# psaegert/bcnf

Hardware: AMD Instinct MI355X
Metric: NLL-training samples/sec + log_prob max-abs-err vs ref, trajectory_FC_small (higher is better)
Workload: dtype f32; 1 GPU; trajectory_FC_small NLL training step (configs[1]); batch_per_gpu=4096, global_batch=4096, parallelism=dp1, hip_graph=True, n_blocks=32, n_conditions=80

## Files before the change

bcnf_amd/_native.py:

```python
from __future__ import annotations

import ctypes
import os
import threading

import torch

_HERE = os.path.dirname(os.path.abspath(__file__))
LIB_PATH = os.environ.get("BCNF_AMD_LIB") or os.path.join(_HERE, "libbcnf_amd.so")

MAX_HIDDEN = 8

OK, ERR_ARG, ERR_UNSUPPORTED, ERR_HIP = 0, 1, 2, 3
ERR_HIP_BASE = 1000

EXPORTS = (
    "bcnf_stack_supported", "bcnf_param_count", "bcnf_packed_bytes", "bcnf_workspace_bytes",
    "bcnf_slab_bytes", "bcnf_pack_params", "bcnf_stack_forward", "bcnf_stack_backward",
    "bcnf_stack_inverse", "bcnf_grad_reduce", "bcnf_status_string",
    "bcnf_nll_forward", "bcnf_nll_backward", "bcnf_grad_partials", "bcnf_adam_step", "bcnf_adam_step_bookkeep",
    "bcnf_grad_sumsq",
    "bcnf_clip_grad_norm", "bcnf_linear_forward", "bcnf_linear_work_bytes", "bcnf_linear_backward",
    "bcnf_linear_gelu_forward", "bcnf_linear_gelu_backward",
    "bcnf_inverse_scratch_bytes", "bcnf_stack_dh", "bcnf_backward_tail", "bcnf_gather_rows2",
    "bcnf_gather_batch", "bcnf_advance_counters", "bcnf_fold_bytes", "bcnf_fold_slab_bytes",
    "bcnf_pack_params_fold", "bcnf_fold_nll_forward", "bcnf_fold_backward_tail",
    "bcnf_fold_raw_table_bytes", "bcnf_fold_raw_table", "bcnf_fold_train_forward", "bcnf_lds_fill",
    "bcnf_wide_supported", "bcnf_wide_param_count", "bcnf_wide_packed_bytes", "bcnf_wide_workspace_bytes", "bcnf_wide_inverse_scratch_bytes",
    "bcnf_wide_pack", "bcnf_wide_forward", "bcnf_wide_nll_finalize", "bcnf_wide_backward", "bcnf_wide_inverse",
    "bcnf_wide_fold_prepare", "bcnf_wide_fold_forward", "bcnf_wide_fold_backward", "bcnf_wide_proj_rows",
    "bcnf_wide_fold_backward_range", "bcnf_wide_fold_backward_phase", "bcnf_wide_block_offset",
    "bcnf_wide_gemm_test", "bcnf_wide_backward_plan", "bcnf_rank_count", "bcnf_resimulate",
    "bcnf_guard_check_global", "bcnf_abi_version",
    "bcnf_head_work_bytes", "bcnf_head_mse_forward", "bcnf_head_mse_backward", "bcnf_hybrid_finalize",
    "bcnf_stack_inverse_logdet", "bcnf_wide_inverse_logdet",
    "bcnf_attn_forward", "bcnf_attn_backward", "bcnf_add_layernorm_forward", "bcnf_add_layernorm_work_bytes",
    "bcnf_add_layernorm_backward",
)
ABI_VERSION = 2
MAX_TENSORS = 48


class BcnfStackDesc(ctypes.Structure):
    _fields_ = [
        ("size", ctypes.c_int32),
        ("n_conditions", ctypes.c_int32),
        ("n_hidden", ctypes.c_int32),
        ("hidden", ctypes.c_int32 * MAX_HIDDEN),
        ("n_blocks", ctypes.c_int32),
        ("act_norm", ctypes.c_int32),
        ("two_way", ctypes.c_int32),
        ("dropout", ctypes.c_float),
        ("gemm_tiling", ctypes.c_int32),
    ]


class BcnfFoldAdam(ctypes.Structure):
    _fields_ = [
        ("params", ctypes.c_void_p * 3),
        ("exp_avg", ctypes.c_void_p * 3),
        ("exp_avg_sq", ctypes.c_void_p * 3),
        ("step", ctypes.c_void_p),
        ("lr", ctypes.c_double),
        ("beta1", ctypes.c_double),
        ("beta2", ctypes.c_double),
        ("eps", ctypes.c_double),
        ("weight_decay", ctypes.c_double),
        ("advance_cursor", ctypes.c_void_p),
        ("cursor_modulo", ctypes.c_int64),
        ("log_values", ctypes.c_void_p),
        ("log_history", ctypes.c_void_p),
        ("done_counter", ctypes.c_void_p),
        ("guard", ctypes.c_void_p),
    ]


class BcnfGather2(ctypes.Structure):
    _fields_ = [
        ("idx", ctypes.c_void_p),
        ("cursor", ctypes.c_void_p),
        ("n", ctypes.c_int64),
        ("src0", ctypes.c_void_p),
        ("cols0", ctypes.c_int32),
        ("dst0", ctypes.c_void_p),
        ("src1", ctypes.c_void_p),
        ("cols1", ctypes.c_int32),
        ("dst1", ctypes.c_void_p),
    ]


def make_desc(size, nested_sizes, n_blocks, n_conditions, dropout=0.0, act_norm=False, two_way=False):
    d = BcnfStackDesc()
    d.size = int(size)
    d.n_conditions = int(n_conditions)
    d.n_hidden = len(nested_sizes)
    if len(nested_sizes) > MAX_HIDDEN:
        raise ValueError(f"bcnf_amd supports at most {MAX_HIDDEN} nested layers, got {len(nested_sizes)}")
    for i, hsz in enumerate(nested_sizes):
        d.hidden[i] = int(hsz)
    d.n_blocks = int(n_blocks)
    d.act_norm = 1 if act_norm else 0
    d.two_way = 1 if two_way else 0
    d.dropout = float(dropout)
    return d


_lib = None
_lock = threading.Lock()

_vp = ctypes.c_void_p
_i32 = ctypes.c_int32
_i64 = ctypes.c_int64
_pdesc = ctypes.POINTER(BcnfStackDesc)
_pi64 = ctypes.POINTER(ctypes.c_int64)


def _bind(lib):
    sig = {
        "bcnf_stack_supported": (_i32, [_pdesc]),
        "bcnf_param_count": (_i32, [_pdesc, _pi64, _pi64]),
        "bcnf_packed_bytes": (_i32, [_pdesc, _pi64]),
        "bcnf_workspace_bytes": (_i32, [_pdesc, _i64, _i32, _pi64]),
        "bcnf_slab_bytes": (_i32, [_pdesc, _i64, _pi64]),
        "bcnf_pack_params": (_i32, [_pdesc, _vp, _vp, _vp, _vp]),
        "bcnf_inverse_scratch_bytes": (_i32, [_pdesc, _i64, _pi64]),
        "bcnf_stack_dh": (_i32, [_pdesc, _vp, _vp, _i64, _i32, _vp, _vp]),
        "bcnf_backward_tail": (_i32, [_pdesc, _vp, _vp, _vp, _vp, _i64, _i32, _vp, _vp, _vp]),
        "bcnf_gather_rows2": (_i32, [_vp, _i64, _vp, _i32, _vp, _vp, _i32, _vp, _vp]),
        "bcnf_gather_batch": (_i32, [_vp, _vp, _i64, _vp, _i32, _vp, _vp, _i32, _vp, _vp]),
        "bcnf_advance_counters": (_i32, [_vp, _vp, _i64, _vp]),
        "bcnf_guard_check_global": (_i32, [_vp, _vp, _vp]),
        "bcnf_stack_forward": (_i32, [_pdesc, _vp, _vp, _vp, _i64, _vp, _vp, _vp, _i32, _vp, _vp, _i32, _vp]),
        "bcnf_stack_backward": (_i32, [_pdesc, _vp, _vp, _vp, _vp, _i64, _i32, _vp, _vp, _vp, _vp, _vp, _vp]),
        "bcnf_stack_inverse": (_i32, [_pdesc, _vp, _vp, _vp, _i64, _vp, _i64, _vp, _i32, _vp, _vp, _vp]),
        "bcnf_stack_inverse_logdet": (_i32, [_pdesc, _vp, _vp, _vp, _i64, _vp, _i64, _vp, _vp, _vp, _vp, _vp]),
        "bcnf_grad_reduce": (_i32, [_pdesc, _vp, _vp, _vp, _i64, _i32, _vp, _vp]),
        "bcnf_nll_forward": (_i32, [_pdesc, _vp, _vp, _vp, _i64, _vp, _vp, _i32, _vp, _vp, _i32, _vp, _vp, _vp]),
        "bcnf_nll_backward": (_i32, [_pdesc, _vp, _vp, _vp, _vp, _i64, _i32, _vp, _vp, _vp, _vp, _vp, _vp, _vp,
                                     _vp, _vp]),
        "bcnf_fold_bytes": (_i32, [_pdesc, _i32, _pi64]),
        "bcnf_fold_slab_bytes": (_i32, [_pdesc, _i32, _i64, _pi64]),
        "bcnf_pack_params_fold": (_i32, [_pdesc, _vp, _vp, _vp, _vp, _i32, _vp, _vp, _vp, _vp]),
        "bcnf_fold_nll_forward": (_i32, [_pdesc, _vp, _vp, _i32, _vp, _vp, _i32, _i64, _vp, _vp, _i32, _vp, _vp,
                                         _i32, _vp, _vp, _vp]),
        "bcnf_fold_raw_table_bytes": (_i32, [_pdesc, _i32, _pi64]),
        "bcnf_lds_fill": (_i32, [ctypes.c_float, _vp]),
        "bcnf_fold_raw_table": (_i32, [_pdesc, _i32, _vp]),
        "bcnf_fold_train_forward": (_i32, [_pdesc, _vp, _vp, _vp, _vp, _vp, _i32, _vp, _vp, _vp, _i32, _i64, _vp,
                                           _vp, _vp, _i32, _vp, _vp, _i32, _vp, _vp, _vp]),
        "bcnf_fold_backward_tail": (_i32, [_pdesc, _vp, _vp, _vp, _i32, _i32, _vp, _vp, _vp, _i64, _i32, _vp, _vp,
                                           _vp, _vp, _vp]),
        "bcnf_grad_partials": (_i64, [_i64]),
        "bcnf_adam_step": (_i32, [_i32, _vp, _vp, _vp, _vp, _vp, _vp, ctypes.c_double, ctypes.c_double,
                                  ctypes.c_double, ctypes.c_double, ctypes.c_double, _vp, _i32, _vp, _vp]),
        "bcnf_adam_step_bookkeep": (_i32, [_i32, _vp, _vp, _vp, _vp, _vp, _vp, ctypes.c_double, ctypes.c_double,
                                           ctypes.c_double, ctypes.c_double, ctypes.c_double, _vp, _i64, _vp, _vp,
                                           _vp, _vp, _vp]),
        "bcnf_grad_sumsq": (_i32, [_i32, _vp, _vp, _vp, _vp]),
        "bcnf_clip_grad_norm": (_i32, [_i32, _vp, _vp, _vp, ctypes.c_float, _vp, _vp, _vp, _i64, _vp, _vp, _vp,
                                       _vp]),
        "bcnf_linear_forward": (_i32, [_vp, _vp, _vp, _i64, _i32, _i32, _vp, _vp]),
        "bcnf_linear_work_bytes": (_i64, [_i64, _i32, _i32]),
        "bcnf_linear_backward": (_i32, [_vp, _vp, _vp, _i64, _i32, _i32, _vp, _vp, _vp, _vp, _vp]),
        "bcnf_linear_gelu_forward": (_i32, [_vp, _vp, _vp, _i64, _i32, _i32, ctypes.c_float, _vp, _i32, _vp, _vp,
                                            _vp]),
        "bcnf_linear_gelu_backward": (_i32, [_vp, _vp, _vp, _vp, _i64, _i32, _i32, _vp, _vp, _vp, _vp, _vp]),
        "bcnf_wide_supported": (_i32, [_pdesc]),
        "bcnf_wide_param_count": (_i32, [_pdesc, _pi64, _pi64]),
        "bcnf_wide_packed_bytes": (_i32, [_pdesc, _pi64]),
        "bcnf_wide_workspace_bytes": (_i32, [_pdesc, _i64, _i32, _pi64]),
        "bcnf_wide_inverse_scratch_bytes": (_i32, [_pdesc, _i64, _i64, _pi64]),
        "bcnf_wide_pack": (_i32, [_pdesc, _vp, _vp, _vp, _vp]),
        "bcnf_wide_forward": (_i32, [_pdesc, _vp, _vp, _vp, _vp, _i64, _vp, _vp, _vp, _i32, _vp, _vp, _i32, _vp]),
        "bcnf_wide_fold_prepare": (_i32, [_pdesc, _vp, _vp, _i32, _vp, _vp]),
        "bcnf_wide_fold_forward": (_i32, [_pdesc, _vp, _vp, _vp, _vp, _i32, _vp, _i64, _vp, _vp, _i32, _vp, _vp, _vp]),
        "bcnf_wide_fold_backward": (_i32, [_pdesc, _vp, _vp, _vp, _i32, _vp, _vp, _vp, _vp, _i64, _vp, _vp, _vp, _vp,
                                           _vp, _vp]),
        "bcnf_wide_fold_backward_range": (_i32, [_pdesc, _vp, _vp, _vp, _i32, _vp, _vp, _vp, _vp, _i64, _vp, _vp, _vp,
                                                 _vp, _vp, _i32, _i32, _vp]),
        "bcnf_wide_fold_backward_phase": (_i32, [_pdesc, _vp, _vp, _vp, _i32, _vp, _vp, _vp, _vp, _i64, _vp, _vp, _vp,
                                                 _vp, _vp, _i32, _vp]),
        "bcnf_wide_block_offset": (_i32, [_pdesc, _i32, _pi64]),
        "bcnf_wide_proj_rows": (_i32, [_pdesc, _pi64]),
        "bcnf_wide_nll_finalize": (_i32, [_pdesc, _vp, _i64, _i32, _vp, _vp, _vp, _vp]),
        "bcnf_wide_backward": (_i32, [_pdesc, _vp, _vp, _vp, _vp, _vp, _vp, _vp, _i32, _i64, _vp, _vp, _vp, _vp,
                                      _vp]),
        "bcnf_wide_inverse": (_i32, [_pdesc, _vp, _vp, _vp, _vp, _i64, _vp, _i64, _vp, _i32, _vp, _vp, _vp]),
        "bcnf_wide_inverse_logdet": (_i32, [_pdesc, _vp, _vp, _vp, _vp, _i64, _vp, _i64, _vp, _vp, _vp, _vp, _vp]),
        "bcnf_rank_count": (_i32, [_vp, _vp, _i64, _i64, _i32, _vp, _vp]),
        "bcnf_resimulate": (_i32, [_vp, _i32, _i64, _i64, _i32, _vp, _vp, _vp, _i32, ctypes.c_double, _i32,
                                   ctypes.c_double, ctypes.c_double, _i32, _vp, _vp, _vp, _vp]),
        "bcnf_wide_gemm_test": (_i32, [_i32, _i32, _i32, _i32, _vp, _i64, _vp, _i64, _vp, _i64, _vp]),
        "bcnf_wide_backward_plan": (_i32, [_pdesc, _i64, _i32, _i32, _i32, _i32, _i32, _pi64]),
        "bcnf_head_work_bytes": (_i32, [_i64, _i32, _i32, _pi64]),
        "bcnf_head_mse_forward": (_i32, [_vp, _i64, _i32, _vp, _vp, _vp, _i64, _i32, _vp, _vp]),
        "bcnf_head_mse_backward": (_i32, [_vp, _i64, _i32, _vp, _vp, _vp, ctypes.c_float, _i64, _i32, _vp, _vp, _vp,
                                          _i64, _i32, _vp]),
        "bcnf_hybrid_finalize": (_i32, [_vp, _vp, _i64, _i32, ctypes.c_float, _vp, _vp]),
        "bcnf_attn_forward": (_i32, [_vp, _vp, _vp, _i64, _i32, _i32, _i32, _i64, _vp, _vp, _vp]),
        "bcnf_attn_backward": (_i32, [_vp, _vp, _vp, _vp, _vp, _vp, _i64, _i32, _i32, _i32, _i64, _vp, _vp, _vp, _vp]),
        "bcnf_add_layernorm_forward": (_i32, [_vp, _vp, _vp, _vp, _i64, _i32, ctypes.c_float, _vp, _vp, _vp, _vp]),
        "bcnf_add_layernorm_work_bytes": (_i32, [_i64, _i32, _pi64]),
        "bcnf_add_layernorm_backward": (_i32, [_vp, _vp, _vp, _vp, _vp, _vp, _i64, _i32, _vp, _vp, _vp, _vp, _vp]),
        "bcnf_status_string": (ctypes.c_char_p, [_i32]),
        "bcnf_abi_version": (_i32, []),
    }
    override = "BCNF_AMD_LIB" in os.environ
    for name, (res, args) in sig.items():
        if override and not hasattr(lib, name):
            continue
        fn = getattr(lib, name)
        fn.restype = res
        fn.argtypes = args


def lib():
    global _lib
    if _lib is None:
        with _lock:
            if _lib is None:
                if not os.path.exists(LIB_PATH):
                    raise RuntimeError(
                        f"bcnf_amd: HIP library {LIB_PATH} is missing. Build it with "
                        "`python -c 'import __graft_entry__ as g; g.build()'` (hipcc --offload-arch=gfx950).")
                handle = ctypes.CDLL(LIB_PATH)
                _bind(handle)
                if (hasattr(handle, "bcnf_abi_version") or "BCNF_AMD_LIB" not in os.environ) and \
                        handle.bcnf_abi_version() != ABI_VERSION:
                    raise RuntimeError(f"bcnf_amd: {LIB_PATH} has ABI version {handle.bcnf_abi_version()}, the "
                                       f"bindings expect {ABI_VERSION}: rebuild the library")
                _lib = handle
    return _lib


# ... 54 lines not shown
```

bcnf_amd/csrc/bcnf_stack.hip:

```cpp
#include "bcnf_device.h"
#include "../../include/bcnf_amd.h"

#include <math.h>
#include <stdlib.h>
#include <string.h>

#include <algorithm>
#include <utility>
#include <vector>


#ifdef BCNF_PHASE_STAMPS
#define BCNF_STAMPS 1
#else
#define BCNF_STAMPS 0
#endif

namespace {

constexpr int NC16_MAX = 16;
constexpr int TILE = 256;
__host__ __device__ constexpr int tile_slot(int r, int q) { return 4 * r + ((q + (r >> 1)) & 3); }
__host__ __device__ constexpr int tile_ix(int s, int r) { return 4 * tile_slot(r, s & 3) + (s >> 2); }
__host__ __device__ constexpr int sample_of(int t8) { return (t8 >> 6) + 4 * ((t8 >> 4) & 3); }
// ... 233 lines not shown
    return rec_f(L, P, Q, k, feat(q, r), (half ? L.rf_s : L.rf_t) + 16, true);
  }
  e -= 32;
  const int q = e >> 4, r = (e >> 2) & 3, i = e & 3;
  return rec_f(L, P, Q, k, feat(q, r), i, true);
}

constexpr int RAW_NP = 10, RAW_NQ = 2, RAW_NZ = 6;
constexpr int RAW_NS = RAW_NP + RAW_NQ + RAW_NZ;
constexpr int RAW_NSP = (RAW_NS + 3) & ~3;
constexpr int RAW_DUMMY = RING - 1;
constexpr int RAW_SRC_MAX = 1 << 20;

__host__ __device__ constexpr uint32_t raw_entry(int dst, int src) { return (uint32_t)dst | ((uint32_t)src << 12); }

int q_quad_source(const BcnfLayout& L, int j, int c, bool inverse, int* off) {
  int qi, src;
  if (!q_entry(L, j, c, &qi, &src)) return 0;
  const int Da = L.Da, Db = L.Db, D = L.D;
  const int no = (qi < 2) ? Da : Db, ni = (qi & 1) ? Db : Da;
  if (j >= no || src >= ni) return 0;
  const int gi = (qi & 1) ? Da + src : src, go = (qi < 2) ? j : Da + j;
  *off = inverse ? go * D + gi : gi * D + go;
  return 2;
}

int rec_f_source(const BcnfLayout& L, int j, int e, int* off) {
  const int Da = L.Da, Db = L.Db, D = L.D, NH = L.NH, an = L.an_size;
  auto lin_w = [&](int l, int row, int col) { return an + L.lin_w[l] + row * L.lin_in[l] + col; };
  *off = 0;
  if (e < 4) {
    if (!L.act_norm) return ((e == 0 && j < Da) || (e == 2 && j < Db)) ? -1 : 0;
    switch (e) {
      case 0: return j < Da ? (*off = j, 1) : 0;
      case 1: return j < Da ? (*off = D + j, 1) : 0;
      case 2: return j < Db ? (*off = Da + j, 1) : 0;
      default: return j < Db ? (*off = D + Da + j, 1) : 0;
    }
  }
  if (e == L.rf_b1) return j < L.H[1] ? (*off = an + L.lin_b[1] + j, 1) : 0;
  if (e >= L.rf_w1 && e < L.rf_w1 + 16) {
    const int src = rec_src(L, j, e - L.rf_w1, QBC_W1);
    return (j < L.H[1] && src < Da) ? (*off = lin_w(1, j, src), 1) : 0;
  }
  if (e >= L.rf_hid && e < L.rf_t) {
    const int l = 2 + (e - L.rf_hid) / 17, r = (e - L.rf_hid) % 17;
    if (r == 16) return j < L.H[l] ? (*off = an + L.lin_b[l] + j, 1) : 0;
    const int src = (j - r) & 15;
    return (j < L.H[l] && src < L.H[l - 1]) ? (*off = lin_w(l, j, src), 1) : 0;
  }
  if (e >= L.rf_t && e < L.rf_t + 34) {
    const int half = (e - L.rf_t) / 17, r = (e - L.rf_t) % 17;
    if (r == 16) return j < Db ? (*off = an + L.lin_b[NH + 1] + half * Db + j, 1) : 0;
    const int src = (j - r) & 15;
    return (j < Db && src < L.H[NH]) ? (*off = lin_w(NH + 1, half * Db + j, src), 1) : 0;
  }
  if (e >= L.rf_q && e < L.rf_q + 64) return q_quad_source(L, j, e - L.rf_q, false, off);
  return 0;
}

int rec_b_source(const BcnfLayout& L, int j, int e, int* off) {
  const int NH = L.NH, Da = L.Da, Db = L.Db, D = L.D, an = L.an_size;
  auto lin_w = [&](int l, int row, int col) { return an + L.lin_w[l] + row * L.lin_in[l] + col; };
  *off = 0;
  if (e >= L.rb_w1t && e < L.rb_w1t + 16) {
    const int src = (j - (e - L.rb_w1t)) & 15;
    return (j < Da && src < L.H[1]) ? (*off = lin_w(1, src, j), 1) : 0;
  }
  if (e >= L.rb_hid && e < L.rb_w1t) {
    const int l = NH - (e - L.rb_hid) / 16, r = (e - L.rb_hid) % 16, src = (j - r) & 15;
    return (j < L.H[l - 1] && src < L.H[l]) ? (*off = lin_w(l, src, j), 1) : 0;
  }
  if (e >= L.rb_tt && e < L.rb_tt + 32) {
    const int half = (e - L.rb_tt) / 16, src = rec_src(L, j, (e - L.rb_tt) % 16, QBC_HEAD);
    return (j < L.H[NH] && src < Db) ? (*off = lin_w(NH + 1, half * Db + src, j), 1) : 0;
  }
  if (e >= L.rb_qt && e < L.rb_qt + 64) return q_quad_source(L, j, e - L.rb_qt, true, off);
  if (e >= L.rb_an && e < L.rb_an + 4) return rec_f_source(L, j, e - L.rb_an, off);
  return 0;
}

long long raw_table_words(const BcnfLayout& L) { return (long long)RAW_NSP * BCNF_WG + 16LL * L.RB; }

bool build_raw_table(const BcnfLayout& L, uint32_t* out) {
  if (L.nb < 2 || 16 * L.RF > RAW_DUMMY || L.blk_stride >= RAW_SRC_MAX) return false;
  std::vector<std::pair<int, int>> ent[3];
  for (int j = 0; j < 16; ++j)
    for (int e = 0; e < L.RF; ++e) {
      int off;
      const int kind = rec_f_source(L, j, e, &off);
      if (kind < 0) return false;
      ent[kind == 1 ? 0 : kind == 2 ? 1 : 2].emplace_back(off, j * L.RF + e);
    }
  const int cap[3] = {RAW_NP, RAW_NQ, RAW_NZ}, first[3] = {0, RAW_NP, RAW_NP + RAW_NQ};
  for (int i = 0; i < RAW_NSP * BCNF_WG; ++i) out[i] = raw_entry(RAW_DUMMY, 0);
  if (L.an_size > BCNF_WG) return false;
  for (int g = 0; g < 3; ++g) {
    if ((int)ent[g].size() > cap[g] * BCNF_WG) return false;
    std::sort(ent[g].begin(), ent[g].end());
    for (int n = 0; n < (int)ent[g].size(); ++n)
      out[(n % BCNF_WG) * RAW_NSP + first[g] + n / BCNF_WG] = raw_entry(ent[g][n].second, ent[g][n].first);
  }
  uint32_t* pb = out + (long long)RAW_NSP * BCNF_WG;
  for (int j = 0; j < 16; ++j)
    for (int e = 0; e < L.RB; ++e) {
      int off;
      const int kind = rec_b_source(L, j, e, &off);
      if (kind < 0 || off >= (1 << 29)) return false;
      pb[j * L.RB + e] = ((uint32_t)off << 2) | (uint32_t)(kind == 1 ? 0 : kind == 2 ? 1 : 2);
    }
  return true;
}

constexpr int PACK_WG_MAX = 4096;

__device__ __forceinline__ void pack_body(const BcnfLayout& L, const float* __restrict__ P,
                                          const float* __restrict__ Q, float* __restrict__ out, int bx, int npw,
                                          float* __restrict__ part, bool train_only = false) {
  if (bx == 0) {
    float acc = 0.f;
    if (L.act_norm) {
      const int n = (L.nb - 1) * L.D;
      for (int i = threadIdx.x; i < n; i += BCNF_WG) {
        const int k = i / L.D, d = i - k * L.D;
        acc += logf(fabsf(P[k * L.blk_stride + d]));
      }
    }
    part[threadIdx.x] = acc;
    __syncthreads();
    for (int s = BCNF_WG / 2; s > 0; s >>= 1) {
      if ((int)threadIdx.x < s) part[threadIdx.x] += part[threadIdx.x + s];
      __syncthreads();
    }
    if (threadIdx.x == 0) out[L.ldc_off] = part[0];
    return;
  }
  const int n_pf = L.nb * 16 * L.RF;
  const int n_pb = L.nb * 16 * L.RB;
  const int n_w = L.Cp * L.NKp;
  const int n_pm = L.nb * L.PMB;
  const int total = train_only ? n_pf + n_pb + n_w : 2 * n_pf + n_pb + 2 * n_w + L.NKp + n_pm;
  for (int ii0 = (bx - 1) * BCNF_WG + threadIdx.x; ii0 < total; ii0 += npw * BCNF_WG) {
    float v;
    long long o;
    const int i = (train_only && ii0 >= n_pf + n_pb) ? ii0 + n_pf + n_w : ii0;
    if (i < n_pf) {
      const int kj = i / L.RF, e = i - kj * L.RF;
      v = rec_f(L, P, Q, kj >> 4, kj & 15, e, false);
      o = L.pf_off + i;
    } else if (i < n_pf + n_pb) {
      const int ii = i - n_pf;
      const int kj = ii / L.RB, e = ii - kj * L.RB;
      v = rec_b(L, P, Q, kj >> 4, kj & 15, e);
      o = L.pb_off + ii;
    } else if (i < 2 * n_pf + n_pb) {
      const int ii = i - n_pf - n_pb;
      const int kj = ii / L.RF, e = ii - kj * L.RF;
      v = rec_f(L, P, Q, kj >> 4, kj & 15, e, true);
      o = L.pi_off + ii;
    } else if (i < 2 * n_pf + n_pb + n_w) {
      const int ii = i - 2 * n_pf - n_pb;
      const int c = ii / L.NKp, kj = ii - c * L.NKp, k = kj >> 4, j = kj & 15;
      v = (k < L.nb && j < L.H[1] && c < L.C) ? cW(L, P, k, 1, j, L.Da + c) : 0.f;
      o = L.w1c_off + ii;
    } else if (i < 2 * n_pf + n_pb + 2 * n_w) {
      const int ii = i - 2 * n_pf - n_pb - n_w;
      const int kj = ii / L.Cp, c = ii - kj * L.Cp, k = kj >> 4, j = kj & 15;
      v = (k < L.nb && j < L.H[1] && c < L.C) ? cW(L, P, k, 1, j, L.Da + c) : 0.f;
      o = L.w1r_off + ii;
    } else if (i < 2 * n_pf + n_pb + 2 * n_w + L.NKp) {
      const int kj = i - 2 * n_pf - n_pb - 2 * n_w, k = kj >> 4, j = kj & 15;
      v = (k < L.nb && j < L.H[1]) ? cB(L, P, k, 1, j) : 0.f;
      o = L.b1c_off + kj;
    } else {
      const int ii = i - 2 * n_pf - n_pb - 2 * n_w - L.NKp;
      const int k = ii / L.PMB, e = ii - k * L.PMB;
      v = rec_pm(L, P, Q, k, e);
      o = L.pm_off + ii;
    }
    out[o] = v;
  }
}

__global__ __launch_bounds__(BCNF_WG) void k_pack(BcnfLayout L, const float* __restrict__ P,
                                                  const float* __restrict__ Q, float* __restrict__ out, int npw) {
  __shared__ float part[BCNF_WG];
  pack_body(L, P, Q, out, blockIdx.x, npw, part);
}

int pack_wgs(const BcnfLayout& L, bool train_only = false) {
  const long long total = train_only ? (long long)L.nb * 16 * (L.RF + L.RB) + (long long)L.Cp * L.NKp
                                     : 2LL * L.nb * 16 * L.RF + (long long)L.nb * 16 * L.RB + 2LL * L.Cp * L.NKp +
                                           L.NKp + (long long)L.nb * L.PMB;
  const long long w = (total + BCNF_WG - 1) / BCNF_WG;
  return (int)(w < PACK_WG_MAX ? (w > 0 ? w : 1) : PACK_WG_MAX);
// ... 443 lines not shown
        const int i4 = tid + 256 * e, r = i4 >> 5, col = c0 + (i4 & 31) * 4;
        if (col < L.Cp) *reinterpret_cast<floatx4*>(Bs + r * hs + col) = rv[e];
      }
    }
    __syncthreads();
#pragma unroll
    for (int j = 0; j < NT; ++j) {
      const int n = n_lo + j;
      if (n >= n_hi) continue;
#pragma unroll
      for (int t0 = 0; t0 < KH / 4; t0 += 8) {
        float a[8], bv[8];
#pragma unroll
        for (int t = 0; t < 8; ++t) {
          a[t] = As[(16 * kw + lr) * KHP + 4 * (t0 + t) + lq];
          bv[t] = Bs[(4 * (t0 + t) + lq) * hs + 16 * n + lr];
        }
#pragma unroll
        for (int t = 0; t < 8; t += 2) {
          acc[j] = mfma4(a[t], bv[t], acc[j]);
          acc1[j] = mfma4(a[t + 1], bv[t + 1], acc1[j]);
        }
      }
    }
  }
  if (k >= L.nb) return;
  float* o = work + (((long long)s * L.nb + k) * 16) * L.Cp;
#pragma unroll
  for (int j = 0; j < NT; ++j) {
    const int n = n_lo + j;
    if (n >= n_hi) continue;
    const floatx4 r = acc[j] + acc1[j];
#pragma unroll
    for (int i = 0; i < 4; ++i) o[(long long)(4 * lq + i) * L.Cp + 16 * n + lr] = r[i];
  }
}
size_t dw1h_half_lds_bytes(const BcnfLayout& L) {
  return sizeof(float) * (size_t)(32 * KHP + KH * bstride16(L.Cp));
}

__global__ __launch_bounds__(BCNF_WG) void k_dw1h_reduce(BcnfLayout L, const float* __restrict__ work, int splits,
                                                         float* __restrict__ dparams) {
  const long long per = 16LL * L.Cp, total = (long long)L.nb * per;
  const long long i = (long long)blockIdx.x * BCNF_WG + threadIdx.x;
  if (i >= total) return;
  const int k = (int)(i / per);
  const int rem = (int)(i - (long long)k * per);
  const int j = rem / L.Cp, c = rem - j * L.Cp;
  if (j >= L.H[1] || c >= L.C) return;
  float acc = 0.f;
  int s = 0;
  for (; s + 8 <= splits; s += 8) {
    float v[8];
#pragma unroll
    for (int t = 0; t < 8; ++t) v[t] = work[(long long)(s + t) * total + i];
#pragma unroll
    for (int t = 0; t < 8; ++t) acc += v[t];
  }
  for (; s < splits; ++s) acc += work[(long long)s * total + i];
  dparams[coupling_base(L, k) + L.lin_w[1] + j * L.lin_in[1] + L.Da + c] = acc;
}

__device__ __forceinline__ void gx_reduce_body(long long total, const float* __restrict__ work, int splits,
                                               float* __restrict__ gx, long long i) {
  if (i >= total) return;
  float acc = 0.f;
  int s = 0;
  for (; s + 16 <= splits; s += 16) {
    float v[16];
#pragma unroll
    for (int t = 0; t < 16; ++t) v[t] = work[(long long)(s + t) * total + i];
#pragma unroll
    for (int t = 0; t < 16; ++t) acc += v[t];
  }
  for (; s < splits; ++s) acc += work[(long long)s * total + i];
  gx[i] = acc;
}

__global__ __launch_bounds__(BCNF_WG) void k_fold_gx(long long total, const float* __restrict__ work, int splits,
                                                     float* __restrict__ gx) {
  gx_reduce_body(total, work, splits, gx, (long long)blockIdx.x * BCNF_WG + threadIdx.x);
}

__device__ __forceinline__ int c0_of_finish(int bx, int nct) { return (bx % nct) * 16; }

constexpr int FIN_KC = 512;
constexpr int FIN_SMEM = 2 * FIN_KC * 16;

__device__ __forceinline__ void tile16_accum(const float* __restrict__ As, const float* __restrict__ Bs, int kn,
                                             floatx4 (&acc)[4]) {
  const int lane = threadIdx.x & 63, ks = lane & 15, rb = lane >> 4, cb = threadIdx.x >> 6;
#pragma unroll 4
  for (int k = ks; k < kn; k += 16) {
    const floatx4 a = *reinterpret_cast<const floatx4*>(As + k * 16 + 4 * rb);
    const floatx4 b = *reinterpret_cast<const floatx4*>(Bs + k * 16 + 4 * cb);
#pragma unroll
    for (int r = 0; r < 4; ++r)
#pragma unroll
      for (int c = 0; c < 4; ++c) acc[r][c] = fmaf(a[r], b[c], acc[r][c]);
  }
}

__device__ __forceinline__ float tile16_reduce(float* __restrict__ red, const floatx4 (&acc)[4]) {
  const int lane = threadIdx.x & 63, ks = lane & 15, rb = lane >> 4, cb = threadIdx.x >> 6;
  __syncthreads();
#pragma unroll
  for (int r = 0; r < 4; ++r)
#pragma unroll
    for (int c = 0; c < 4; ++c) red[ks * 256 + (4 * rb + r) * 16 + 4 * cb + c] = acc[r][c];
  __syncthreads();
  float v = 0.f;
#pragma unroll
  for (int q = 0; q < 16; ++q) v += red[q * 256 + threadIdx.x];
  return v;
}

__global__ __launch_bounds__(BCNF_WG) void k_fold_finish(BcnfLayout L, const float* __restrict__ pk,
                                                         const float* __restrict__ gx, const float* __restrict__ wf,
                                                         const float* __restrict__ bf, int X,
                                                         float* __restrict__ dparams, float* __restrict__ dwf,
                                                         float* __restrict__ dbf, FoldAdamArgs A) {
  extern __shared__ __attribute__((aligned(16))) float smem[];
  float* As = smem;
  float* Bs = smem + FIN_KC * 16;
  const int Xp = fold_xp(X), tid = threadIdx.x, nct = L.Cp >> 4;
  floatx4 acc[4];
#pragma unroll
  for (int q = 0; q < 4; ++q) acc[q] = floatx4{0.f, 0.f, 0.f, 0.f};
  const bool adam = A.on && !(A.guard && A.guard[BCNF_GUARD_HALTED]);
  AdamScalars as{};
  const bool keeper = adam && blockIdx.x == 0 && tid == 0;
  const bool logger = keeper && A.log_values && A.log_history;
  long long log_row = 0;
  float step0 = 0.f, log_v[3];
  if (adam) {
    as = adam_scalars_of(A, A.asc[0], A.asc[1]);
    if (keeper) {
      log_row = A.cursor ? A.cursor[0] : 0LL;
      step0 = A.step[0];
    }
    if (logger) {
#pragma unroll
      for (int i = 0; i < 3; ++i) log_v[i] = A.log_values[i];
    }
  }
  int slot = -1;
  long long idx = 0;
  float ap = 0.f, am = 0.f, av = 0.f;
  if ((int)blockIdx.x < L.nb * nct) {
    const int j = tid >> 4, c = c0_of_finish(blockIdx.x, nct) + (tid & 15), k = blockIdx.x / nct;
    if (j < L.H[1] && c < L.C) {
      slot = 0;
      idx = coupling_base(L, k) + L.lin_w[1] + j * L.lin_in[1] + L.Da + c;
    }
  } else {
    const int tile = blockIdx.x - L.nb * nct, c = (tile % nct) * 16 + (tid >> 4), x = (tile / nct) * 16 + (tid & 15);
    if (c < L.C) {
      if (x < X) {
        slot = 1;
        idx = (long long)c * X + x;
      } else if (x == X && dbf) {
        slot = 2;
        idx = c;
      }
    }
  }
// ... 174 lines not shown
  return l <= NH ? 24 + 17 * (l - 1) : (l == NH + 1 ? RecF<NH>::S + 17 : RecF<NH>::USED);
}
template <int NH>
__host__ __device__ constexpr int rf_stage_q(int l) {
  int q = 6;
  for (int i = 1; i <= l; ++i) {
    const int want = (rf_stage_end<NH>(i + FWD_AHEAD < NH + 2 ? i + FWD_AHEAD : NH + 2) + 3) / 4;
    q = i >= NH + 2 ? want : (want < q + 8 ? want : q + 8);
  }
  return q;
}
template <int NH>
__device__ __forceinline__ void rf_issue(float* __restrict__ rr, const float* __restrict__ R, int l) {
  const floatx4* R4 = reinterpret_cast<const floatx4*>(R);
#pragma unroll
  for (int q = rf_stage_q<NH>(l - 1); q < rf_stage_q<NH>(l); ++q) {
    const floatx4 v = R4[q];
    rr[4 * q] = v.x;
    rr[4 * q + 1] = v.y;
    rr[4 * q + 2] = v.z;
    rr[4 * q + 3] = v.w;
  }
  __builtin_amdgcn_sched_barrier(0);
}
template <int NH, bool KEEP, bool DROP, typename Emit>
__device__ __forceinline__ void mlp_forward_s(float* __restrict__ rr, const float* __restrict__ R, float x, float hp,
                                              const float* __restrict__ msk, float& T, float& Sp, float* ar,
                                              Emit&& emit, bool qbc) {
  static_assert(RecF<NH>::HID == 24, "stage 1 reads only the prefetched head (FWD_HEAD = 24)");
  using F = RecF<NH>;
  using AR = ActRec<NH>;
  float a = x;
#pragma unroll
  for (int l = 1; l <= NH; ++l) {
    rf_issue<NH>(rr, R, l);
    const float* w = (l == 1) ? rr + F::W1 : rr + F::HID + 17 * (l - 2);
    const float pre = (l == 1 && qbc) ? bc10(a, w, hp) : rot16(a, w, (l == 1) ? hp : w[16]);
    if (KEEP) {
      float g, dg;
      gelu_fg(pre, g, dg);
      a = DROP ? g * msk[l - 1] : g;
      ar[AR::act(l - 1)] = a;
      ar[AR::gd(l - 1)] = DROP ? dg * msk[l - 1] : dg;
#pragma unroll
      for (int q = 0; q < AR::AR4; ++q)
        if (AR::ready_layer(q) == l) emit(q);
    } else if (DROP) {
      float g, dg;
      gelu_fg(pre, g, dg);
      a = g * msk[l - 1];
    } else {
      a = gelu_f(pre);
    }
  }
  rf_issue<NH>(rr, R, NH + 1);
  T = rr[F::T + 16];
  Sp = rr[F::S + 16];
  rot16x2(a, rr + F::T, T, a, rr + F::S, Sp);
  rf_issue<NH>(rr, R, NH + 2);
}

__device__ __forceinline__ void mix(const float* __restrict__ rq, float a, float b, float& na, float& nbv) {
  na = 0.f;
  nbv = 0.f;
  rot16x2(a, rq, na, a, rq + 32, nbv);
  rot16x2(b, rq + 16, na, b, rq + 48, nbv);
}

#if BCNF_STAMPS
__device__ unsigned long long g_phase[32];
#endif

struct ProjArgs {
  const float* h;
  const float* w1c;
  const float* b1c;
  long long ldh;
  int C, Cp, NKp;
};
struct RawArgs {
  const float* P;
  const float* Q;
  const uint32_t* table;
  const float* wf;
  const float* bf;
  const float* ypool;
  float* ydst;
  const float* xpool;
  float* xdst;
  const int64_t* idx;
  const long long* cursor;
  float* pk;
  int X, ldx;
};
constexpr int RAW_WQ = 8;
constexpr int RAW_TPW = 2;
constexpr int RAW_SIDE_Q = 4;
__host__ __device__ constexpr int raw_hs_pitch(int C) { return 16 * ((C + 15) / 16) + 4; }
__device__ __forceinline__ long long raw_row(const RawArgs& R, long long B, long long b) {
  return R.idx ? (long long)R.idx[(R.cursor ? R.cursor[0] * B : 0) + b] : b;
}

constexpr int FWD_WG = 2 * BCNF_WG;
constexpr int HP_SMAX = 16;
constexpr int FWD_SLOTS = 3;
constexpr int FWD_HP = FWD_SLOTS * 4 * 256;
constexpr int FWD_HEAD = 24;

template <int NH, bool DROP, bool SAVE, bool RAW = false>
__global__ __launch_bounds__(2 * BCNF_WG) void k_forward(BcnfLayout L, const float* __restrict__ pk,
                                                    const float* __restrict__ y, ProjArgs P,
                                                    long long B, float* __restrict__ z, float* __restrict__ ldj_out,
                                                    float* __restrict__ logp, const uint64_t* rng,
                                                    float* __restrict__ arec, float* __restrict__ nll_part,
                                                    RawArgs R) {
  extern __shared__ __attribute__((aligned(16))) float smem[];
  const int RFL = 16 * L.RF;
  float* rec = smem;
  float* hpb = rec + FWD_SLOTS * RING;
  floatx4* mkb = reinterpret_cast<floatx4*>(hpb + FWD_HP);
  float* lps = hpb + FWD_HP + FWD_SLOTS * 8 * 256;
  float* hs = lps + 4;
  using AR = ActRec<NH>;
  static_assert(NH <= 8, "two float4 of dropout multipliers");
  const int nb = L.nb;
  const float* pf = pk + L.pf_off;
  const bool helper = threadIdx.x >= BCNF_WG;
  const int t8 = (int)threadIdx.x & (BCNF_WG - 1);
  const int j = t8 & 15, s = sample_of(t8);
  const long long b = (long long)blockIdx.x * 16 + s;
  const long long bc = b < B ? b : B - 1;
  uint64_t seed = 0, off = 0;
  if (DROP) { seed = rng[0]; off = rng[1]; }
  unsigned long long ph_t = BCNF_STAMPS ? __builtin_amdgcn_s_memtime() : 0ULL, ph_acc[3] = {0, 0, 0};
  const unsigned long long ph_t0 = ph_t;
  const unsigned long long ph_r0 = BCNF_STAMPS ? __builtin_amdgcn_s_memrealtime() : 0ULL;
  unsigned long long ph_b[2] = {0, 0};
#define PHB(i)                                                 \
  if (BCNF_STAMPS) ph_b[i] = __builtin_amdgcn_s_memtime() - ph_t0;
  unsigned long long ph_p[4] = {0, 0, 0, 0};
#define PHP(i)                                                                           \
  if (BCNF_STAMPS) {                                                                     \
    asm volatile("s_waitcnt vmcnt(0) lgkmcnt(0)" ::: "memory");                          \
    ph_p[i] = __builtin_amdgcn_s_memtime() - ph_t0;                                      \
  }
#define PHF(i)                                                                                   \
  if (BCNF_STAMPS) {                                                                             \
    const unsigned long long _t = __builtin_amdgcn_s_memtime();                                  \
    ph_acc[i] += _t - ph_t;                                                                      \
    ph_t = _t;                                                                                   \
  }

  if (helper) {
    const int hw = __builtin_amdgcn_readfirstlane(t8 >> 6);
    const int l64 = t8 & 63, lr = l64 & 15, lq = l64 >> 4;
    if constexpr (RAW) {
      const int Da = L.Da, C = L.C, X = R.X, H1 = L.H[1], D = L.D, an = L.an_size;
      const int nt = (C + 15) >> 4;
      const long long row = (long long)blockIdx.x * 16 + lr;
      const float* xrow = R.xpool + raw_row(R, B, row < B ? row : B - 1) * R.ldx;
      uint32_t tw[RAW_NSP];
#pragma unroll
      for (int i = 0; i < RAW_NSP / 4; ++i) {
        const uint4 v = reinterpret_cast<const uint4*>(R.table + t8 * RAW_NSP)[i];
        tw[4 * i] = v.x;
        tw[4 * i + 1] = v.y;
        tw[4 * i + 2] = v.z;
        tw[4 * i + 3] = v.w;
      }
      const int rb16 = 16 * L.RB, ch = (rb16 + BCNF_WG - 1) / BCNF_WG, n_units = nb * ch + L.NKp;
      const uint32_t* tpb = R.table + RAW_NSP * BCNF_WG;
      uint32_t pbe[RAW_SIDE_Q];
#pragma unroll
      for (int q = 0; q < RAW_SIDE_Q; ++q) {
        const int u = blockIdx.x + q * gridDim.x, n = (u % ch) * BCNF_WG + t8;
        pbe[q] = tpb[n < rb16 ? n : 0];
      }
      asm volatile("" ::: "memory");
      uint32_t srcb[RAW_NP + RAW_NQ], dstb[RAW_NP + RAW_NQ];
#pragma unroll
      for (int i = 0; i < RAW_NP + RAW_NQ; ++i) {
        srcb[i] = (tw[i] >> 12) * 4u;
        dstb[i] = (tw[i] & 4095u) * 4u;
      }
      uint32_t zw[RAW_NZ];
#pragma unroll
      for (int i = 0; i < RAW_NZ; ++i) zw[i] = tw[RAW_NP + RAW_NQ + i] & 4095u;
      PHP(0)
      int wo[RAW_TPW];
      uint32_t wok = 0;
#pragma unroll
      for (int i = 0; i < RAW_TPW; ++i) {
        const int c0 = 16 * (hw + 4 * i) + 4 * lq;
        wo[i] = (c0 < C && lr < H1) ? L.lin_w[1] + lr * L.lin_in[1] + Da + c0 : 0;
#pragma unroll
        for (int r = 0; r < 4; ++r) wok |= (c0 + r < C && lr < H1) ? 1u << (4 * i + r) : 0u;
      }
      const bool bias_lane = hw == 0 && lr < H1;
      struct Pre {
// ... 14 lines not shown
        const int cb = coupling_base(L, k);
        const int sp = (k < nb - 1 ? k * L.blk_stride : k * L.blk_stride - an) * 4, sq = k * D * D * 4;
#pragma unroll
        for (int i = 0; i < RAW_NP; ++i)
          g.v[i] = __uint_as_float(__builtin_amdgcn_raw_buffer_load_b32(rP, srcb[i], sp, 0));
#pragma unroll
        for (int i = RAW_NP; i < RAW_NP + RAW_NQ; ++i)
          g.v[i] = __uint_as_float(__builtin_amdgcn_raw_buffer_load_b32(rQ, srcb[i], sq, 0));
#pragma unroll
        for (int i = 0; i < RAW_TPW; ++i) {
          const auto w = __builtin_amdgcn_raw_buffer_load_b128(rP, wo[i] * 4, cb * 4, 0);
          g.w4[i] = floatx4{__uint_as_float(w[0]), __uint_as_float(w[1]), __uint_as_float(w[2]), __uint_as_float(w[3])};
        }
        g.bias = __uint_as_float(__builtin_amdgcn_raw_buffer_load_b32(rP, (L.lin_b[1] + lr) * 4, cb * 4, 0));
      };
      float xa[RAW_TPW][4];
      auto finish_rec = [&](int k, int sl, const Pre& g) {
        if (DROP) {
          const uint32_t bits = dropout_bits<NH>(L, seed, off, bc, k, j, 0u);
          float m[8];
#pragma unroll
          for (int i = 0; i < 8; ++i) m[i] = ((bits >> i) & 1u) ? L.keep_scale : 0.f;
          mkb[(2 * sl) * BCNF_WG + t8] = floatx4{m[0], m[1], m[2], m[3]};
          mkb[(2 * sl + 1) * BCNF_WG + t8] = floatx4{m[4], m[5], m[6], m[7]};
        }
        char* slot = reinterpret_cast<char*>(rec + sl * RING);
        float v0 = g.v[0], vq[RAW_NQ];
#pragma unroll
        for (int i = 0; i < RAW_NQ; ++i) vq[i] = g.v[RAW_NP + i];
        if (k == nb - 1) {
          v0 = an_word ? an_val : v0;
#pragma unroll
          for (int i = 0; i < RAW_NQ; ++i) vq[i] = q_diag[i] ? 1.f : vq[i];
        }
        *reinterpret_cast<float*>(slot + dstb[0]) = v0;
#pragma unroll
        for (int i = 1; i < RAW_NP; ++i) *reinterpret_cast<float*>(slot + dstb[i]) = g.v[i];
#pragma unroll
        for (int i = 0; i < RAW_NQ; ++i) *reinterpret_cast<float*>(slot + dstb[RAW_NP + i]) = vq[i];
      };
      auto finish_proj = [&](int sl, const Pre& g) {
        const float bias = bias_lane ? g.bias : 0.f;
        floatx4 acc = {bias, bias, bias, bias};
#pragma unroll
        for (int i = 0; i < RAW_TPW; ++i)
          if (hw + 4 * i < nt)
#pragma unroll
            for (int r = 0; r < 4; ++r)
              acc = mfma4(xa[i][r], ((wok >> (4 * i + r)) & 1u) ? g.w4[i][r] : 0.f, acc);
        float* hd = hpb + sl * 1024 + hw * 256 + 64 * lq + lr;
#pragma unroll
        for (int r = 0; r < 4; ++r) hd[16 * r] = acc[r];
      };
      auto finish = [&](int k, int sl, const Pre& g) {
        finish_rec(k, sl, g);
        finish_proj(sl, g);
      };
      Pre gb[FWD_SLOTS];
      load(0, gb[0]);
      load(1, gb[1]);
      load(nb > 2 ? 2 : 1, gb[2]);
      asm volatile("" ::: "memory");
      PHP(1)
#pragma unroll
      for (int i = 0; i < RAW_NZ; ++i)
#pragma unroll
        for (int sl = 0; sl < FWD_SLOTS; ++sl) rec[sl * RING + zw[i]] = 0.f;
      finish_rec(0, 0, gb[0]);
      finish_rec(1, 1, gb[1]);
      PHP(2)
      __syncthreads();
      PHB(0)
      __syncthreads();
#pragma unroll
      for (int i = 0; i < RAW_TPW; ++i) {
        const floatx4 v = *reinterpret_cast<const floatx4*>(hs + lr * raw_hs_pitch(C) + 16 * (hw + 4 * i) + 4 * lq);
#pragma unroll
        for (int r = 0; r < 4; ++r) xa[i][r] = v[r];
      }
      finish_proj(0, gb[0]);
      finish_proj(1, gb[1]);
      auto side_unit = [&](int u, uint32_t e) {
        if (u < nb * ch) {
          const int k = u / ch, n = (u - k * ch) * BCNF_WG + t8;
          if (n >= rb16) return;
          const uint32_t kind = e & 3u, src = e >> 2;
          float v = 0.f;
          if (k < nb - 1) {
            if (kind == 0) v = R.P[(long long)k * L.blk_stride + src];
            else if (kind == 1) v = R.Q[(long long)k * D * D + src];
          } else if (kind == 0) {
            v = (int)src < an ? ((int)src < D ? 1.f : 0.f) : R.P[(long long)k * L.blk_stride - an + src];
          } else if (kind == 1) {
            v = (src % (uint32_t)(D + 1)) == 0 ? 1.f : 0.f;
          }
          R.pk[L.pb_off + (long long)k * rb16 + n] = v;
        } else if (u < n_units) {
          const int kj = u - nb * ch, k = kj >> 4, jj = kj & 15;
          const bool live = k < nb && jj < H1;
          const float* w = live ? R.P + coupling_base(L, k) + L.lin_w[1] + jj * L.lin_in[1] + Da : R.P;
          for (int c = t8; c < L.Cp; c += BCNF_WG) R.pk[L.w1r_off + (long long)kj * L.Cp + c] = (live && c < C) ? w[c] : 0.f;
        }
      };
      PHB(1)
      auto interval = [&](int k, int sl) {
        load(k + 3 < nb ? k + 3 : nb - 1, gb[sl == FWD_SLOTS - 1 ? 0 : sl + 1]);
        asm volatile("" ::: "memory");
        finish(k + 2, sl, gb[sl]);
        PHF(1)
        asm volatile("s_waitcnt lgkmcnt(0)\n\ts_barrier" ::: "memory");
        PHF(2)
      };
      __syncthreads();
      PHF(0)
      for (int k = 0; k < nb - 2; k += FWD_SLOTS) {
        interval(k, 2);
        if (k + 1 < nb - 2) interval(k + 1, 0);
        if (k + 2 < nb - 2) interval(k + 2, 1);
      }
#pragma unroll
      for (int q = 0; q < RAW_SIDE_Q; ++q) side_unit(blockIdx.x + q * gridDim.x, pbe[q]);
      {
        constexpr int LU = 4;
        float acc = 0.f;
        const int n = (nb - 1) * D;
        for (int i0 = t8; i0 < n; i0 += LU * BCNF_WG) {
          float v[LU];
#pragma unroll
          for (int u = 0; u < LU; ++u) {
            const int i = i0 + u * BCNF_WG, ii = i < n ? i : 0, kb = ii / D;
            v[u] = R.P[(long long)kb * L.blk_stride + (ii - kb * D)];
          }
#pragma unroll
          for (int u = 0; u < LU; ++u)
            if (i0 + u * BCNF_WG < n) acc += logf(fabsf(v[u]));
        }
#pragma unroll
        for (int m = 32; m > 0; m >>= 1) acc += __shfl_xor(acc, m);
        if (l64 == 0) lps[hw] = acc;
      }
      __syncthreads();
      __syncthreads();
      for (int u = blockIdx.x + RAW_SIDE_Q * gridDim.x; u < n_units; u += gridDim.x)
        side_unit(u, u < nb * ch ? tpb[(u % ch) * BCNF_WG + t8 < rb16 ? (u % ch) * BCNF_WG + t8 : 0] : 0u);
    } else {
    const int S = P.Cp >> 4;
    const long long row = (long long)blockIdx.x * 16 + lr;
    const float* hrow = P.h + (row < B ? row : B - 1) * P.ldh;
    float xa[HP_SMAX];
#pragma unroll
    for (int t = 0; t < HP_SMAX; ++t) {
      const int kk = 4 * (hw * S + t) + lq;
      xa[t] = (t < S && kk < P.C) ? hrow[kk < P.C ? kk : 0] : 0.f;
    }
    const float* wcol = P.w1c + (long long)(4 * hw * S + lq) * P.NKp + lr;
    auto prepare = [&](int k, int sl) {
      Stage<STAGE_REC> sr;
      sr.load_t(pf + (long long)k * RFL, RFL, t8);
      float wb[HP_SMAX];
#pragma unroll
      for (int t = 0; t < HP_SMAX; ++t) wb[t] = (t < S) ? wcol[(long long)4 * t * P.NKp + 16 * k] : 0.f;
      if (DROP) {
        const uint32_t bits = dropout_bits<NH>(L, seed, off, bc, k, j, 0u);
        float m[8];
#pragma unroll
        for (int i = 0; i < 8; ++i) m[i] = ((bits >> i) & 1u) ? L.keep_scale : 0.f;
// ... 142 lines not shown
        if (16 * ct < C) {
          floatx4 o;
#pragma unroll
          for (int r = 0; r < 4; ++r) {
            const int cc = 16 * ct + 4 * lq + r;
            o[r] = cc < C ? (acc[i][0][r] + acc[i][1][r]) + (R.bf ? hb[i][r] : 0.f) : 0.f;
          }
          *reinterpret_cast<floatx4*>(hs + lr * raw_hs_pitch(C) + 16 * ct + 4 * lq) = o;
        }
      }
      PHB(0)
      __syncthreads();
      PHB(1)
      if (R.ydst && b < B) {
        if (j < Da) R.ydst[b * D + j] = ya;
        if (j < Db) R.ydst[b * D + Da + j] = yb;
      }
    } else {
      ya = (j < Da) ? y[bc * D + j] : 0.f;
      yb = (j < Db) ? y[bc * D + Da + j] : 0.f;
      ldc = pk[L.ldc_off];
    }
    __syncthreads();
    float hd[FWD_HEAD], hq4[4];
    floatx4 mk0 = {1.f, 1.f, 1.f, 1.f}, mk1 = {1.f, 1.f, 1.f, 1.f};
    auto fetch_head = [&](int sl) {
      ld_rec<0, FWD_HEAD>(hd, rec + sl * RING + j * L.RF);
      const float* hq = hpb + sl * 1024 + 16 * s + j;
#pragma unroll
      for (int i = 0; i < 4; ++i) hq4[i] = hq[256 * i];
      if (DROP) {
        mk0 = mkb[(2 * sl) * BCNF_WG + tid];
        mk1 = mkb[(2 * sl + 1) * BCNF_WG + tid];
      }
    };
    fetch_head(0);
    float ldj = 0.f;
    int cur = 0;
    int gdim = gridDim.x;
    asm volatile("" : "+s"(gdim));
    floatx4* d4 = reinterpret_cast<floatx4*>(arec) + (long long)blockIdx.x * AR::AR4 * BCNF_WG + tid;
    float* d1p = arec + ar1_off(nb, gdim, AR::AR4) + (long long)blockIdx.x * AR::AR1 * BCNF_WG + tid;
    const long long d4s = (long long)gdim * AR::AR4 * BCNF_WG, d1s = (long long)gdim * AR::AR1 * BCNF_WG;
    for (int k = 0; k < nb; ++k) {
      const int nxt = cur == FWD_SLOTS - 1 ? 0 : cur + 1;
      float rr[RecF<NH>::USED];
#pragma unroll
      for (int i = 0; i < FWD_HEAD; ++i) rr[i] = hd[i];
      const float hpk = ((hq4[0] + hq4[1]) + hq4[2]) + hq4[3];
      const float msk[8] = {mk0[0], mk0[1], mk0[2], mk0[3], mk1[0], mk1[1], mk1[2], mk1[3]};
      const float xa = fmaf(rr[0], ya, rr[1]);
      const float xb = fmaf(rr[2], yb, rr[3]);
      float T, Sp;
      float ar[AR::AR];
      ar[AR::YA] = ya;
      ar[AR::YB] = yb;
      auto emit = [&](int q) {
        if (SAVE) st4_wt(d4 + q * BCNF_WG, floatx4{ar[4 * q], ar[4 * q + 1], ar[4 * q + 2], ar[4 * q + 3]});
      };
      mlp_forward_s<NH, SAVE, DROP>(rr, rec + cur * RING + j * L.RF, xa, hpk, msk, T, Sp, ar, emit, QBC_DEV(L, QBC_W1));
      const float Sv = tanh_bf(Sp);
      const float zb = fmaf(exp_fast(Sv), xb, T);
      ldj += Sv;
      if (SAVE) {
        ar[AR::S] = Sv;
#pragma unroll
        for (int q = 0; q < AR::AR4; ++q)
          if (AR::ready_layer(q) == NH + 1) emit(q);
#pragma unroll
        for (int i = 0; i < AR::AR1; ++i) st1_wt(d1p + i * BCNF_WG, ar[4 * AR::AR4 + i]);
        d4 += d4s;
        d1p += d1s;
      }
      fetch_head(nxt);
      if (QBC_DEV(L, QBC_MIX)) mix_bc(rr + RecF<NH>::Q, xa, zb, ya, yb);
      else mix(rr + RecF<NH>::Q, xa, zb, ya, yb);
      cur = nxt;
      PHF(1)
      asm volatile("s_barrier" ::: "memory");
      PHF(2)
    }
    if constexpr (RAW) ldc = ((lps[0] + lps[1]) + lps[2]) + lps[3];
    const float ltot = row_sum16(ldj) + ldc;
    const float q2 = row_sum16(ya * ya + yb * yb);
    if (j < Da) z[bc * D + j] = ya;
    if (j < Db) z[bc * D + Da + j] = yb;
    if (j == 0 && ldj_out) ldj_out[bc] = ltot;
    if (logp && j == 0) logp[bc] = -(0.5f * q2 - ltot) - 0.5f * (float)D * 1.8378770664093454836f;
    if (nll_part && j == 0) rec[s] = (b < B) ? 0.5f * q2 - ltot : 0.f;
  }
#if BCNF_STAMPS
  if (SAVE && blockIdx.x == 0 && (threadIdx.x == 0 || threadIdx.x == BCNF_WG))
  {
    for (int i = 0; i < 3; ++i) g_phase[8 + (helper ? 4 : 0) + i] = ph_acc[i];
    g_phase[helper ? 15 : 11] = (ph_b[1] << 32) | (ph_b[0] & 0xffffffffULL);
    for (int i = 0; i < 4; ++i) g_phase[16 + (helper ? 4 : 0) + i] = ph_p[i];
    g_phase[24 + (helper ? 2 : 0)] = __builtin_amdgcn_s_memtime() - ph_t0;
    g_phase[25 + (helper ? 2 : 0)] = __builtin_amdgcn_s_memrealtime() - ph_r0;
  }
#endif
#undef PHF
#undef PHB
#undef PHP
  if (nll_part) {
    __syncthreads();
    if (threadIdx.x == 0) {
      float acc = 0.f;
      for (int i = 0; i < 16; ++i) acc += rec[i];
      nll_part[blockIdx.x] = acc;
    }
  }
}

template <int NTH = BCNF_WG>
__device__ void nll_finalize(const float* __restrict__ part, int nparts, long long B, float* __restrict__ loss_out,
                             uint64_t* rng_w, int32_t* guard, float* __restrict__ red) {
  float acc = 0.f;
  for (int i = threadIdx.x; i < nparts; i += NTH) acc += part[i];
  red[threadIdx.x] = acc;
  __syncthreads();
  for (int w = NTH / 2; w > 0; w >>= 1) {
    if ((int)threadIdx.x < w) red[threadIdx.x] += red[threadIdx.x + w];
    __syncthreads();
  }
  if (threadIdx.x == 0) {
    const float nll = red[0] / (float)B;
    loss_out[0] = nll;
    loss_out[1] = nll;
    loss_out[2] = 0.f;
    bool halt = false;
    if (guard) {
      if (guard[BCNF_GUARD_DIVERGED]) {
        guard[BCNF_GUARD_HALTED] = 1;
        halt = true;
      } else if (guard[BCNF_GUARD_CHECK] && (nll > 1e5f || isnan(nll))) {
        guard[BCNF_GUARD_DIVERGED] = 1;
      }
    }
    if (rng_w && !halt) rng_w[1] += 1;
  }
}

__global__ __launch_bounds__(BCNF_WG) void k_nll_finalize(const float* __restrict__ part, int nparts, long long B,
                                                          float* __restrict__ loss_out, uint64_t* rng_w,
                                                          int32_t* guard) {
  __shared__ float red[BCNF_WG];
  nll_finalize(part, nparts, B, loss_out, rng_w, guard, red);
}

template <int NH, bool DROP>
__global__ __launch_bounds__(BCNF_WG) void k_inverse(BcnfLayout L, const float* __restrict__ pk,
                                                     const float* __restrict__ zin, const float* __restrict__ hp,
                                                     long long R, const int64_t* __restrict__ cond_index, long long N,
                                                     float* __restrict__ yout, const uint64_t* __restrict__ rng) {
  extern __shared__ __attribute__((aligned(16))) float smem[];
  const int RFL = 16 * L.RF;
  float* rec = smem;
  const int tid = threadIdx.x, j = tid & 15, s = tid >> 4;
  const long long b = (long long)blockIdx.x * 16 + s;
  const long long bc = b < N ? b : N - 1;
  const int D = L.D, Da = L.Da, Db = L.Db, nb = L.nb;
  const float* pi = pk + L.pi_off;
  const long long hr = cond_index ? (long long)cond_index[bc] : bc;
  const float* hpl = hp + hr * 16 + j;
  const long long hps = R * 16;

  float ya = (j < Da) ? zin[bc * D + j] : 0.f;
  float yb = (j < Db) ? zin[bc * D + Da + j] : 0.f;
  uint64_t seed = 0, off = 0;
  if (DROP) { seed = rng[0]; off = rng[1]; }
  const int kl = nb - 1;
  float hp_n = hpl[kl * hps];
  {
    Stage<STAGE_REC> sr;
    sr.load(pi + (long long)kl * RFL, RFL);
    sr.store(rec + (kl & 1) * RING);
  }
  __syncthreads();

  for (int k = kl; k >= 0; --k) {
    const int cur = k & 1;
    const int k1 = k >= 1 ? k - 1 : 0;
    Stage<STAGE_REC> sr;
    sr.load(pi + (long long)k1 * RFL, RFL);
    const float hpk = hp_n;
    hp_n = hpl[k1 * hps];
    __builtin_amdgcn_sched_barrier(0);
    float rr[RecF<NH>::USED];
    ld_rec<0, RecF<NH>::USED>(rr, rec + cur * RING + j * L.RF);
    float za, zb;
    if (QBC_DEV(L, QBC_MIX)) mix_bc(rr + RecF<NH>::Q, ya, yb, za, zb);
    else mix(rr + RecF<NH>::Q, ya, yb, za, zb);
    uint32_t bits = 0xffu;
    if (DROP) bits = dropout_bits<NH>(L, seed, off, bc, k, j, 0x40000000u);
    float T, Sp;
    mlp_forward<NH, false>(L, rr, za, hpk, bits, DROP, T, Sp, nullptr, nullptr);
    const float S = tanh_bf(Sp);
    const float ybn = (zb - T) * exp_fast(-S);
    ya = (j < Da) ? (za - rr[1]) * rr[0] : 0.f;
    yb = (j < Db) ? (ybn - rr[3]) * rr[2] : 0.f;
    sr.store(rec + (cur ^ 1) * RING);
// ... 203 lines not shown
    }
    asm volatile("s_waitcnt vmcnt(0)" ::: "memory");
    __syncthreads();
  }
#pragma unroll
  for (int g = 0; g < G; ++g) {
    if (b[g] < N) {
#pragma unroll
      for (int r = 0; r < 4; ++r) {
        const int f = feat(r);
        if (f < Da) yout[b[g] * D + f] = ya[g][r];
        if (f < Db) yout[b[g] * D + Da + f] = yb[g][r];
      }
    }
  }
  if (LDJ) {
    const float ldc = pk[L.ldc_off];
#pragma unroll
    for (int g = 0; g < G; ++g) {
      const float ltot = sum_rows4(ls[g]) + ldc;
      if (q == 0 && b[g] < N) {
        ldj_out[b[g]] = ltot;
        if (logp_out) logp_out[b[g]] += ltot;
      }
    }
  }
}

template <int NH>
struct BwdJobs {
  static constexpr int ND = NH + 6, NA = NH + 1;
  static constexpr int NW = NH + 2, NS = NH + 6;
  static constexpr int SUM_OFF = NW * 256;
  static constexpr int BLK = NW * 256 + NS * 16;
  __device__ static constexpr int wb(int c) { return c < NH ? c : NH; }
};

__device__ __forceinline__ float sum_rows4(float v) {
  const auto p = __builtin_amdgcn_permlane32_swap(__float_as_uint(v), __float_as_uint(v), false, false);
  v = __uint_as_float(p[0]) + __uint_as_float(p[1]);
  const auto p2 = __builtin_amdgcn_permlane16_swap(__float_as_uint(v), __float_as_uint(v), false, false);
  return __uint_as_float(p2[0]) + __uint_as_float(p2[1]);
}

template <int NH>
__device__ __forceinline__ void bwd_grad_jobs(const float* __restrict__ Td, const float* __restrict__ Ta,
                                              float* __restrict__ out, int hw) {
  using J = BwdJobs<NH>;
  const int l64 = threadIdx.x & 63, q = l64 >> 4, r = l64 & 15;
  constexpr int UW = (J::NW + 3) / 4, US = (J::NS + 3) / 4;
  floatx4 a[UW], bv[UW], v[US];
  const int o = 4 * tile_slot(r, q);
#pragma unroll
  for (int u = 0; u < UW; ++u) {
    const int c = hw + 4 * u < J::NW ? hw + 4 * u : J::NW - 1;
    a[u] = *reinterpret_cast<const floatx4*>(Td + c * TILE + o);
    bv[u] = *reinterpret_cast<const floatx4*>(Ta + J::wb(c) * TILE + o);
  }
#pragma unroll
  for (int u = 0; u < US; ++u) {
    const int c = hw + 4 * u < J::NS ? hw + 4 * u : J::NS - 1;
    v[u] = *reinterpret_cast<const floatx4*>(Td + c * TILE + o);
  }
  floatx4 acc[UW];
#pragma unroll
  for (int u = 0; u < UW; ++u) acc[u] = floatx4{0.f, 0.f, 0.f, 0.f};
#pragma unroll
  for (int t = 0; t < 4; ++t)
#pragma unroll
    for (int u = 0; u < UW; ++u) acc[u] = mfma4(a[u][t], bv[u][t], acc[u]);
#pragma unroll
  for (int u = 0; u < US; ++u) {
    const float tot = sum_rows4((v[u][0] + v[u][1]) + (v[u][2] + v[u][3]));
    if (hw + 4 * u < J::NS && q == 0) out[J::SUM_OFF + 16 * (hw + 4 * u) + r] = tot;
  }
#pragma unroll
  for (int u = 0; u < UW; ++u)
    if (hw + 4 * u < J::NW) st4_wt_mfma(reinterpret_cast<floatx4*>(out + 256 * (hw + 4 * u)) + l64, acc[u]);
}

constexpr int BWD_WG = 2 * BCNF_WG;
constexpr int BWD_G4 = 3;

template <int NH>
__global__ __launch_bounds__(BWD_WG) void k_backward(BcnfLayout L, const float* __restrict__ pk,
                                                     const float* __restrict__ dz, const float* __restrict__ dldj,
                                                     const float* __restrict__ dloss, int nll, long long B,
                                                     const float* __restrict__ arec,
                                                     float* __restrict__ dy, float* __restrict__ d1,
                                                     float* __restrict__ slab_all, long long slab_stride,
                                                     const float* __restrict__ nll_part, float* __restrict__ loss_out,
                                                     uint64_t* rng_w, int32_t* guard) {
  static_assert(NH + 3 <= 4 * BWD_G4, "derivative slot");
  extern __shared__ __attribute__((aligned(16))) float smem[];
  using AR = ActRec<NH>;
  using RBk = RecB<NH>;
  using J = BwdJobs<NH>;
  const int RBL = 16 * L.RB;
  float* recB = smem;
  float* dT = recB + 2 * RING;
  float* aT = dT + 2 * J::ND * TILE;
  floatx4* gsl = reinterpret_cast<floatx4*>(aT + 3 * J::NA * TILE);
  const int nb = L.nb;
  const float* pbk = pk + L.pb_off;
  const bool helper = threadIdx.x >= BCNF_WG;
  const int t8 = (int)threadIdx.x & (BCNF_WG - 1);
  const int j = t8 & 15, s = sample_of(t8);
  const int tix = tile_ix(s, j);
  unsigned long long ph_t = BCNF_STAMPS ? __builtin_amdgcn_s_memtime() : 0ULL, ph_acc[4] = {0, 0, 0, 0};
#define PHS(i)                                                                                   \
  if (BCNF_STAMPS) {                                                                             \
    const unsigned long long _t = __builtin_amdgcn_s_memtime();                                  \
    ph_acc[i] += _t - ph_t;                                                                      \
    ph_t = _t;                                                                                   \
  }

  if (helper) {
    const int hw = __builtin_amdgcn_readfirstlane(t8 >> 6);
    float* slab = slab_all + (long long)blockIdx.x * slab_stride;
    const floatx4* arl = reinterpret_cast<const floatx4*>(arec) + (long long)blockIdx.x * AR::AR4 * BCNF_WG + t8;
    const long long ars = (long long)gridDim.x * AR::AR4 * BCNF_WG;
    struct Prep {
      Stage<STAGE_REC> sr;
      floatx4 rec[AR::AR4];
      float rec1[AR::AR1 > 0 ? AR::AR1 : 1];
      float sa, ba;
    };
    const float* ar1l = arec + ar1_off(nb, gridDim.x, AR::AR4) + (long long)blockIdx.x * AR::AR1 * BCNF_WG + t8;
    const long long ar1s = (long long)gridDim.x * AR::AR1 * BCNF_WG;
    auto prep_load = [&](Prep& P, int k) {
      P.sr.load_t(pbk + (long long)k * RBL, RBL, t8);
#pragma unroll
      for (int i = 0; i < AR::AR4; ++i) P.rec[i] = arl[(long long)k * ars + i * BCNF_WG];
#pragma unroll
      for (int i = 0; i < AR::AR1; ++i) P.rec1[i] = ar1l[(long long)k * ar1s + i * BCNF_WG];
      const float* an = pbk + (long long)k * RBL + j * L.RB + RBk::AN;
      P.sa = an[0];
      P.ba = an[1];
    };
    auto prep_store = [&](Prep& P, int k) {
#pragma unroll
      for (int i = 0; i < AR::AR4; ++i) asm volatile("" : "+v"(P.rec[i]));
#pragma unroll
      for (int i = 0; i < AR::AR1; ++i) asm volatile("" : "+v"(P.rec1[i]));
      asm volatile("" : "+v"(P.sa), "+v"(P.ba));
      float ar[4 * AR::AR4 + AR::AR1];
#pragma unroll
      for (int i = 0; i < AR::AR4; ++i) {
        ar[4 * i] = P.rec[i][0];
        ar[4 * i + 1] = P.rec[i][1];
        ar[4 * i + 2] = P.rec[i][2];
        ar[4 * i + 3] = P.rec[i][3];
      }
#pragma unroll
      for (int i = 0; i < AR::AR1; ++i) ar[4 * AR::AR4 + i] = P.rec1[i];
      float* ta = aT + (k % 3) * J::NA * TILE + tix;
#pragma unroll
      for (int l = 1; l <= NH; ++l) ta[l * TILE] = ar[AR::act(l - 1)];
      ta[0] = fmaf(P.sa, ar[AR::YA], P.ba);
      float gs[4 * BWD_G4];
#pragma unroll
      for (int l = 0; l < NH; ++l) gs[l] = ar[AR::gd(l)];
      gs[NH] = ar[AR::S];
      gs[NH + 1] = ar[AR::YA];
      gs[NH + 2] = ar[AR::YB];
#pragma unroll
      for (int i = NH + 3; i < 4 * BWD_G4; ++i) gs[i] = 0.f;
      floatx4* gd = gsl + (k & 1) * BWD_G4 * BCNF_WG + t8;
#pragma unroll
      for (int i = 0; i < BWD_G4; ++i) gd[i * BCNF_WG] = floatx4{gs[4 * i], gs[4 * i + 1], gs[4 * i + 2], gs[4 * i + 3]};
      P.sr.store_t(recB + (k & 1) * RING, t8);
    };
    Prep Pa, Pb;
    prep_load(Pa, nb - 1);
    prep_load(Pb, nb >= 2 ? nb - 2 : 0);
    prep_store(Pa, nb - 1);
    __syncthreads();
    auto step = [&](int k, Prep& Pc, Prep& Pnext) {
      PHS(0)
      prep_load(Pnext, k >= 2 ? k - 2 : 0);
      PHS(1)
      if (k + 1 < nb)
        bwd_grad_jobs<NH>(dT + ((k + 1) & 1) * J::ND * TILE, aT + ((k + 1) % 3) * J::NA * TILE,
                          slab + (long long)(k + 1) * J::BLK, hw);
      PHS(2)
      if (k >= 1) prep_store(Pc, k - 1);
      PHS(3)
      __syncthreads();
    };
    for (int k = nb - 1; k >= 0; k -= 2) {
      step(k, Pb, Pa);
      if (k == 0) break;
      step(k - 1, Pa, Pb);
    }
    bwd_grad_jobs<NH>(dT, aT, slab, hw);
  } else {
    const int tid = t8;
    const long long b = (long long)blockIdx.x * 16 + s;
    const bool valid = b < B;
    const long long bc = valid ? b : B - 1;
    const int D = L.D, Da = L.Da, Db = L.Db;
    float* d1l = d1 + bc * 16 + j;
    float* d1_dummy = d1 + (long long)nb * B * 16 + j;
    const long long hps = B * 16;

    float gya = 0.f, gyb = 0.f, dl = 0.f;
    if (valid) {
      if (nll) {
        const float sc = (dloss ? dloss[0] + dloss[1] : 1.f) / (float)B;
        gya = (j < Da) ? dz[b * D + j] * sc : 0.f;
        gyb = (j < Db) ? dz[b * D + Da + j] * sc : 0.f;
        dl = -sc;
      } else {
        if (dz) {
          gya = (j < Da) ? dz[b * D + j] : 0.f;
          gyb = (j < Db) ? dz[b * D + Da + j] : 0.f;
        }
        if (dldj) dl = dldj[b];
      }
    }
    __syncthreads();
    PHS(0)
    for (int k = nb - 1; k >= 0; --k) {
      const int cur = k & 1;
      float gs[4 * BWD_G4];
      {
        const floatx4* gd4 = gsl + cur * BWD_G4 * BCNF_WG + tid;
#pragma unroll
        for (int i = 0; i < BWD_G4; ++i) {
          const floatx4 v = gd4[i * BCNF_WG];
          gs[4 * i] = v[0];
          gs[4 * i + 1] = v[1];
          gs[4 * i + 2] = v[2];
          gs[4 * i + 3] = v[3];
        }
      }
      float* Tt = dT + cur * J::ND * TILE + tix;
      const float* R = recB + cur * RING + j * L.RB;
      float rb[RBk::USED];
      ld_rec<0, RBk::HID>(rb, R);
      __builtin_amdgcn_sched_barrier(0);
      const float* gd = gs;
      const float S = gs[NH], ya = gs[NH + 1], yb = gs[NH + 2];
      const float an_sa = rb[RBk::AN], an_sb = rb[RBk::AN + 2], an_bb = rb[RBk::AN + 3];
      const float xb = fmaf(an_sb, yb, an_bb);
      const float e = exp_fast(S);
      float gza, gzb;
      if (QBC_DEV(L, QBC_MIX)) mix_bc(rb + RBk::QT, gya, gyb, gza, gzb);
      else mix(rb + RBk::QT, gya, gyb, gza, gzb);
      ld16(rb + RBk::HID, R + RBk::HID);
      __builtin_amdgcn_sched_barrier(0);
      const float dT_ = gzb;
      const float dS = (j < Db) ? fmaf(gzb * e, xb, dl) : 0.f;
      const float dSp = dS * (1.f - S * S);
      const float dxb = gzb * e;
      Tt[NH * TILE] = dT_;
      Tt[(NH + 1) * TILE] = dSp;
      float da = 0.f, da2 = 0.f;
      if (QBC_DEV(L, QBC_HEAD)) bc9x2(dT_, rb + RBk::TT, da, dSp, rb + RBk::ST, da2);
      else rot16x2(dT_, rb + RBk::TT, da, dSp, rb + RBk::ST, da2);
      da += da2;
#pragma unroll
      for (int l = NH; l >= 2; --l) {
        ld16(rb + RBk::HID + 16 * (NH - l + 1), R + RBk::HID + 16 * (NH - l + 1));
        __builtin_amdgcn_sched_barrier(0);
        const float dpre = da * gd[l - 1];
        Tt[(l - 1) * TILE] = dpre;
        da = rot16(dpre, rb + RBk::HID + 16 * (NH - l), 0.f);
      }
      const float dpre1 = da * gd[0];
      Tt[0] = dpre1;
      *(valid ? d1l + k * hps : d1_dummy) = dpre1;
      const float dxa = rot16(dpre1, rb + RBk::W1T, gza);
      {
        const float inv_a = (j < Da) ? __builtin_amdgcn_rcpf(an_sa) : 0.f;
        const float inv_b = (j < Db) ? __builtin_amdgcn_rcpf(an_sb) : 0.f;
        Tt[(NH + 2) * TILE] = fmaf(dxa, ya, dl * inv_a);
        Tt[(NH + 3) * TILE] = dxa;
        Tt[(NH + 4) * TILE] = fmaf(dxb, yb, dl * inv_b);
        Tt[(NH + 5) * TILE] = dxb;
      }
      gya = an_sa * dxa;
      gyb = an_sb * dxb;
      PHS(1)
      __syncthreads();
      PHS(2)
    }
    if (dy && valid) {
      if (j < Da) dy[b * D + j] = gya;
      if (j < Db) dy[b * D + Da + j] = gyb;
    }
  }
#if BCNF_STAMPS
  if (blockIdx.x == 0 && (threadIdx.x == 0 || threadIdx.x == BCNF_WG))
    for (int i = 0; i < 4; ++i) g_phase[(helper ? 4 : 0) + i] = ph_acc[i];
#endif
#undef PHS
  if (loss_out && blockIdx.x == 0) {
    __syncthreads();
    nll_finalize<BWD_WG>(nll_part, (int)gridDim.x, B, loss_out, rng_w, guard, dT);
  }
}

template <int N>
__device__ __forceinline__ int lpick(const int (&a)[N], int i) {
  int r = a[0];
#pragma unroll
  for (int t = 1; t < N; ++t) r = (i == t) ? a[t] : r;
  return r;
}

__device__ __forceinline__ long long slab_to_canonical(const BcnfLayout& L, int m, int o) {
  const int NH = L.NH, NW = NH + 2;
  const int cb = m * L.blk_stride + ((m < L.nb - 1) ? L.an_size : 0);
  if (o < NW * 256) {
    const int c = o >> 8, e = o & 255, lane = e >> 2;
    const int row = 4 * (lane >> 4) + (e & 3), col = lane & 15;
    const int l = c < NH ? c + 1 : NH + 1;
    const int nrows = c < NH ? lpick(L.H, l) : L.Db, ncols = (l == 1) ? L.Da : lpick(L.H, l - 1);
    if (row >= nrows || col >= ncols) return -1;
    const int row0 = (c == NH + 1) ? L.Db : 0;
    return (long long)cb + lpick(L.lin_w, l) + (row0 + row) * lpick(L.lin_in, l) + col;
  }
  const int o2 = o - NW * 256, c = o2 >> 4, r = o2 & 15;
  if (c < NH) return r < lpick(L.H, c + 1) ? (long long)cb + lpick(L.lin_b, c + 1) + r : -1;
  if (c < NH + 2) return r < L.Db ? (long long)cb + lpick(L.lin_b, NH + 1) + ((c == NH + 1) ? L.Db : 0) + r : -1;
  const int a = c - NH - 2;
  if (a >= 4 || !L.act_norm || m >= L.nb - 1 || r >= ((a < 2) ? L.Da : L.Db)) return -1;
  return (long long)m * L.blk_stride + ((a & 1) ? L.D : 0) + ((a < 2) ? 0 : L.Da) + r;
}

constexpr int RED_G = 8, RED_O4 = 32, RED_T = 16;

constexpr int RED_SMEM = RED_G * RED_O4 * 4 + 4;

__device__ __forceinline__ void reduce_body(const BcnfLayout& L, const float* __restrict__ slab, long long stride,
                                            int nwg, float* __restrict__ out, int bx, float* __restrict__ smem,
                                            const FoldAdamArgs* A = nullptr) {
  floatx4 (*part)[RED_O4] = reinterpret_cast<floatx4 (*)[RED_O4]>(smem);
  float* sc = smem + RED_G * RED_O4 * 4;
  const int g = threadIdx.x / RED_O4, o4 = threadIdx.x % RED_O4;
  const long long i = ((long long)bx * RED_O4 + o4) * 4;
  const bool live = i < stride;
  const long long ic = live ? i : 0;
  const int m = (int)(ic / L.sblk), o = (int)(ic - (long long)m * L.sblk);
  long long ci[4];
  float ap[4], am[4], av[4];
  const float step0 = A ? A->step[0] : 0.f;
#pragma unroll
  for (int e = 0; e < 4; ++e) {
    ci[e] = slab_to_canonical(L, m, o + e);
    if (A && g == 0) {
      const long long c = ci[e] >= 0 ? ci[e] : 0;
      ap[e] = A->p[0][c];
      am[e] = A->m[0][c];
      av[e] = A->v[0][c];
    }
  }
  bool scalars_due = A != nullptr;
  auto scalars = [&]() {
    const double t = (double)(step0 + 1.0f);
    if (threadIdx.x == 0) sc[0] = (float)(A->lr / (1.0 - pow(A->b1, t)));
    if (threadIdx.x == 64) sc[1] = (float)sqrt(1.0 - pow(A->b2, t));
    scalars_due = false;
  };
  floatx4 acc = {0.f, 0.f, 0.f, 0.f};
  int w = g;
  for (; w + RED_G * (RED_T - 1) < nwg; w += RED_G * RED_T) {
    floatx4 v[RED_T];
#pragma unroll
    for (int t = 0; t < RED_T; ++t)
      v[t] = *reinterpret_cast<const floatx4*>(slab + (long long)(w + RED_G * t) * stride + ic);
    if (scalars_due) scalars();
#pragma unroll
    for (int t = 0; t < RED_T; ++t) acc += v[t];
  }
  for (; w < nwg; w += RED_G) acc += *reinterpret_cast<const floatx4*>(slab + (long long)w * stride + ic);
  if (scalars_due) scalars();
  part[g][o4] = acc;
  __syncthreads();
  if (g != 0 || !live) return;
  floatx4 tot = part[0][o4];
#pragma unroll
  for (int q = 1; q < RED_G; ++q) tot += part[q][o4];
  AdamScalars as{};
  if (A) as = adam_scalars_of(*A, sc[0], sc[1]);
#pragma unroll
  for (int e = 0; e < 4; ++e) {
    if (ci[e] < 0) continue;
    out[ci[e]] = tot[e];
    if (A) {
      adam_elem(ap[e], tot[e], am[e], av[e], as);
      A->p[0][ci[e]] = ap[e];
      A->m[0][ci[e]] = am[e];
      A->v[0][ci[e]] = av[e];
    }
  }
}

struct TailGrid {
  int n_dh, gx_dh;
  int n_red;
  int gx_dw;
};

template <bool VEC>
__global__ __launch_bounds__(BCNF_WG) void k_bwd_tail(BcnfLayout L, TailGrid G, const float* __restrict__ pk,
                                                      const float* __restrict__ d1, const float* __restrict__ h,
                                                      long long B, float* __restrict__ dh,
                                                      const float* __restrict__ slab, long long stride, int nwg,
                                                      float* __restrict__ dparams, int rows_per_split,
                                                      float* __restrict__ work) {
  extern __shared__ __attribute__((aligned(16))) float smem[];
  int i = blockIdx.x;
  if (i < G.n_dh) {
    dh_body(L, pk, d1, B, dh, i % G.gx_dh, i / G.gx_dh, smem);
    return;
  }
  i -= G.n_dh;
  if (i < G.n_red) {
    reduce_body(L, slab, stride, nwg, dparams, i, smem);
    return;
  }
  i -= G.n_red;
  dw1h_body<VEC>(L, d1, h, B, rows_per_split, work, i % G.gx_dw, i / G.gx_dw, smem);
}

template <bool VEC, int NT>
__global__ __launch_bounds__(BCNF_WG, VEC && NT <= 3 ? 4 : 2) void k_fold_tail(BcnfLayout L, BcnfLayout F, const float* __restrict__ d1,
                                                       const float* __restrict__ x, long long B, int rows_per_split,
                                                       float* __restrict__ work, int gx_dw, int n_sk, int ones,
                                                       const float* __restrict__ slab, long long stride, int nwg,
                                                       float* __restrict__ dparams, const float* __restrict__ wf,
                                                       const float* __restrict__ bf, float* __restrict__ wf1,
                                                       FoldAdamArgs A) {
  extern __shared__ __attribute__((aligned(16))) float smem[];
  const int bx = blockIdx.x;
  if (bx < n_sk) {
    dw1h_half_body<VEC, NT>(F, d1, x, B, rows_per_split, work, bx % gx_dw, bx / gx_dw, smem, ones);
    return;
  }
  if (bx == n_sk) {
    const int nw = L.C * F.C, n1 = nw + (bf ? L.C : 0);
    for (int i0 = 0; i0 < n1; i0 += 16 * BCNF_WG) {
      float v[16];
#pragma unroll
      for (int e = 0; e < 16; ++e) {
        const int i = min(i0 + e * BCNF_WG + (int)threadIdx.x, n1 - 1);
        v[e] = i < nw ? wf[i] : bf[i - nw];
      }
#pragma unroll
      for (int e = 0; e < 16; ++e) {
        const int i = i0 + e * BCNF_WG + (int)threadIdx.x;
        if (i < n1) wf1[i] = v[e];
      }
    }
    if (A.on && threadIdx.x == 0) adam_scalars_publish(A);
    return;
  }
  if (A.on && !(A.guard && A.guard[BCNF_GUARD_HALTED])) {
    reduce_body(L, slab, stride, nwg, dparams, bx - n_sk - 1, smem, &A);
    return;
  }
  reduce_body(L, slab, stride, nwg, dparams, bx - n_sk - 1, smem);
}

__global__ __launch_bounds__(BCNF_WG) void k_fill_lds(float value) {
  extern __shared__ __attribute__((aligned(16))) float smem[];
  for (int i = threadIdx.x; i < (int)(LDS_MAX / 16); i += BCNF_WG)
    reinterpret_cast<floatx4*>(smem)[i] = floatx4{value, value, value, value};
  __syncthreads();
}

template <int NH>
bool layout_matches(const BcnfLayout& L) {
  return L.rf_b1 == RecF<NH>::B1 && L.rf_w1 == RecF<NH>::W1 && L.rf_hid == RecF<NH>::HID && L.rf_t == RecF<NH>::T &&
         L.rf_s == RecF<NH>::S && L.rf_q == RecF<NH>::Q && L.RF >= RecF<NH>::USED && L.rb_w1t == RecB<NH>::W1T &&
         L.rb_hid == RecB<NH>::HID && L.rb_tt == RecB<NH>::TT && L.rb_st == RecB<NH>::ST && L.rb_qt == RecB<NH>::QT &&
         L.rb_an == RecB<NH>::AN && L.RB >= RecB<NH>::USED;
}

bool vec_rows(const BcnfLayout& L, const float* h) { return L.ldh % 4 == 0 && ((uintptr_t)h & 15) == 0; }

int launch_hp(const BcnfLayout& L, const float* pk, const float* h, long long R, float* hp, hipStream_t st) {
  const size_t lds = hp_lds_bytes();
  const dim3 grid((unsigned)((R + 63) / 64), (unsigned)(L.NKp / 64));
  return vec_rows(L, h) ? launch<k_hp<true>>(grid, dim3(BCNF_WG), lds, st, L, pk, h, R, hp)
                        : launch<k_hp<false>>(grid, dim3(BCNF_WG), lds, st, L, pk, h, R, hp);
}

template <int NH>
int fwd_dispatch(const BcnfLayout& L, const float* pk, const float* y, const ProjArgs& P, long long B, float* z,
                 float* ldj, float* logp, bool drop, const uint64_t* rng, float* arec, float* part, hipStream_t st,
                 const RawArgs* raw = nullptr) {
  if (!layout_matches<NH>(L)) return BCNF_ERR_ARG;
  if (P.Cp % 16 != 0 || P.Cp / 16 > HP_SMAX || P.C > P.Cp) return BCNF_ERR_UNSUPPORTED;
  const dim3 grid((unsigned)((B + 15) / 16));
  const size_t lds = fwd2_lds_bytes(L, raw != nullptr);
  const bool save = arec != nullptr;
  const RawArgs R = raw ? *raw : RawArgs{};
#define FWD(DR, SV, RW) \
  launch<k_forward<NH, DR, SV, RW>>(grid, dim3(2 * BCNF_WG), lds, st, L, pk, y, P, B, z, ldj, logp, rng, arec, part, R)
  if (raw) return !save ? BCNF_ERR_ARG : drop ? FWD(true, true, true) : FWD(false, true, true);
  if (save) return drop ? FWD(true, true, false) : FWD(false, true, false);
  return drop ? FWD(true, false, false) : FWD(false, false, false);
#undef FWD
}

template <int NH>
int inv_dispatch(const BcnfLayout& L, const float* pk, const float* zin, const float* hp, long long R,
                 const int64_t* ci, long long N, float* y, bool drop, const uint64_t* rng, hipStream_t st) {
  if (!layout_matches<NH>(L)) return BCNF_ERR_ARG;
  if (!drop && L.RF == inv_m_rf<NH>() && L.PMB == (NH + 6) * 256 + (NH - 1) * 16 + 96) {
    const size_t lds_m = sizeof(float) * (size_t)(2 * RING);
    const dim3 grid_m((unsigned)((N + INV_M_SPB - 1) / INV_M_SPB));
    float* const none = nullptr;
    return L.Da <= 12 && L.Db <= 12
               ? launch<k_inverse_mfma<NH, true>>(grid_m, dim3(INV_M_WG), lds_m, st, L, pk, zin, hp, R, ci, N, y, none, none)
               : launch<k_inverse_mfma<NH, false>>(grid_m, dim3(INV_M_WG), lds_m, st, L, pk, zin, hp, R, ci, N, y, none, none);
  }
  const dim3 grid((unsigned)((N + 15) / 16));
  const size_t lds = fwd_lds_bytes(L);
  return drop ? launch<k_inverse<NH, true>>(grid, dim3(BCNF_WG), lds, st, L, pk, zin, hp, R, ci, N, y, rng)
              : launch<k_inverse<NH, false>>(grid, dim3(BCNF_WG), lds, st, L, pk, zin, hp, R, ci, N, y, rng);
}

template <int NH>
int inv_ldj_dispatch(const BcnfLayout& L, const float* pk, const float* zin, const float* hp, long long R,
                     const int64_t* ci, long long N, float* y, float* ldj, float* logp, hipStream_t st) {
  if (!layout_matches<NH>(L)) return BCNF_ERR_ARG;
  if (L.RF != inv_m_rf<NH>() || L.PMB != (NH + 6) * 256 + (NH - 1) * 16 + 96) return BCNF_ERR_UNSUPPORTED;
  const size_t lds_m = sizeof(float) * (size_t)(2 * RING);
  const dim3 grid_m((unsigned)((N + INV_M_SPB - 1) / INV_M_SPB));
  return L.Da <= 12 && L.Db <= 12
             ? launch<k_inverse_mfma<NH, true, true>>(grid_m, dim3(INV_M_WG), lds_m, st, L, pk, zin, hp, R, ci, N, y, ldj, logp)
             : launch<k_inverse_mfma<NH, false, true>>(grid_m, dim3(INV_M_WG), lds_m, st, L, pk, zin, hp, R, ci, N, y, ldj, logp);
}

long long slab_stride_of(const BcnfLayout& L) { return (long long)L.nb * L.sblk; }

template <int NH>
int bwd_dispatch(const BcnfLayout& L, const float* pk, const float* dz, const float* dldj, const float* dloss,
                 int nll, long long B, const float* arec, float* dy, float* d1, float* slab, long long stride,
                 const float* part, float* loss_out, uint64_t* rng_w, int32_t* guard, hipStream_t st) {
  if (!layout_matches<NH>(L)) return BCNF_ERR_ARG;
  const dim3 grid((unsigned)((B + 15) / 16));
  return launch<k_backward<NH>>(grid, dim3(BWD_WG), bwd_lds_bytes(L), st, L, pk, dz, dldj, dloss, nll, B, arec, dy, d1,
                                slab, stride, part, loss_out, rng_w, guard);
}

constexpr int W1H_ROWS_PER_SPLIT = KC;
long long w1h_splits(long long B) { return (B + W1H_ROWS_PER_SPLIT - 1) / W1H_ROWS_PER_SPLIT; }
long long w1h_work_floats(const BcnfLayout& L, long long B) { return w1h_splits(B) * L.nb * 16LL * L.Cp; }

long long ws_part_off(const BcnfLayout& L, long long B) {
  return (long long)L.nb * ((B + 15) / 16) * BCNF_WG * act_rec_floats(L.NH);
}
long long ws_hp_off(const BcnfLayout& L, long long B) { return ws_part_off(L, B) + (((B + 15) / 16 + 3) & ~3LL); }
long long ws_d1_off(const BcnfLayout& L, long long B) { return ws_hp_off(L, B) + (long long)L.nb * B * 16; }
long long ws_floats(const BcnfLayout& L, long long B) {
  return ws_d1_off(L, B) + (long long)L.nb * B * 16 + 16;
}

int stack_setup(const BcnfStackDesc* desc, BcnfLayout* L) {
  const int rc = make_layout(desc, L);
  if (rc) return rc;
  return layout_supported(*L, desc) ? BCNF_OK : BCNF_ERR_UNSUPPORTED;
}

int forward_impl(const BcnfStackDesc* desc, const void* packed, const float* y, const float* h, int64_t batch,
                 float* z, float* ldj, float* log_prob, int32_t training, const uint64_t* rng_state, void* workspace,
                 bool save, bool nll, bool finalize, float* loss_out, int32_t* guard, void* stream,
                 const float* fold = nullptr, int X = 0, int ldx = 0, const RawArgs* raw = nullptr) {
  BcnfLayout L;
  int rc = stack_setup(desc, &L);
  if (rc) return rc;
  if (batch < 0) return BCNF_ERR_ARG;
  if (batch == 0) return nll ? BCNF_ERR_ARG : BCNF_OK;
  if (!packed || !y || !h || !z || !workspace) return BCNF_ERR_ARG;
  if (nll && finalize && !loss_out) return BCNF_ERR_ARG;
  const bool drop = training && L.p > 0.f;
  if (drop && !rng_state) return BCNF_ERR_ARG;
  float* ws = (float*)workspace;
  float* arec = (save || nll) ? ws : nullptr;
  float* part = nll ? ws + ws_part_off(L, batch) : nullptr;
  const float* pk = (const float*)packed;
  hipStream_t st = (hipStream_t)stream;
  const BcnfLayout Lp = fold ? fold_layout(L, X, ldx) : L;
  const float* pbase = fold ? fold : pk;
  const ProjArgs P{h, pbase + Lp.w1c_off, pbase + Lp.b1c_off, (long long)Lp.ldh, Lp.C, Lp.Cp, Lp.NKp};
  switch (L.NH) {
#define BCNF_CASE(N) case N: rc = fwd_dispatch<N>(L, pk, y, P, batch, z, ldj, log_prob, drop, rng_state, arec, part, st, raw); break;
    BCNF_CASE(1) BCNF_CASE(2) BCNF_CASE(3) BCNF_CASE(4) BCNF_CASE(5) BCNF_CASE(6) BCNF_CASE(7) BCNF_CASE(8)
#undef BCNF_CASE
    default: return BCNF_ERR_UNSUPPORTED;
  }
  if (rc || !nll || !finalize) return rc;
  return launch<k_nll_finalize>(dim3(1), dim3(BCNF_WG), 0, st, (const float*)part, (int)((batch + 15) / 16),
                                (long long)batch, loss_out, drop ? const_cast<uint64_t*>(rng_state) : nullptr, guard);
}

int backward_impl(const BcnfStackDesc* desc, const void* packed, const float* h, const float* dz, const float* dldj,
                  const float* dloss, int nll, int64_t batch, int32_t training, void* workspace, float* dy,
                  float* dh, float* dparams, void* slab, float* loss_out, uint64_t* rng_state, int32_t* guard,
                  void* stream);

}

extern "C" {

int bcnf_stack_supported(const BcnfStackDesc* desc) {
  BcnfLayout L;
  return stack_setup(desc, &L) == BCNF_OK ? 1 : 0;
}

int bcnf_param_count(const BcnfStackDesc* desc, int64_t* n_trainable, int64_t* n_frozen) {
  BcnfLayout L;
  const int rc = make_layout(desc, &L);
  if (rc) return rc;
  if (n_trainable) *n_trainable = L.n_trainable;
  if (n_frozen) *n_frozen = (int64_t)(L.nb - 1) * L.D * L.D;
  return BCNF_OK;
}

int bcnf_packed_bytes(const BcnfStackDesc* desc, int64_t* bytes) {
  BcnfLayout L;
  const int rc = make_layout(desc, &L);
  if (rc) return rc;
  if (!bytes) return BCNF_ERR_ARG;
  *bytes = (int64_t)L.total * (int64_t)sizeof(float);
  return BCNF_OK;
// ... 30 lines not shown
  BcnfLayout L;
  const int rc = stack_setup(desc, &L);
  if (rc) return rc;
  if (!params || !packed || (L.nb > 1 && !qmats)) return BCNF_ERR_ARG;
  const int npw = pack_wgs(L);
  return launch<k_pack>(dim3(npw + 1), dim3(BCNF_WG), 0, (hipStream_t)stream, L, params, qmats, (float*)packed, npw);
}

int bcnf_stack_forward(const BcnfStackDesc* desc, const void* packed, const float* y, const float* h, int64_t batch,
                       float* z, float* ldj, float* log_prob, int32_t training, const uint64_t* rng_state,
                       void* workspace, int32_t save, void* stream) {
  return forward_impl(desc, packed, y, h, batch, z, ldj, log_prob, training, rng_state, workspace, save != 0, false,
                      false, nullptr, nullptr, stream);
}

int bcnf_nll_forward(const BcnfStackDesc* desc, const void* packed, const float* y, const float* h, int64_t batch,
                     float* z, float* ldj, int32_t training, uint64_t* rng_state, void* workspace, int32_t finalize,
                     float* loss_out, int32_t* guard, void* stream) {
  return forward_impl(desc, packed, y, h, batch, z, ldj, nullptr, training, rng_state, workspace, true, true,
                      finalize != 0, loss_out, guard, stream);
}

int bcnf_stack_backward(const BcnfStackDesc* desc, const void* packed, const float* h, const float* dz,
                        const float* dldj, int64_t batch, int32_t training, void* workspace, float* dy,
                        float* dh, float* dparams, void* slab, void* stream) {
  return backward_impl(desc, packed, h, dz, dldj, nullptr, 0, batch, training, workspace, dy, dh, dparams, slab,
                       nullptr, nullptr, nullptr, stream);
}

int bcnf_nll_backward(const BcnfStackDesc* desc, const void* packed, const float* h, const float* z,
                      const float* dloss, int64_t batch, int32_t training, void* workspace, float* dy,
                      float* dh, float* dparams, void* slab, float* loss_out, uint64_t* rng_state, int32_t* guard,
                      void* stream) {
  if (!z && batch > 0) return BCNF_ERR_ARG;
  return backward_impl(desc, packed, h, z, nullptr, dloss, 1, batch, training, workspace, dy, dh, dparams, slab,
                       loss_out, rng_state, guard, stream);
}

int bcnf_backward_tail(const BcnfStackDesc* desc, const void* packed, const void* slab, const float* h,
                       const void* workspace, int64_t batch, int32_t training, float* dh, float* dparams,
                       void* stream) {
  BcnfLayout L;
  int rc = stack_setup(desc, &L);
  if (rc) return rc;
  if (!packed || !slab || !h || !workspace || !dparams || batch < 1) return BCNF_ERR_ARG;
  hipStream_t st = (hipStream_t)stream;
  const long long S = slab_stride_of(L);
  const int nwg = (int)((batch + 15) / 16);
  const float* d1 = (const float*)workspace + ws_d1_off(L, batch);
  float* work = (float*)slab + (long long)nwg * S;
  const int rps = W1H_ROWS_PER_SPLIT;
  const long long splits = w1h_splits(batch);
  TailGrid G;
  G.gx_dh = (int)((batch + 63) / 64);
  G.n_dh = dh ? G.gx_dh * (L.Cp >> 4) : 0;
  G.n_red = (int)((S / 4 + RED_O4 - 1) / RED_O4);
  G.gx_dw = (L.nb + 3) / 4;
  const long long n_dw = (long long)G.gx_dw * splits;
  size_t lds = dw1h_lds_bytes(L);
  if (dh_lds_bytes() > lds) lds = dh_lds_bytes();
  const dim3 grid((unsigned)(G.n_dh + G.n_red + n_dw));
  rc = vec_rows(L, h) ? launch<k_bwd_tail<true>>(grid, dim3(BCNF_WG), lds, st, L, G, (const float*)packed, d1, h,
                                                 (long long)batch, dh, (const float*)slab, S, nwg, dparams, rps, work)
                      : launch<k_bwd_tail<false>>(grid, dim3(BCNF_WG), lds, st, L, G, (const float*)packed, d1, h,
                                                  (long long)batch, dh, (const float*)slab, S, nwg, dparams, rps, work);
  if (rc) return rc;
  const long long outs = (long long)L.nb * 16 * L.Cp;
  return launch<k_dw1h_reduce>(dim3((unsigned)((outs + BCNF_WG - 1) / BCNF_WG)), dim3(BCNF_WG), 0, st, L,
                               (const float*)work, (int)splits, dparams);
}

namespace {
int fold_setup(const BcnfStackDesc* desc, int32_t X, BcnfLayout* L) {
  const int rc = stack_setup(desc, L);
  if (rc) return rc;
  if (X < 1 || fold_xp(X) > 16 * NC16_MAX) return BCNF_ERR_UNSUPPORTED;
  if (dw1h_lds_bytes(fold_layout(*L, X, X)) > LDS_MAX) return BCNF_ERR_UNSUPPORTED;
  return BCNF_OK;
}
long long fold_floats(const BcnfLayout& L, int X) { return (long long)(fold_xp(X) + 1) * L.NKp; }
bool raw_applicable(const BcnfLayout& L, int X) {
  return X <= RAW_KP - 4 && L.C <= 64 * RAW_TPW && L.nb >= 2 && L.act_norm;
}
}

int bcnf_fold_bytes(const BcnfStackDesc* desc, int32_t in_features, int64_t* bytes) {
  BcnfLayout L;
  const int rc = fold_setup(desc, in_features, &L);
  if (rc) return rc;
  if (!bytes) return BCNF_ERR_ARG;
  *bytes = fold_floats(L, in_features) * 4;
  return BCNF_OK;
}

int bcnf_fold_slab_bytes(const BcnfStackDesc* desc, int32_t in_features, int64_t batch, int64_t* bytes) {
  BcnfLayout L;
  const int rc = fold_setup(desc, in_features, &L);
  if (rc) return rc;
  if (!bytes || batch < 0) return BCNF_ERR_ARG;
  const BcnfLayout F = fold_layout(L, in_features, in_features);
  *bytes = ((int64_t)((batch + 15) / 16) * slab_stride_of(L) + w1h_work_floats(F, batch) +
            (int64_t)L.nb * 16 * F.Cp + 4 +
            (int64_t)L.C * (in_features + 1)) * 4;
  return BCNF_OK;
}

int bcnf_pack_params_fold(const BcnfStackDesc* desc, const float* params, const float* qmats,
                          const float* feat_weight, const float* feat_bias, int32_t in_features, void* packed,
                          float* fold, const BcnfGather2* gather, void* stream) {
  BcnfLayout L;
  int rc = fold_setup(desc, in_features, &L);
  if (rc) return rc;
  if (!params || !packed || !fold || !feat_weight || (L.nb > 1 && !qmats)) return BCNF_ERR_ARG;
  BcnfGatherArgs ga = {};
  if (gather) {
    const BcnfGather2& g = *gather;
    if (g.n < 1 || g.cols0 < 1 || g.cols1 < 1 || !g.idx || !g.src0 || !g.dst0 || !g.src1 || !g.dst1)
      return BCNF_ERR_ARG;
    if (g.n * (int64_t)(g.cols0 + g.cols1) >= (1LL << 31)) return BCNF_ERR_UNSUPPORTED;
    ga = BcnfGatherArgs{g.idx, (const long long*)g.cursor, g.src0, g.dst0, g.src1, g.dst1, (int)g.n, 0, g.cols0,
                        g.cols1, 0};
    gather2_plan(g.n, &ga.rpw, &ga.nwg);
  }
  const int npw = pack_wgs(L, true);
  const unsigned grid = (unsigned)(L.NKp / 16 * FOLD_SPLIT + ga.nwg + npw + 1);
  return launch<k_pack_fold>(dim3(grid), dim3(BCNF_WG), 0, (hipStream_t)stream, L, params, qmats, (float*)packed,
                             feat_weight, feat_bias, (int)in_features, fold, ga, npw);
}

int bcnf_fold_nll_forward(const BcnfStackDesc* desc, const void* packed, const float* fold, int32_t in_features,
                          const float* y, const float* x, int32_t ldx, int64_t batch, float* z, float* ldj, int32_t training,
                          uint64_t* rng_state, void* workspace, int32_t finalize, float* loss_out, int32_t* guard,
                          void* stream) {
  BcnfLayout L;
  const int rc = fold_setup(desc, in_features, &L);
  if (rc) return rc;
  if (!fold || ldx < in_features) return BCNF_ERR_ARG;
  return forward_impl(desc, packed, y, x, batch, z, ldj, nullptr, training, rng_state, workspace, true, true,
                      finalize != 0, loss_out, guard, stream, fold, in_features, ldx);
}

int bcnf_lds_fill(float value, void* stream) {
  return launch<k_fill_lds>(dim3(4 * 256), dim3(BCNF_WG), LDS_MAX, (hipStream_t)stream, value);
}

int bcnf_fold_raw_table_bytes(const BcnfStackDesc* desc, int32_t in_features, int64_t* bytes) {
  BcnfLayout L;
  const int rc = fold_setup(desc, in_features, &L);
  if (rc) return rc;
  if (!bytes) return BCNF_ERR_ARG;
  if (!raw_applicable(L, in_features)) return BCNF_ERR_UNSUPPORTED;
  std::vector<uint32_t> t((size_t)raw_table_words(L));
  if (!build_raw_table(L, t.data())) return BCNF_ERR_UNSUPPORTED;
  *bytes = (int64_t)t.size() * (int64_t)sizeof(uint32_t);
  return BCNF_OK;
}

int bcnf_fold_raw_table(const BcnfStackDesc* desc, int32_t in_features, void* host_table) {
  BcnfLayout L;
  const int rc = fold_setup(desc, in_features, &L);
  if (rc) return rc;
  if (!host_table) return BCNF_ERR_ARG;
  if (!raw_applicable(L, in_features)) return BCNF_ERR_UNSUPPORTED;
  return build_raw_table(L, (uint32_t*)host_table) ? BCNF_OK : BCNF_ERR_UNSUPPORTED;
}

int bcnf_fold_train_forward(const BcnfStackDesc* desc, const float* params, const float* qmats, const void* table,
                            const float* feat_weight, const float* feat_bias, int32_t in_features,
                            const BcnfGather2* gather, const float* y, const float* x, int32_t ldx, int64_t batch,
                            void* packed, float* z, float* ldj, int32_t training, uint64_t* rng_state,
                            void* workspace, int32_t finalize, float* loss_out, int32_t* guard, void* stream) {
  BcnfLayout L;
  const int rc = fold_setup(desc, in_features, &L);
  if (rc) return rc;
  if (!raw_applicable(L, in_features)) return BCNF_ERR_UNSUPPORTED;
  if (!params || !qmats || !table || !feat_weight || !packed || batch < 1) return BCNF_ERR_ARG;
  RawArgs R = {};
  R.P = params;
  R.Q = qmats;
  R.table = (const uint32_t*)table;
  R.wf = feat_weight;
  R.bf = feat_bias;
  R.pk = (float*)packed;
  R.X = in_features;
  if (gather) {
    const BcnfGather2& g = *gather;
    if (g.n != batch || g.cols0 != L.D || g.cols1 < in_features || !g.idx || !g.src0 || !g.src1 || !g.dst0 ||
        !g.dst1)
      return BCNF_ERR_ARG;
    R.idx = g.idx;
    R.cursor = (const long long*)g.cursor;
    R.ypool = g.src0;
    R.ydst = g.dst0;
    R.xpool = g.src1;
    R.xdst = g.dst1;
    R.ldx = g.cols1;
  } else {
    if (!y || !x || ldx < in_features) return BCNF_ERR_ARG;
    R.ypool = y;
    R.xpool = x;
    R.ldx = ldx;
  }
  return forward_impl(desc, packed, R.ypool, R.xpool, batch, z, ldj, nullptr, training, rng_state, workspace, true,
                      true, finalize != 0, loss_out, guard, stream, nullptr, 0, 0, &R);
}

int bcnf_fold_backward_tail(const BcnfStackDesc* desc, const void* packed, const void* slab, const float* x,
                            int32_t ldx, int32_t in_features, const float* feat_weight, const float* feat_bias,
                            const void* workspace, int64_t batch, int32_t training, float* dparams,
                            float* dfeat_weight, float* dfeat_bias, const BcnfFoldAdam* adam, void* stream) {
  BcnfLayout L;
  int rc = fold_setup(desc, in_features, &L);
  if (rc) return rc;
  if (!packed || !slab || !x || !feat_weight || !workspace || !dparams || batch < 1 || ldx < in_features)
    return BCNF_ERR_ARG;
  FoldAdamArgs A = {};
  if (adam) {
    const BcnfFoldAdam& a = *adam;
    if (!a.params[0] || !a.exp_avg[0] || !a.exp_avg_sq[0] || !a.params[1] || !a.exp_avg[1] || !a.exp_avg_sq[1] ||
        !a.step || !a.done_counter || (feat_bias && (!a.params[2] || !a.exp_avg[2] || !a.exp_avg_sq[2])) ||
        (a.advance_cursor && a.cursor_modulo < 1))
      return BCNF_ERR_ARG;
    for (int t = 0; t < 3; ++t) {
      A.p[t] = a.params[t];
      A.m[t] = a.exp_avg[t];
      A.v[t] = a.exp_avg_sq[t];
    }
    if (!feat_bias) A.p[2] = A.m[2] = A.v[2] = nullptr;
    A.step = a.step;
    A.lr = a.lr;
    A.b1 = a.beta1;
    A.b2 = a.beta2;
    A.eps = a.eps;
    A.wd = a.weight_decay;
    A.cursor = (long long*)a.advance_cursor;
    A.n_batches = (long long)a.cursor_modulo;
    A.log_values = a.log_values;
    A.log_history = a.log_history;
    A.done = (int*)a.done_counter;
    A.guard = (const int*)a.guard;
    A.on = 1;
  }
  const BcnfLayout F = fold_layout(L, in_features, ldx);
  hipStream_t st = (hipStream_t)stream;
  const long long S = slab_stride_of(L);
  const int nwg = (int)((batch + 15) / 16);
  const float* d1 = (const float*)workspace + ws_d1_off(L, batch);
  float* work = (float*)slab + (long long)nwg * S;
  float* gx = work + w1h_work_floats(F, batch);
  A.asc = gx + (long long)L.nb * 16 * F.Cp;
  const int rps = W1H_ROWS_PER_SPLIT;
  const long long splits = w1h_splits(batch);
  float* wf1 = A.asc + 4;
  const float* bf1 = feat_bias ? wf1 + (long long)L.C * in_features : nullptr;
  const int n_red = (int)((S / 4 + RED_O4 - 1) / RED_O4);
  const int gx_dw = (L.nb + 1) / 2;
  const long long n_sk = (long long)gx_dw * splits;
  const dim3 grid((unsigned)(n_sk + 1 + n_red));
  size_t lds = dw1h_half_lds_bytes(F);
  if (lds < sizeof(float) * RED_SMEM) lds = sizeof(float) * RED_SMEM;
  const bool vec = vec_rows(F, x);
  const bool nt3 = (F.Cp >> 4) <= 6;
#define FOLD_TAIL(V, NT)                                                                                          \
  launch<k_fold_tail<V, NT>>(grid, dim3(BCNF_WG), lds, st, L, F, d1, x, (long long)batch, rps, work, gx_dw, (int)n_sk, \
                             (int)in_features, (const float*)slab, S, nwg, dparams, feat_weight, feat_bias, wf1, A)
  rc = vec ? (nt3 ? FOLD_TAIL(true, 3) : FOLD_TAIL(true, 8)) : (nt3 ? FOLD_TAIL(false, 3) : FOLD_TAIL(false, 8));
#undef FOLD_TAIL
  if (rc) return rc;
  const long long total = (long long)L.nb * 16 * F.Cp;
  rc = launch<k_fold_gx>(dim3((unsigned)((total + BCNF_WG - 1) / BCNF_WG)), dim3(BCNF_WG), 0, st, total,
                         (const float*)work, (int)splits, gx);
  if (rc) return rc;
  const int n_fin = (L.nb + (F.Cp >> 4)) * (L.Cp >> 4);
  return launch<k_fold_finish>(dim3((unsigned)n_fin), dim3(BCNF_WG), sizeof(float) * FIN_SMEM, st, L,
                               (const float*)packed, (const float*)gx, (const float*)wf1, bf1, (int)in_features,
                               dparams, dfeat_weight, dfeat_bias, A);
}

int bcnf_grad_reduce(const BcnfStackDesc* desc, const void* slab, const float* h, const void* workspace,
                     int64_t batch, int32_t training, float* dparams, void* stream) {
  return bcnf_backward_tail(desc, slab, slab, h, workspace, batch, training, nullptr, dparams, stream);
}

int bcnf_stack_dh(const BcnfStackDesc* desc, const void* packed, const void* workspace, int64_t batch, int32_t training,
                  float* dh, void* stream) {
  BcnfLayout L;
  const int rc = stack_setup(desc, &L);
  if (rc) return rc;
  if (batch < 0 || !packed || !workspace || !dh) return BCNF_ERR_ARG;
  if (batch == 0) return BCNF_OK;
  const float* d1 = (const float*)workspace + ws_d1_off(L, batch);
  return launch<k_dh>(dim3((unsigned)((batch + 63) / 64), (unsigned)(L.Cp >> 4)), dim3(BCNF_WG), dh_lds_bytes(),
                      (hipStream_t)stream, L, (const float*)packed, d1, (long long)batch, dh);
}

int bcnf_stack_inverse(const BcnfStackDesc* desc, const void* packed, const float* z, const float* h, int64_t h_rows,
                       const int64_t* cond_index, int64_t n_rows, float* y, int32_t training,
                       const uint64_t* rng_state, void* scratch, void* stream) {
  BcnfLayout L;
  int rc = stack_setup(desc, &L);
  if (rc) return rc;
  if (n_rows == 0) return BCNF_OK;
  if (n_rows < 0 || h_rows < 1 || !packed || !z || !h || !y || !scratch) return BCNF_ERR_ARG;
  if (!cond_index && h_rows != n_rows) return BCNF_ERR_ARG;
  const bool drop = training && L.p > 0.f;
  if (drop && !rng_state) return BCNF_ERR_ARG;
  const float* pk = (const float*)packed;
  hipStream_t st = (hipStream_t)stream;
  float* hp = (float*)scratch;
  if ((rc = launch_hp(L, pk, h, h_rows, hp, st))) return rc;
  switch (L.NH) {
#define BCNF_CASE(N) case N: return inv_dispatch<N>(L, pk, z, hp, h_rows, cond_index, n_rows, y, drop, rng_state, st);
    BCNF_CASE(1) BCNF_CASE(2) BCNF_CASE(3) BCNF_CASE(4) BCNF_CASE(5) BCNF_CASE(6) BCNF_CASE(7) BCNF_CASE(8)
#undef BCNF_CASE
    default: return BCNF_ERR_UNSUPPORTED;
  }
}

int bcnf_stack_inverse_logdet(const BcnfStackDesc* desc, const void* packed, const float* z, const float* h,
                              int64_t h_rows, const int64_t* cond_index, int64_t n_rows, float* y, float* ldj,
                              float* log_prob, void* scratch, void* stream) {
  if (!desc) return BCNF_ERR_ARG;
  if (desc->two_way) return BCNF_ERR_UNSUPPORTED;
  if (!y || !ldj) return BCNF_ERR_ARG;
  BcnfLayout L;
  int rc = stack_setup(desc, &L);
  if (rc) return rc;
  if (n_rows == 0) return BCNF_OK;
  if (n_rows < 0 || h_rows < 1 || !packed || !z || !h || !scratch) return BCNF_ERR_ARG;
  if (!cond_index && h_rows != n_rows) return BCNF_ERR_ARG;
  const float* pk = (const float*)packed;
  hipStream_t st = (hipStream_t)stream;
  float* hp = (float*)scratch;
  if ((rc = launch_hp(L, pk, h, h_rows, hp, st))) return rc;
  switch (L.NH) {
#define BCNF_CASE(N) case N: return inv_ldj_dispatch<N>(L, pk, z, hp, h_rows, cond_index, n_rows, y, ldj, log_prob, st);
    BCNF_CASE(1) BCNF_CASE(2) BCNF_CASE(3) BCNF_CASE(4) BCNF_CASE(5) BCNF_CASE(6) BCNF_CASE(7) BCNF_CASE(8)
#undef BCNF_CASE
    default: return BCNF_ERR_UNSUPPORTED;
  }
}

const char* bcnf_status_string(int status) {
  switch (status) {
    case BCNF_OK: return "ok";
    case BCNF_ERR_ARG: return "invalid argument";
    case BCNF_ERR_UNSUPPORTED: return "unsupported stack shape for the fused kernel family";
    default: return status >= BCNF_ERR_HIP_BASE ? hipGetErrorString((hipError_t)(status - BCNF_ERR_HIP_BASE))
                                                 : "unknown status";
  }
}

#if BCNF_STAMPS
int bcnf_debug_phases(unsigned long long* out) {
  return bcnf_rt::hip_status(hipMemcpyFromSymbol(out, HIP_SYMBOL(g_phase), sizeof(g_phase)));
}
#endif


// ... 39 lines not shown
```

bcnf_amd/fused.py:

```python
from __future__ import annotations

import ctypes
import math
import os
from dataclasses import dataclass

import torch

from bcnf_amd import _native as N


@dataclass
class StackConfig:
    size: int
    nested_sizes: tuple
    n_blocks: int
    n_conditions: int
    dropout: float
    act_norm: bool
    two_way: bool

    def desc(self):
        return N.make_desc(self.size, list(self.nested_sizes), self.n_blocks, self.n_conditions, self.dropout,
                           self.act_norm, self.two_way)
# ... 228 lines not shown
        z = torch.empty_like(y)
        ldj = torch.empty(B, dtype=torch.float32, device=y.device)
        rng = self.rng_state() if self._dropping(training) else None
        wb, _ = self.workspace_bytes(B, training)
        ws = torch.empty(max(wb // 4, 1), dtype=torch.float32, device=y.device)
        return z, ldj, rng, ws

    def _backward_buffers(self, h, slab_bytes, want_dy, want_dh):
        slab = torch.empty(max(slab_bytes // 4, 1), dtype=torch.float32, device=h.device)
        dparams = torch.empty_like(self.flat)
        dh = torch.empty_like(h) if want_dh else None
        dy = torch.empty((h.shape[0], self.cfg.size), dtype=torch.float32, device=h.device) if want_dy else None
        return slab, dparams, dh, dy

    def launch_forward(self, y, h, training: bool, save: bool, want_logp: bool = False):
        self._check_forward(y, h)
        B = y.shape[0]
        z, ldj, rng, ws = self._forward_buffers(y, training)
        logp = torch.empty(B, dtype=torch.float32, device=y.device) if want_logp else None
        pk = self.packed(fresh=save)
        N.call("bcnf_stack_forward", self._pdesc, pk, y, h, B, z, ldj, logp, training, rng, ws, save,
               N.stream_handle(y.device))
        self._advance_rng(rng)
        return z, ldj, logp, (ws, pk)

    def launch_backward(self, h, dz, dldj, training: bool, saved, want_dy: bool, want_dh: bool):
        ws, pk = saved
        B = h.shape[0]
        slab, dparams, dh, dy = self._backward_buffers(h, self.workspace_bytes(B, training)[1], want_dy, want_dh)
        N.call("bcnf_stack_backward", self._pdesc, pk, h, dz, dldj, B, training, ws, dy, None, None, slab,
               N.stream_handle(h.device))
        N.call(*self._tail_call(h, saved, slab, training, dh, dparams))
        return dy, dh, dparams

    def _tail_call(self, h, saved, slab, training, dh, dparams):
        ws, pk = saved
        return ("bcnf_backward_tail", self._pdesc, pk, slab, h, ws, h.shape[0], training, dh, dparams,
                N.stream_handle(h.device))

    def _nll_forward_call(self, y, h, training, finalize):
        self._check_forward(y, h)
        B = y.shape[0]
        if B == 0:
            raise ValueError("bcnf_amd: the NLL of an empty batch is undefined")
        z, ldj, rng, ws = self._forward_buffers(y, training)
        vals = torch.empty(3, dtype=torch.float32, device=y.device)
        pk = self.packed(fresh=True)
        launch = ("bcnf_nll_forward", self._pdesc, pk, y, h, B, z, ldj, training, rng, ws, finalize, vals,
                  self.guard if finalize else None, N.stream_handle(y.device))
        return launch, (z, ldj, vals, (ws, pk))

    def launch_nll_forward(self, y, h, training: bool, finalize: bool = True):
        launch, out = self._nll_forward_call(y, h, training, finalize)
        N.call(*launch)
        return out

    def _nll_backward_call(self, rows, z, dvals, training, saved, slab, dy, finalize_into):
        ws, pk = saved
        rng = self.rng_state() if (finalize_into is not None and self._dropping(training)) else None
        return ("bcnf_nll_backward", self._pdesc, pk, rows, z, dvals, rows.shape[0], training, ws, dy, None, None, slab,
                finalize_into, rng, self.guard if finalize_into is not None else None, N.stream_handle(rows.device))

    def _nll_backward_calls(self, h, z, dvals, training, saved, want_dy, want_dh, finalize_into=None):
        slab, dparams, dh, dy = self._backward_buffers(h, self.workspace_bytes(h.shape[0], training)[1], want_dy,
                                                       want_dh)
        return ((self._nll_backward_call(h, z, dvals, training, saved, slab, dy, finalize_into),
                 self._tail_call(h, saved, slab, training, dh, dparams)), (dy, dh, dparams))

    def launch_nll_backward(self, h, z, dvals, training: bool, saved, want_dy: bool, want_dh: bool,
                            finalize_into=None):
        launches, out = self._nll_backward_calls(h, z, dvals, training, saved, want_dy, want_dh, finalize_into)
        for launch in launches:
            N.call(*launch)
        return out

    def fold_supported(self, in_features: int) -> bool:
        return N.query_status("bcnf_fold_bytes", self._pdesc, int(in_features))[0] == N.OK

    use_raw_forward = os.environ.get("BCNF_FOLD_RAW", "1") != "0"

    def raw_table(self, X: int):
        if not self.use_raw_forward or not hasattr(N.lib(), "bcnf_fold_train_forward"):
            return None
        dev = self.flat.device
        key = (X, str(dev))
        if key not in self._raw_tables:
            if torch.cuda.is_current_stream_capturing():
                return None
            rc, (nb,) = N.query_status("bcnf_fold_raw_table_bytes", self._pdesc, X)
            if rc != N.OK:
                self._raw_tables[key] = None
            else:
                host = torch.empty(nb // 4, dtype=torch.int32)
                N.call("bcnf_fold_raw_table", self._pdesc, X, host)
                self._raw_tables[key] = host.to(dev)
        return self._raw_tables[key]

    def _fold_forward_calls(self, y, x, wf, bf, training, finalize, gather):
        self._check_device(y, x, wf, bf)
        B, X = x.shape
        if y.dim() != 2 or y.shape != (B, self.cfg.size):
            raise ValueError(f"bcnf_amd folded forward: y {tuple(y.shape)} vs x {tuple(x.shape)}")
        if B == 0:
            raise ValueError("bcnf_amd: the NLL of an empty batch is undefined")
        stream = N.stream_handle(y.device)
        pk = self._empty_pack()
        table = self.raw_table(X)
        z, ldj, rng, ws = self._forward_buffers(y, training)
        vals = torch.empty(3, dtype=torch.float32, device=y.device)
        guard = self.guard if finalize else None
        if table is not None:
            launches = (("bcnf_fold_train_forward", self._pdesc, self.flat, self.qflat, table, wf, bf, X, gather, y, x,
                         x.stride(0), B, pk, z, ldj, training, rng, ws, finalize, vals, guard, stream),)
        else:
            fold = torch.empty(N.query_i64("bcnf_fold_bytes", self._pdesc, X) // 4, dtype=torch.float32,
                               device=y.device)
            launches = (("bcnf_pack_params_fold", self._pdesc, self.flat, self.qflat, wf, bf, X, pk, fold, gather,
                         stream),
                        ("bcnf_fold_nll_forward", self._pdesc, pk, fold, X, y, x, x.stride(0), B, z, ldj, training,
                         rng, ws, finalize, vals, guard, stream))
        return launches, (z, ldj, vals, (ws, pk))

    def launch_fold_nll_forward(self, y, x, wf, bf, training: bool, finalize: bool = True, gather=None):
        launches, out = self._fold_forward_calls(y, x, wf, bf, training, finalize, gather)
        for launch in launches:
            N.call(*launch)
        return out

    pending_adam = None
    grad_bucket = None

    def _fold_backward_calls(self, x, z, dvals, wf, bf, training, saved, want_feat, finalize_into=None, adam=None):
        ws, pk = saved
        B, X = x.shape
        sb = N.query_i64("bcnf_fold_slab_bytes", self._pdesc, X, B)
        slab = torch.empty(max(sb // 4, 1), dtype=torch.float32, device=x.device)
        gb = self.grad_bucket
        if gb is not None and want_feat:
            bucket, offs = gb
            dparams = bucket.narrow(0, offs[0], self.flat.numel()).view_as(self.flat)
            dwf = bucket.narrow(0, offs[1], wf.numel()).view_as(wf)
            dbf = bucket.narrow(0, offs[2], bf.numel()).view_as(bf) if bf is not None else None
        else:
            dparams = torch.empty_like(self.flat)
            dwf = torch.empty_like(wf) if want_feat else None
            dbf = torch.empty_like(bf) if (want_feat and bf is not None) else None
        tail = ("bcnf_fold_backward_tail", self._pdesc, pk, slab, x, x.stride(0), X, wf, bf, ws, B, training, dparams,
                dwf, dbf, adam, N.stream_handle(x.device))
        return ((self._nll_backward_call(x, z, dvals, training, saved, slab, None, finalize_into), tail),
                (dparams, dwf, dbf))

    def launch_fold_nll_backward(self, x, z, dvals, wf, bf, training: bool, saved, want_feat: bool,
                                 finalize_into=None, adam=None):
        launches, out = self._fold_backward_calls(x, z, dvals, wf, bf, training, saved, want_feat, finalize_into, adam)
        for launch in launches:
            N.call(*launch)
        return out

    @torch.no_grad()
    def time_kernels(self, y, h, training: bool = True, iters: int = 20, fold=None):
        if fold is None:
            forward, (z, _, _, saved) = self._nll_forward_call(y, h, training, finalize=False)
            (backward, tail), _ = self._nll_backward_calls(h, z, None, training, saved, want_dy=False, want_dh=True)
            calls = {"k_forward": forward}
        else:
            x, wf, bf = fold
            forwards, (z, _, _, saved) = self._fold_forward_calls(y, x, wf, bf, training, finalize=False, gather=None)
            (backward, tail), _ = self._fold_backward_calls(x, z, None, wf, bf, training, saved, want_feat=True)
            calls = dict(zip(("k_pack_fold", "k_forward")[-len(forwards):], forwards))
        calls.update(k_backward=backward, tail=tail)
        return self._time_calls(calls, iters)

    def _inverse_scratch_bytes(self, feature_rows, n):
        return N.query_i64("bcnf_inverse_scratch_bytes", self._pdesc, feature_rows)

    def _native_inverse(self, z, h, cond_index, y, training, rng, scratch):
        N.call("bcnf_stack_inverse", self._pdesc, self.packed(), z, h, h.shape[0], cond_index, z.shape[0], y, training,
               rng, scratch, N.stream_handle(z.device))

    def _native_inverse_logdet(self, z, h, cond_index, y, training, ldj, logp, scratch):
        rc = N.call_raw("bcnf_stack_inverse_logdet", self._pdesc, self.packed(), z, h, h.shape[0], cond_index,
                           z.shape[0], y, ldj, logp, scratch, N.stream_handle(z.device))
        if rc == N.ERR_UNSUPPORTED:
            y = self.launch_inverse(z, h, cond_index, training)
            hh = h if cond_index is None else h.index_select(0, cond_index)
            _, ldj, _, _ = self.launch_forward(y, hh.contiguous(), False, save=False)
            return y, ldj, log_prob_of_latent(z, ldj)
        N.check(rc, "bcnf_stack_inverse_logdet")
        return y, ldj, logp


class _StackForward(torch.autograd.Function):

    @staticmethod
    def forward(ctx, y, h, flat_param, stack: StackBase, training: bool):
        needs = ctx.needs_input_grad
        save = any(needs[:3])
        z, ldj, _, saved = stack.launch_forward(y, h, training, save=save)
        ctx.stack = stack
        ctx.training = training
        ctx.saved = saved
        ctx.save_for_backward(h)
        return z, ldj

    @staticmethod
    def backward(ctx, dz, dldj):
        (h,) = ctx.saved_tensors
        stack = ctx.stack
        if dz is not None:
            dz = dz.contiguous()
        if dldj is not None:
            dldj = dldj.contiguous()
        need_y, need_h, need_p = ctx.needs_input_grad[0], ctx.needs_input_grad[1], ctx.needs_input_grad[2]
        dy, dh, dparams = stack.launch_backward(h, dz, dldj, ctx.training, ctx.saved, want_dy=need_y, want_dh=need_h)
        return dy, dh, (dparams if need_p else None), None, None


class _StackNLL(torch.autograd.Function):

    @staticmethod
    def forward(ctx, y, h, flat_param, stack: StackBase, training: bool, defer: bool):
        z, _, vals, saved = stack.launch_nll_forward(y, h, training, finalize=not defer)
        ctx.stack = stack
        ctx.training = training
        ctx.saved = saved
        ctx.defer = defer
        ctx.save_for_backward(h, z, vals)
        return vals

    @staticmethod
    def backward(ctx, dvals):
        h, z, vals = ctx.saved_tensors
        need_y, need_h, need_p = ctx.needs_input_grad[0], ctx.needs_input_grad[1], ctx.needs_input_grad[2]
        dy, dh, dparams = ctx.stack.launch_nll_backward(h, z, dvals.contiguous(), ctx.training, ctx.saved,
                                                        want_dy=need_y, want_dh=need_h,
                                                        finalize_into=vals if ctx.defer else None)
        return dy, dh, (dparams if need_p else None), None, None, None
# ... 18 lines not shown
    B, K = h.shape
    N.call("bcnf_head_mse_forward", h, h.stride(0), K, wp, bp, y, B, y.shape[1], work, N.stream_handle(h.device))


def launch_head_backward(h, wp, work, dvals, weight: float, D: int, dwp, dbp, dh, accumulate: bool):
    B, K = h.shape
    N.call("bcnf_head_mse_backward", h, h.stride(0), K, wp, work, dvals, weight, B, D, dwp, dbp, dh,
           dh.stride(0) if dh is not None else K, accumulate, N.stream_handle(h.device))


def launch_hybrid_finalize(vals, work, B: int, D: int, weight: float, guard):
    N.call("bcnf_hybrid_finalize", vals, work, B, D, weight, guard, N.stream_handle(vals.device))


class _HybridNLL(torch.autograd.Function):

    @staticmethod
    def forward(ctx, y, h, flat_param, wp, bp, stack: StackBase, training: bool, defer: bool, weight: float):
        z, _, vals, saved = stack.launch_nll_forward(y, h, training, finalize=not defer)
        B, D = y.shape
        work = head_workspace(B, h.shape[1], D, y.device)
        launch_head_forward(h, wp, bp, y, work)
        if not defer:
            launch_hybrid_finalize(vals, work, B, D, weight, stack.hybrid_guard())
        ctx.stack, ctx.training, ctx.saved, ctx.defer, ctx.weight, ctx.work = stack, training, saved, defer, weight, work
        ctx.has_bias = bp is not None
        ctx.save_for_backward(h, z, vals, wp)
        return vals

    @staticmethod
    def backward(ctx, dvals):
        h, z, vals, wp = ctx.saved_tensors
        stack, w, work = ctx.stack, ctx.weight, ctx.work
        need_y, need_h, need_p, need_w, need_b = ctx.needs_input_grad[:5]
        dvals = dvals.contiguous()
        B, D = z.shape
        hc = stack.hybrid_cot
        if hc is not None and hc[2] == w and dvals.data_ptr() == hc[0].data_ptr():
            cot = hc[1]
        else:
            cot = dvals * dvals.new_tensor([1.0 / (1.0 + w), 1.0, 0.0])
        dy, dh, dparams = stack.launch_nll_backward(h, z, cot, ctx.training, ctx.saved, want_dy=need_y,
                                                    want_dh=need_h, finalize_into=vals if ctx.defer else None)
        dwp = torch.empty_like(wp) if need_w else None
        dbp = torch.empty(D, dtype=torch.float32, device=wp.device) if (need_b and ctx.has_bias) else None
        if need_h or need_w or dbp is not None:
            launch_head_backward(h, wp, work, dvals, w, D, dwp, dbp, dh, accumulate=True)
        if need_y:
            g = dvals[0] * (w / (1.0 + w)) + dvals[2]
            dy = dy - (2.0 * g / (B * D)) * work[:B * D].view(B, D)
        if ctx.defer:
            launch_hybrid_finalize(vals, work, B, D, w, stack.hybrid_guard())
        return dy, dh, (dparams if need_p else None), dwp, dbp, None, None, None, None


def stack_hybrid(stack: StackBase, y, h, wp, bp, weight: float, training: bool, defer: bool = False):
    y = y.contiguous()
    h = h.contiguous()
    stack._check_device(y, h, wp, bp)
    if tuple(wp.shape) != (y.shape[1], h.shape[1]) or not wp.is_contiguous() or \
            (bp is not None and not bp.is_contiguous()):
        raise ValueError(f"bcnf_amd hybrid loss: prediction head {tuple(wp.shape)} does not map features "
                         f"{tuple(h.shape)} to {tuple(y.shape)}")
    stack.sync_grad_state()
    params_grad = stack.trainable[0].requires_grad
    fp = stack.flat_param
    any_grad = params_grad or y.requires_grad or h.requires_grad or wp.requires_grad or \
        (bp is not None and bp.requires_grad)
    if torch.is_grad_enabled() and any_grad:
        return _HybridNLL.apply(y, h, fp if params_grad else fp.detach(), wp, bp, stack, training, defer,
                                float(weight))
    z, _, vals, _ = stack.launch_nll_forward(y, h, training)
    B, D = y.shape
    work = head_workspace(B, h.shape[1], D, y.device)
    launch_head_forward(h, wp, bp, y, work)
    launch_hybrid_finalize(vals, work, B, D, float(weight), stack.hybrid_guard())
    return vals


class _FoldNLL(torch.autograd.Function):

    @staticmethod
    def forward(ctx, y, x, wf, bf, flat_param, stack: FusedStack, training: bool, defer: bool, gather):
        z, _, vals, saved = stack.launch_fold_nll_forward(y, x, wf, bf, training, finalize=not defer, gather=gather)
        ctx.stack = stack
        ctx.training = training
        ctx.saved = saved
        ctx.defer = defer
        ctx.save_for_backward(x, wf, bf, z, vals)
        return vals

    @staticmethod
    def backward(ctx, dvals):
        x, wf, bf, z, vals = ctx.saved_tensors
        need = ctx.needs_input_grad
        adam, ctx.stack.pending_adam = ctx.stack.pending_adam, None
        dparams, dwf, dbf = ctx.stack.launch_fold_nll_backward(x, z, dvals.contiguous(), wf, bf, ctx.training,
                                                               ctx.saved, want_feat=need[2] or need[3] or
                                                               adam is not None,
                                                               finalize_into=vals if ctx.defer else None, adam=adam)
        return (None, None, dwf if need[2] else None, dbf if need[3] else None, dparams if need[4] else None,
                None, None, None, None)


def stack_nll_fold(stack: FusedStack, y, x, wf, bf, training: bool, defer: bool = False, gather=None):
    if gather is not None and not (y.is_contiguous() and x.stride(1) == 1):
        raise ValueError("bcnf_amd: a deferred gather needs its own (contiguous) output buffers")
    y = y.contiguous()
    if x.stride(1) != 1 or x.stride(0) < x.shape[1]:
        x = x.contiguous()
    stack.sync_grad_state()
    params_grad = stack.trainable[0].requires_grad
    fp = stack.flat_param
    feat_grad = wf.requires_grad or (bf is not None and bf.requires_grad)
    if torch.is_grad_enabled() and (params_grad or feat_grad):
        return _FoldNLL.apply(y, x, wf, bf, fp if params_grad else fp.detach(), stack, training, defer, gather)
    return stack.launch_fold_nll_forward(y, x, wf, bf, training, gather=gather)[2]


def log_prob_of_latent(z, ldj):
    return -0.5 * z.pow(2).sum(dim=-1) + ldj - 0.5 * z.shape[-1] * math.log(2.0 * math.pi)


class _StackInverse(torch.autograd.Function):
    @staticmethod
    def forward(ctx, z, h, stack: StackBase, cond_index, training: bool, want_ldj: bool = False):
        out = stack.launch_inverse(z, h, cond_index, training, want_ldj)
        if want_ldj:
            ctx.mark_non_differentiable(*out[1:])
        return out

    @staticmethod
    def backward(ctx, dy, *unused):
        raise NotImplementedError("bcnf_amd: CondRealNVP_v2.inverse is not differentiable (sampling path); "
                                  "run it under torch.no_grad().")


def _set_standalone_params(stack: StackBase, flat, device):
    stack.flat = flat.detach().contiguous()
    if stack.qflat is None or stack.qflat.device != device:
        stack.qflat = torch.zeros(1, dtype=torch.float32, device=device)


def stack_forward(stack: StackBase, y, h, training: bool, flat=None):
    y = y.contiguous()
    h = h.contiguous()
    if flat is not None:
        _set_standalone_params(stack, flat, y.device)
        fp = flat
        params_grad = flat.requires_grad
    else:
        stack.sync_grad_state()
        params_grad = stack.trainable[0].requires_grad
        fp = stack.flat_param
    if torch.is_grad_enabled():
        if params_grad or y.requires_grad or h.requires_grad:
            return _StackForward.apply(y, h, fp if params_grad else fp.detach(), stack, training)
    z, ldj, _, _ = stack.launch_forward(y, h, training, save=False)
    return z, ldj


def stack_inverse(stack: StackBase, z, h, cond_index=None, training: bool = False, flat=None,
                  want_ldj: bool = False):
    z = z.contiguous()
    h = h.contiguous()
    if flat is not None:
        _set_standalone_params(stack, flat, z.device)
    if torch.is_grad_enabled() and (z.requires_grad or h.requires_grad):
        return _StackInverse.apply(z, h, stack, cond_index, training, want_ldj)
    return stack.launch_inverse(z, h, cond_index, training, want_ldj)
```

bcnf_amd/train.py:

```python
from __future__ import annotations

import contextlib
import math
import os

import torch
import torch.distributed as dist

from bcnf_amd.errors import TrainingDivergedError
from bcnf_amd.optim import FusedAdam, clip_grad_norm_
from bcnf_amd.utils import inn_nll_loss

GUARD_CHECK, GUARD_DIVERGED, GUARD_HALTED, GUARD_CHECK_GLOBAL, GUARD_WORDS = 0, 1, 2, 3, 4


class _PackedParameters:

    def __init__(self, members):
        self.members = list(members)
        dev = self.members[0].device
        flat = torch.empty(sum(p.numel() for p in self.members), dtype=torch.float32, device=dev)
        self.slices = []
        off = 0
        with torch.no_grad():
# ... 38 lines not shown
            feature = [p for p in self.params if id(p) in members]
            if feature and all(p.is_cuda and p.dtype == torch.float32 for p in feature):
                self._packed = _PackedParameters(feature)
                self.params = [p for p in self.params if id(p) not in members]
                self.params.insert(1, self._packed.param)
        self.hybrid_weight = float(hybrid_weight)
        self.max_norm = max_norm
        self.capture = capture and not self.layerwise
        self.pg = process_group
        self.world = dist.get_world_size(process_group) if (dist.is_available() and dist.is_initialized()) else 1
        self.opt = FusedAdam(self.params, lr=lr)
        self.mse = torch.nn.MSELoss()
        self.fused_loss = self.hybrid_weight == 0.0
        self._cot_stack = None
        self._cot = None
        self._graphs = None
        self._static = None
        self._pool = None
        self._multi = {}
        self._single_grads = None
        self._rebind = False
        self._book = None
        self._g2_hidden = None
        self._g21 = None
        self._cond_shape = None
        self._epoch = None
        self._bucket = None
        self._n_grad = 0
        self._gvals = None
        self._packed_inplace = False
        self._host_cursor = 0
        self.last_clip_norm = None
        self.overlap_ranges = 0
        self._works = []
        self._reduced = []
        self._hooks = None
        from bcnf_amd.wide import WideStack
        if self.world > 1 and overlap_ranges > 0 and isinstance(getattr(model, "fused", None), WideStack):
            self.overlap_ranges = min(int(overlap_ranges), model.fused.cfg.n_blocks)
            self.capture = False
        dev = self.params[0].device
        self._side = None
        if dev.type == "cuda" and self.overlap_ranges == 0 and isinstance(getattr(model, "fused", None), WideStack) \
                and os.environ.get("BCNF_WIDE_SIDE", "0") != "0":
            self._side = torch.cuda.Stream(device=dev)
        self._guard = None
        self._hist = None
        if dev.type == "cuda":
            self._guard = torch.zeros(GUARD_WORDS, dtype=torch.int32, device=dev)
            model.fused.guard = self._guard
            self._hist = torch.zeros((1, 3), dtype=torch.float32, pin_memory=True)

    def _forward_backward(self, y, traj, gather=None, adam=None):
        if self._packed is not None:
            if not self._packed.intact():
                raise RuntimeError("bcnf_amd TrainStep: the model's feature-network parameters were replaced (moved or "
                                   "cast) after this TrainStep packed them; build a new TrainStep")
            self._packed.clear()
        with self._stack_hooks(), self._side_overlap():
            vals = self._forward_backward_body(y, traj, gather, adam)
        if self._packed is not None:
            self._packed.gather()
        return vals

    @contextlib.contextmanager
    def _side_overlap(self):
        if self._side is None:
            yield
            return
        st = self.model.fused
        st.side_stream = self._side
        try:
            yield
        except BaseException:
            st.side_stream = None
            st.join_side(None)
            raise
        st.side_stream = None
        st.join_side(st.flat_param)

    def _forward_backward_body(self, y, traj, gather=None, adam=None):
        self.opt.zero_grad(set_to_none=True)
        if self.fused_loss:
            vals = self.model.nll_loss(y, traj, defer_reduction=True, gather=gather)
            if self._cot is None or self._cot.device != vals.device:
                self._cot = torch.tensor([1.0, 0.0, 0.0], device=vals.device)
            if adam is not None:
                self.model.fused.pending_adam = adam(vals)
            torch.autograd.backward(vals, self._cot)
            if adam is not None and self.model.fused.pending_adam is not None:
                self.model.fused.pending_adam = None
                raise RuntimeError("bcnf_amd TrainStep: the folded backward did not take the fused Adam update")
            return vals.detach()
        if self.hybrid:
            vals = self.model.hybrid_loss(y, traj, hybrid_weight=self.hybrid_weight, defer_reduction=True)
            if self._cot is None or self._cot.device != vals.device:
                self._cot = torch.tensor([1.0, 0.0, 0.0], device=vals.device)
                self._cot_stack = torch.tensor([1.0 / (1.0 + self.hybrid_weight), 0.0, 0.0], device=vals.device)
            st = self.model.fused
            st.hybrid_cot = (self._cot, self._cot_stack, self.hybrid_weight)
            st.hybrid_judge = self.world == 1
            try:
                torch.autograd.backward(vals, self._cot)
            finally:
                st.hybrid_cot = None
                st.hybrid_judge = True
            return vals.detach()
        z, h = self.model(y, traj, log_det_J=True, return_features=True)
        nll = inn_nll_loss(z, self.model.log_det_J)
        mse = self.mse(self.model.prediction_head(h), y)
        loss = (nll + mse * self.hybrid_weight) / (1 + self.hybrid_weight)
        loss.backward()
        return torch.stack([loss.detach(), nll.detach(), mse.detach()])

    def _pack_grads(self):
        grads = [p.grad for p in self.params]
        if any(g is None for g in grads):
            raise RuntimeError("bcnf_amd TrainStep: a parameter received no gradient")
        if self._bucket is None:
            self._alloc_bucket(grads[0].device)
        base, off, slots = self._bucket.data_ptr(), 0, []
        for g in grads:
            slots.append((g, off, g.is_contiguous() and g.data_ptr() == base + 4 * off))
            off += g.numel()
        self._packed_inplace = all(ok for _, _, ok in slots)
        if self._packed_inplace:
            return
        if not any(ok for _, _, ok in slots):
            torch.cat([g.reshape(-1) for g in grads], out=self._bucket[:self._n_grad])
            return
        for g, o, ok in slots:
            if ok:
                continue
            if any(lo < o + g.numel() and o < hi for lo, hi in self._reduced):
                raise RuntimeError("bcnf_amd TrainStep: a gradient of an already all-reduced bucket slice is not in "
                                   "its slot")
            self._bucket[o:o + g.numel()].copy_(g.reshape(-1))

    def _alloc_bucket(self, dev):
        self._n_grad = sum(p.numel() for p in self.params)
        self._bucket = torch.zeros(self._n_grad + 4, dtype=torch.float32, device=dev)
        self._gvals = self._bucket[self._n_grad:self._n_grad + 3]

    def _setup_bucket(self):
        if self.world == 1 or self._bucket is not None:
            return
        self._alloc_bucket(self.params[0].device)
        lin = self.model._fold_linear() if hasattr(self.model, "_fold_linear") else None
        if lin is None or not self.fused_loss or self.layerwise:
            return
        offs, off = {}, 0
        for p in self.params:
            offs[id(p)] = off
            off += p.numel()
        fp = self.model.fused.flat_param
        from bcnf_amd.wide import WideStack
        if isinstance(self.model.fused, WideStack):
            if id(fp) not in offs:
                return
            st = self.model.fused
            hooks = {"grad_bucket": (self._bucket, offs[id(fp)])}
            if self.overlap_ranges > 0:
                nb, r = st.cfg.n_blocks, self.overlap_ranges
                cuts = [round(nb * i / r) for i in range(r + 1)]
                hooks["range_blocks"] = [(cuts[i - 1], cuts[i]) for i in range(r, 0, -1) if cuts[i] > cuts[i - 1]]
                hooks["on_range"] = self._reduce_range
            self._hooks = hooks
            return
        if len(self.params) != (3 if lin.bias is not None else 2) or id(fp) not in offs or id(lin.weight) not in offs:
# ... 475 lines not shown
```

include/bcnf_amd.h:

```cpp
#ifndef BCNF_AMD_H
#define BCNF_AMD_H

#include <stdint.h>

#ifdef __cplusplus
extern "C" {
#endif

#define BCNF_MAX_HIDDEN 8
#define BCNF_MAX_TENSORS 48
#define BCNF_AMD_ABI_VERSION 2

int bcnf_abi_version(void);

enum {
  BCNF_OK = 0,
  BCNF_ERR_ARG = 1,
  BCNF_ERR_UNSUPPORTED = 2,
  BCNF_ERR_HIP = 3
};
#define BCNF_ERR_HIP_BASE 1000

typedef struct BcnfStackDesc {
  int32_t size;
// ... 4 lines not shown
  int32_t act_norm;
  int32_t two_way;
  float dropout;
  int32_t gemm_tiling;
} BcnfStackDesc;

int bcnf_stack_supported(const BcnfStackDesc* desc);

int bcnf_param_count(const BcnfStackDesc* desc, int64_t* n_trainable, int64_t* n_frozen);

int bcnf_packed_bytes(const BcnfStackDesc* desc, int64_t* bytes);

int bcnf_workspace_bytes(const BcnfStackDesc* desc, int64_t batch, int32_t training, int64_t* bytes);

int bcnf_slab_bytes(const BcnfStackDesc* desc, int64_t batch, int64_t* bytes);

int bcnf_inverse_scratch_bytes(const BcnfStackDesc* desc, int64_t h_rows, int64_t* bytes);

int bcnf_pack_params(const BcnfStackDesc* desc, const float* params, const float* qmats, void* packed,
                     void* stream);

int bcnf_stack_forward(const BcnfStackDesc* desc, const void* packed, const float* y, const float* h,
                       int64_t batch, float* z, float* ldj, float* log_prob, int32_t training,
                       const uint64_t* rng_state, void* workspace, int32_t save, void* stream);

int bcnf_stack_backward(const BcnfStackDesc* desc, const void* packed, const float* h, const float* dz,
                        const float* dldj, int64_t batch, int32_t training, void* workspace, float* dy,
                        float* dh, float* dparams, void* slab, void* stream);

int bcnf_stack_dh(const BcnfStackDesc* desc, const void* packed, const void* workspace, int64_t batch,
                  int32_t training, float* dh, void* stream);

int bcnf_backward_tail(const BcnfStackDesc* desc, const void* packed, const void* slab, const float* h,
                       const void* workspace, int64_t batch, int32_t training, float* dh, float* dparams,
                       void* stream);

int bcnf_fold_bytes(const BcnfStackDesc* desc, int32_t in_features, int64_t* bytes);
int bcnf_fold_slab_bytes(const BcnfStackDesc* desc, int32_t in_features, int64_t batch, int64_t* bytes);
typedef struct BcnfGather2 {
  const int64_t* idx;
  const int64_t* cursor;
  int64_t n;
  const float* src0;
  int32_t cols0;
  float* dst0;
  const float* src1;
  int32_t cols1;
  float* dst1;
} BcnfGather2;
int bcnf_pack_params_fold(const BcnfStackDesc* desc, const float* params, const float* qmats,
                          const float* feat_weight, const float* feat_bias, int32_t in_features, void* packed,
                          float* fold, const BcnfGather2* gather , void* stream);
int bcnf_fold_nll_forward(const BcnfStackDesc* desc, const void* packed, const float* fold, int32_t in_features,
                          const float* y, const float* x, int32_t ldx, int64_t batch, float* z, float* ldj,
                          int32_t training,
                          uint64_t* rng_state, void* workspace, int32_t finalize, float* loss_out, int32_t* guard,
                          void* stream);
int bcnf_fold_raw_table_bytes(const BcnfStackDesc* desc, int32_t in_features, int64_t* bytes);
int bcnf_fold_raw_table(const BcnfStackDesc* desc, int32_t in_features, void* host_table);
int bcnf_fold_train_forward(const BcnfStackDesc* desc, const float* params, const float* qmats, const void* table,
                            const float* feat_weight, const float* feat_bias, int32_t in_features,
                            const BcnfGather2* gather , const float* y, const float* x, int32_t ldx,
                            int64_t batch, void* packed, float* z, float* ldj, int32_t training,
                            uint64_t* rng_state, void* workspace, int32_t finalize, float* loss_out, int32_t* guard,
                            void* stream);
typedef struct BcnfFoldAdam {
  float* params[3];
  float* exp_avg[3];
  float* exp_avg_sq[3];
  float* step;
  double lr, beta1, beta2, eps, weight_decay;
  int64_t* advance_cursor;
  int64_t cursor_modulo;
  const float* log_values;
  float* log_history;
  int32_t* done_counter;
  const int32_t* guard;
} BcnfFoldAdam;
int bcnf_fold_backward_tail(const BcnfStackDesc* desc, const void* packed, const void* slab, const float* x,
                            int32_t ldx, int32_t in_features, const float* feat_weight, const float* feat_bias,
                            const void* workspace, int64_t batch, int32_t training, float* dparams,
                            float* dfeat_weight, float* dfeat_bias, const BcnfFoldAdam* adam ,
                            void* stream);

int bcnf_grad_reduce(const BcnfStackDesc* desc, const void* slab, const float* h, const void* workspace,
                     int64_t batch, int32_t training, float* dparams, void* stream);

int bcnf_stack_inverse(const BcnfStackDesc* desc, const void* packed, const float* z, const float* h,
                       int64_t h_rows, const int64_t* cond_index, int64_t n_rows, float* y, int32_t training,
                       const uint64_t* rng_state, void* scratch, void* stream);

int bcnf_stack_inverse_logdet(const BcnfStackDesc* desc, const void* packed, const float* z, const float* h,
                              int64_t h_rows, const int64_t* cond_index, int64_t n_rows, float* y, float* ldj,
                              float* log_prob , void* scratch, void* stream);

int bcnf_nll_forward(const BcnfStackDesc* desc, const void* packed, const float* y, const float* h, int64_t batch,
                     float* z, float* ldj, int32_t training, uint64_t* rng_state, void* workspace, int32_t finalize,
                     float* loss_out, int32_t* guard, void* stream);

int bcnf_nll_backward(const BcnfStackDesc* desc, const void* packed, const float* h, const float* z,
                      const float* dloss, int64_t batch, int32_t training, void* workspace, float* dy,
                      float* dh, float* dparams, void* slab, float* loss_out, uint64_t* rng_state, int32_t* guard,
                      void* stream);

int64_t bcnf_grad_partials(int64_t total_numel);

int bcnf_adam_step(int32_t n_tensors, float* const* params, float* const* grads, float* const* exp_avg,
                   float* const* exp_avg_sq, const int64_t* numel, float* step, double lr, double beta1,
                   double beta2, double eps, double weight_decay, float* grad_partials, int32_t advance_step,
                   const int32_t* guard, void* stream);

int bcnf_adam_step_bookkeep(int32_t n_tensors, float* const* params, float* const* grads, float* const* exp_avg,
                            float* const* exp_avg_sq, const int64_t* numel, float* step, double lr, double beta1,
                            double beta2, double eps, double weight_decay, int64_t* advance_cursor,
                            int64_t cursor_modulo, const float* log_values, float* log_history, int32_t* done_counter,
                            const int32_t* guard, void* stream);

int bcnf_grad_sumsq(int32_t n_tensors, float* const* grads, const int64_t* numel, float* grad_partials, void* stream);

int bcnf_clip_grad_norm(int32_t n_tensors, float* const* grads, const int64_t* numel, const float* grad_partials,
                        float max_norm, float* total_norm, float* advance_step, int64_t* advance_cursor,
                        int64_t cursor_modulo, const float* log_values, float* log_history, const int32_t* guard,
                        void* stream);

#define BCNF_GUARD_CHECK 0
#define BCNF_GUARD_DIVERGED 1
#define BCNF_GUARD_HALTED 2
#define BCNF_GUARD_CHECK_GLOBAL 3
#define BCNF_GUARD_WORDS 4

int bcnf_guard_check_global(const float* global_values, int32_t* guard, void* stream);

int bcnf_advance_counters(float* step, int64_t* cursor, int64_t n_batches, void* stream);

int bcnf_gather_rows2(const int64_t* idx, int64_t n, const float* src0, int32_t cols0, float* dst0,
                      const float* src1, int32_t cols1, float* dst1, void* stream);
int bcnf_gather_batch(const int64_t* order, const int64_t* cursor, int64_t batch, const float* src0, int32_t cols0,
                      float* dst0, const float* src1, int32_t cols1, float* dst1, void* stream);

int bcnf_linear_forward(const float* x, const float* weight, const float* bias, int64_t rows, int32_t in_features,
                        int32_t out_features, float* y, void* stream);
int64_t bcnf_linear_work_bytes(int64_t rows, int32_t in_features, int32_t out_features);
int bcnf_linear_backward(const float* x, const float* weight, const float* dy, int64_t rows, int32_t in_features,
                         int32_t out_features, float* dx, float* dweight, float* dbias, void* work, void* stream);
int bcnf_linear_gelu_forward(const float* x, const float* weight, const float* bias, int64_t rows, int32_t in_features,
                             int32_t out_features, float p, const uint64_t* rng, int32_t salt, float* a, float* g,
                             void* stream);
int bcnf_linear_gelu_backward(const float* x, const float* weight, const float* da, const float* g, int64_t rows,
                              int32_t in_features, int32_t out_features, float* dx, float* dweight, float* dbias,
                              void* work, void* stream);

int bcnf_wide_supported(const BcnfStackDesc* desc);
int bcnf_wide_param_count(const BcnfStackDesc* desc, int64_t* n_trainable, int64_t* n_frozen);
int bcnf_wide_packed_bytes(const BcnfStackDesc* desc, int64_t* bytes);
int bcnf_wide_workspace_bytes(const BcnfStackDesc* desc, int64_t batch, int32_t save, int64_t* bytes);
int bcnf_wide_inverse_scratch_bytes(const BcnfStackDesc* desc, int64_t h_rows, int64_t n_rows, int64_t* bytes);
int bcnf_wide_pack(const BcnfStackDesc* desc, const float* params, const float* qmats, void* packed, void* stream);
int bcnf_wide_forward(const BcnfStackDesc* desc, const float* params, const void* packed, const float* y,
                      const float* h, int64_t batch, float* z, float* ldj, float* nll_part, int32_t training,
                      const uint64_t* rng_state, void* workspace, int32_t save, void* stream);
int bcnf_wide_nll_finalize(const BcnfStackDesc* desc, const void* workspace, int64_t batch, int32_t save,
                           float* loss_out, uint64_t* rng_state, int32_t* guard, void* stream);
int bcnf_wide_backward(const BcnfStackDesc* desc, const float* params, const void* packed, const float* h,
                       const float* z, const float* dz, const float* dldj, const float* dloss, int32_t nll,
                       int64_t batch, void* workspace, float* dy, float* dh, float* dparams, void* stream);
int bcnf_wide_fold_prepare(const BcnfStackDesc* desc, const void* packed, const float* wfb, int32_t xp, float* wcb,
// ... 73 lines not shown
```

Baseline: 30.88 million samples/s.

## Fuse fold forward and backward into one kernel with raw backward weight table

Adds a fused forward+backward launch for the folded NLL training step. It is armed with the known cotangent, so the backward reads weights straight from the raw parameter and Q buffers through a new backward gather table rather than a packed copy. The NLL finalize reduction is folded into the last block of the gx-reduce kernel to save a launch. The aim is fewer kernel launches and less packed-weight traffic per step. The cost is more code paths, higher register and LDS pressure in the fused kernel, and fallbacks whenever the cotangent does not match.

```diff
diff --git a/bcnf_amd/_native.py b/bcnf_amd/_native.py
--- a/bcnf_amd/_native.py
+++ b/bcnf_amd/_native.py
@@ -26,6 +26,8 @@
     "bcnf_gather_batch", "bcnf_advance_counters", "bcnf_fold_bytes", "bcnf_fold_slab_bytes",
     "bcnf_pack_params_fold", "bcnf_fold_nll_forward", "bcnf_fold_backward_tail",
     "bcnf_fold_raw_table_bytes", "bcnf_fold_raw_table", "bcnf_fold_train_forward", "bcnf_lds_fill",
+    "bcnf_fold_train_fb", "bcnf_fold_backward_tail_fin", "bcnf_fold_nll_backward_raw",
+    "bcnf_fold_raw_btable_bytes", "bcnf_fold_raw_btable",
     "bcnf_wide_supported", "bcnf_wide_param_count", "bcnf_wide_packed_bytes", "bcnf_wide_workspace_bytes", "bcnf_wide_inverse_scratch_bytes",
     "bcnf_wide_pack", "bcnf_wide_forward", "bcnf_wide_nll_finalize", "bcnf_wide_backward", "bcnf_wide_inverse",
     "bcnf_wide_fold_prepare", "bcnf_wide_fold_forward", "bcnf_wide_fold_backward", "bcnf_wide_proj_rows",
@@ -150,6 +152,14 @@
                                            _vp, _vp, _i32, _vp, _vp, _i32, _vp, _vp, _vp]),
         "bcnf_fold_backward_tail": (_i32, [_pdesc, _vp, _vp, _vp, _i32, _i32, _vp, _vp, _vp, _i64, _i32, _vp, _vp,
                                            _vp, _vp, _vp]),
+        "bcnf_fold_raw_btable_bytes": (_i32, [_pdesc, _i32, _pi64]),
+        "bcnf_fold_raw_btable": (_i32, [_pdesc, _i32, _vp]),
+        "bcnf_fold_train_fb": (_i32, [_pdesc, _vp, _vp, _vp, _vp, _vp, _vp, _i32, _vp, _vp, _vp, _i32, _i64, _vp, _vp, _vp,
+                                      _i32, _vp, _vp, _vp, _vp, _vp]),
+        "bcnf_fold_backward_tail_fin": (_i32, [_pdesc, _vp, _vp, _vp, _i32, _i32, _vp, _vp, _vp, _i64, _i32, _vp,
+                                               _vp, _vp, _vp, _vp, _vp, _vp, _vp]),
+        "bcnf_fold_nll_backward_raw": (_i32, [_pdesc, _vp, _vp, _vp, _i32, _vp, _vp, _i64, _i32, _vp, _vp, _vp, _vp,
+                                              _vp, _vp]),
         "bcnf_grad_partials": (_i64, [_i64]),
         "bcnf_adam_step": (_i32, [_i32, _vp, _vp, _vp, _vp, _vp, _vp, ctypes.c_double, ctypes.c_double,
                                   ctypes.c_double, ctypes.c_double, ctypes.c_double, _vp, _i32, _vp, _vp]),
diff --git a/bcnf_amd/csrc/bcnf_stack.hip b/bcnf_amd/csrc/bcnf_stack.hip
--- a/bcnf_amd/csrc/bcnf_stack.hip
+++ b/bcnf_amd/csrc/bcnf_stack.hip
@@ -339,15 +339,15 @@
 
 long long raw_table_words(const BcnfLayout& L) { return (long long)RAW_NSP * BCNF_WG + 16LL * L.RB; }
 
-bool build_raw_table(const BcnfLayout& L, uint32_t* out) {
-  if (L.nb < 2 || 16 * L.RF > RAW_DUMMY || L.blk_stride >= RAW_SRC_MAX) return false;
+bool build_raw_slots(const BcnfLayout& L, int RW, int (*source)(const BcnfLayout&, int, int, int*), uint32_t* out) {
+  if (L.nb < 2 || 16 * RW > RAW_DUMMY || L.blk_stride >= RAW_SRC_MAX) return false;
   std::vector<std::pair<int, int>> ent[3];
   for (int j = 0; j < 16; ++j)
-    for (int e = 0; e < L.RF; ++e) {
+    for (int e = 0; e < RW; ++e) {
       int off;
-      const int kind = rec_f_source(L, j, e, &off);
+      const int kind = source(L, j, e, &off);
       if (kind < 0) return false;
-      ent[kind == 1 ? 0 : kind == 2 ? 1 : 2].emplace_back(off, j * L.RF + e);
+      ent[kind == 1 ? 0 : kind == 2 ? 1 : 2].emplace_back(off, j * RW + e);
     }
   const int cap[3] = {RAW_NP, RAW_NQ, RAW_NZ}, first[3] = {0, RAW_NP, RAW_NP + RAW_NQ};
   for (int i = 0; i < RAW_NSP * BCNF_WG; ++i) out[i] = raw_entry(RAW_DUMMY, 0);
@@ -358,6 +358,11 @@
     for (int n = 0; n < (int)ent[g].size(); ++n)
       out[(n % BCNF_WG) * RAW_NSP + first[g] + n / BCNF_WG] = raw_entry(ent[g][n].second, ent[g][n].first);
   }
+  return true;
+}
+
+bool build_raw_table(const BcnfLayout& L, uint32_t* out) {
+  if (!build_raw_slots(L, L.RF, rec_f_source, out)) return false;
   uint32_t* pb = out + (long long)RAW_NSP * BCNF_WG;
   for (int j = 0; j < 16; ++j)
     for (int e = 0; e < L.RB; ++e) {
@@ -368,6 +373,9 @@
     }
   return true;
 }
+
+long long raw_btable_words() { return (long long)RAW_NSP * BCNF_WG; }
+bool build_raw_btable(const BcnfLayout& L, uint32_t* out) { return build_raw_slots(L, L.RB, rec_b_source, out); }
 
 constexpr int PACK_WG_MAX = 4096;
 
@@ -977,6 +985,22 @@
   gx_reduce_body(total, work, splits, gx, (long long)blockIdx.x * BCNF_WG + threadIdx.x);
 }
 
+template <int NTH, int WIDE>
+__device__ void nll_finalize(const float* __restrict__ part, int nparts, long long B, float* __restrict__ loss_out,
+                             uint64_t* rng_w, int32_t* guard, float* __restrict__ red);
+
+__global__ __launch_bounds__(BCNF_WG) void k_fold_gx_fin(long long total, const float* __restrict__ work, int splits,
+                                                         float* __restrict__ gx, const float* __restrict__ part,
+                                                         int nparts, long long B, float* __restrict__ loss_out,
+                                                         uint64_t* rng_w, int32_t* guard) {
+  __shared__ float red[BCNF_WG];
+  if (blockIdx.x + 1 == gridDim.x) {
+    nll_finalize<BCNF_WG, 2>(part, nparts, B, loss_out, rng_w, guard, red);
+    return;
+  }
+  gx_reduce_body(total, work, splits, gx, (long long)blockIdx.x * BCNF_WG + threadIdx.x);
+}
+
 __device__ __forceinline__ int c0_of_finish(int bx, int nct) { return (bx % nct) * 16; }
 
 constexpr int FIN_KC = 512;
@@ -1317,6 +1341,7 @@
   const float* P;
   const float* Q;
   const uint32_t* table;
+  const uint32_t* btable;
   const float* wf;
   const float* bf;
   const float* ypool;
@@ -1342,14 +1367,14 @@
 constexpr int FWD_HP = FWD_SLOTS * 4 * 256;
 constexpr int FWD_HEAD = 24;
 
-template <int NH, bool DROP, bool SAVE, bool RAW = false>
-__global__ __launch_bounds__(2 * BCNF_WG) void k_forward(BcnfLayout L, const float* __restrict__ pk,
-                                                    const float* __restrict__ y, ProjArgs P,
-                                                    long long B, float* __restrict__ z, float* __restrict__ ldj_out,
-                                                    float* __restrict__ logp, const uint64_t* rng,
-                                                    float* __restrict__ arec, float* __restrict__ nll_part,
-                                                    RawArgs R) {
-  extern __shared__ __attribute__((aligned(16))) float smem[];
+template <int NH, bool DROP, bool SAVE, bool RAW, bool FUSED>
+__device__ __forceinline__ void fwd_body(float* __restrict__ smem, const BcnfLayout& L, const float* __restrict__ pk,
+                                         const float* __restrict__ y, const ProjArgs& P, long long B,
+                                         float* __restrict__ z, float* __restrict__ ldj_out,
+                                         float* __restrict__ logp, const uint64_t* rng, float* __restrict__ arec,
+                                         float* __restrict__ nll_part, const RawArgs& R, float& ya_out,
+                                         float& yb_out) {
+  static_assert(!FUSED || (RAW && SAVE), "the fused launch is the pack-free saving forward");
   const int RFL = 16 * L.RF;
   float* rec = smem;
   float* hpb = rec + FWD_SLOTS * RING;
@@ -1530,6 +1555,7 @@
       finish_proj(1, gb[1]);
       auto side_unit = [&](int u, uint32_t e) {
         if (u < nb * ch) {
+          if constexpr (FUSED) return;
           const int k = u / ch, n = (u - k * ch) * BCNF_WG + t8;
           if (n >= rb16) return;
           const uint32_t kind = e & 3u, src = e >> 2;
@@ -1838,12 +1864,14 @@
     }
     if constexpr (RAW) ldc = ((lps[0] + lps[1]) + lps[2]) + lps[3];
     const float ltot = row_sum16(ldj) + ldc;
-    const float q2 = row_sum16(ya * ya + yb * yb);
+    const float q2 = row_sum16(FUSED ? fmaf(yb, yb, ya * ya) : ya * ya + yb * yb);
     if (j < Da) z[bc * D + j] = ya;
     if (j < Db) z[bc * D + Da + j] = yb;
     if (j == 0 && ldj_out) ldj_out[bc] = ltot;
     if (logp && j == 0) logp[bc] = -(0.5f * q2 - ltot) - 0.5f * (float)D * 1.8378770664093454836f;
     if (nll_part && j == 0) rec[s] = (b < B) ? 0.5f * q2 - ltot : 0.f;
+    ya_out = ya;
+    yb_out = yb;
   }
 #if BCNF_STAMPS
   if (SAVE && blockIdx.x == 0 && (threadIdx.x == 0 || threadIdx.x == BCNF_WG))
@@ -1858,6 +1886,7 @@
 #undef PHF
 #undef PHB
 #undef PHP
+  if constexpr (FUSED) return;
   if (nll_part) {
     __syncthreads();
     if (threadIdx.x == 0) {
@@ -1868,11 +1897,28 @@
   }
 }
 
-template <int NTH = BCNF_WG>
+template <int NH, bool DROP, bool SAVE, bool RAW = false>
+__global__ __launch_bounds__(2 * BCNF_WG) void k_forward(BcnfLayout L, const float* __restrict__ pk,
+                                                    const float* __restrict__ y, ProjArgs P,
+                                                    long long B, float* __restrict__ z, float* __restrict__ ldj_out,
+                                                    float* __restrict__ logp, const uint64_t* rng,
+                                                    float* __restrict__ arec, float* __restrict__ nll_part,
+                                                    RawArgs R) {
+  extern __shared__ __attribute__((aligned(16))) float smem[];
+  float ya, yb;
+  fwd_body<NH, DROP, SAVE, RAW, false>(smem, L, pk, y, P, B, z, ldj_out, logp, rng, arec, nll_part, R, ya, yb);
+}
+
+template <int NTH = BCNF_WG, int WIDE = 1>
 __device__ void nll_finalize(const float* __restrict__ part, int nparts, long long B, float* __restrict__ loss_out,
                              uint64_t* rng_w, int32_t* guard, float* __restrict__ red) {
   float acc = 0.f;
-  for (int i = threadIdx.x; i < nparts; i += NTH) acc += part[i];
+  for (int i = threadIdx.x; i < nparts; i += NTH * WIDE) acc += part[i];
+  if (WIDE == 2) {
+    float hi = 0.f;
+    for (int i = threadIdx.x + NTH; i < nparts; i += NTH * WIDE) hi += part[i];
+    acc += hi;
+  }
   red[threadIdx.x] = acc;
   __syncthreads();
   for (int w = NTH / 2; w > 0; w >>= 1) {
@@ -2242,23 +2288,20 @@
 constexpr int BWD_WG = 2 * BCNF_WG;
 constexpr int BWD_G4 = 3;
 
-template <int NH>
-__global__ __launch_bounds__(BWD_WG) void k_backward(BcnfLayout L, const float* __restrict__ pk,
-                                                     const float* __restrict__ dz, const float* __restrict__ dldj,
-                                                     const float* __restrict__ dloss, int nll, long long B,
-                                                     const float* __restrict__ arec,
-                                                     float* __restrict__ dy, float* __restrict__ d1,
-                                                     float* __restrict__ slab_all, long long slab_stride,
-                                                     const float* __restrict__ nll_part, float* __restrict__ loss_out,
-                                                     uint64_t* rng_w, int32_t* guard) {
+template <int NH, bool RAWB, bool FUSED>
+__device__ __forceinline__ void bwd_body(float* __restrict__ recB, float* __restrict__ dT, const BcnfLayout& L,
+                                         const float* __restrict__ pk, const float* __restrict__ dz,
+                                         const float* __restrict__ dldj, const float* __restrict__ dloss, int nll,
+                                         long long B, const float* __restrict__ arec, float* __restrict__ dy,
+                                         float* __restrict__ d1, float* __restrict__ slab_all, long long slab_stride,
+                                         const float* __restrict__ nll_part, float* __restrict__ loss_out,
+                                         uint64_t* rng_w, int32_t* guard, const RawArgs& R, float ya_in,
+                                         float yb_in) {
   static_assert(NH + 3 <= 4 * BWD_G4, "derivative slot");
-  extern __shared__ __attribute__((aligned(16))) float smem[];
   using AR = ActRec<NH>;
   using RBk = RecB<NH>;
   using J = BwdJobs<NH>;
   const int RBL = 16 * L.RB;
-  float* recB = smem;
-  float* dT = recB + 2 * RING;
   float* aT = dT + 2 * J::ND * TILE;
   floatx4* gsl = reinterpret_cast<floatx4*>(aT + 3 * J::NA * TILE);
   const int nb = L.nb;
@@ -2280,8 +2323,45 @@
     float* slab = slab_all + (long long)blockIdx.x * slab_stride;
     const floatx4* arl = reinterpret_cast<const floatx4*>(arec) + (long long)blockIdx.x * AR::AR4 * BCNF_WG + t8;
     const long long ars = (long long)gridDim.x * AR::AR4 * BCNF_WG;
+    constexpr int NWD = RAWB ? RAW_NP + RAW_NQ : 1;
+    uint32_t srcb[NWD], dstb[NWD], sab[2] = {0, 0};
+    bool an_word = false, q_diag[RAW_NQ] = {};
+    float an_val = 0.f;
+    const __amdgpu_buffer_rsrc_t rP = __builtin_amdgcn_make_buffer_rsrc(const_cast<float*>(R.P), (short)0,
+                                                                       (int)(L.n_trainable * 4), 0x00020000);
+    const __amdgpu_buffer_rsrc_t rQ = __builtin_amdgcn_make_buffer_rsrc(const_cast<float*>(R.Q), (short)0,
+                                                                       (nb - 1) * L.D * L.D * 4, 0x00020000);
+    if constexpr (RAWB) {
+      uint32_t tw[RAW_NSP];
+#pragma unroll
+      for (int i = 0; i < RAW_NSP / 4; ++i) {
+        const uint4 v = reinterpret_cast<const uint4*>(R.btable + t8 * RAW_NSP)[i];
+        tw[4 * i] = v.x;
+        tw[4 * i + 1] = v.y;
+        tw[4 * i + 2] = v.z;
+        tw[4 * i + 3] = v.w;
+      }
+#pragma unroll
+      for (int i = 0; i < NWD; ++i) {
+        srcb[i] = (tw[i] >> 12) * 4u;
+        dstb[i] = (tw[i] & 4095u) * 4u;
+      }
+#pragma unroll
+      for (int i = 0; i < RAW_NZ; ++i) {
+        const uint32_t z = tw[RAW_NP + RAW_NQ + i] & 4095u;
+        recB[z] = 0.f;
+        recB[RING + z] = 0.f;
+      }
+      an_word = (int)(srcb[0] >> 2) < L.an_size;
+      an_val = (int)(srcb[0] >> 2) < L.D ? 1.f : 0.f;
+#pragma unroll
+      for (int i = 0; i < RAW_NQ; ++i) q_diag[i] = ((srcb[RAW_NP + i] >> 2) % (uint32_t)(L.D + 1)) == 0;
+      sab[0] = j < L.Da ? (uint32_t)j * 4u : 0x7fff0000u;
+      sab[1] = j < L.Da ? (uint32_t)(L.D + j) * 4u : 0x7fff0000u;
+    }
     struct Prep {
-      Stage<STAGE_REC> sr;
+      Stage<RAWB ? 1 : STAGE_REC> sr;
+      float w[NWD];
       floatx4 rec[AR::AR4];
       float rec1[AR::AR1 > 0 ? AR::AR1 : 1];
       float sa, ba;
@@ -2289,21 +2369,55 @@
     const float* ar1l = arec + ar1_off(nb, gridDim.x, AR::AR4) + (long long)blockIdx.x * AR::AR1 * BCNF_WG + t8;
     const long long ar1s = (long long)gridDim.x * AR::AR1 * BCNF_WG;
     auto prep_load = [&](Prep& P, int k) {
-      P.sr.load_t(pbk + (long long)k * RBL, RBL, t8);
+      if constexpr (RAWB) {
+        const bool last = k == nb - 1;
+        const int sp = (last ? k * L.blk_stride - L.an_size : k * L.blk_stride) * 4, sq = k * L.D * L.D * 4;
+#pragma unroll
+        for (int i = 0; i < RAW_NP; ++i)
+          P.w[i] = __uint_as_float(__builtin_amdgcn_raw_buffer_load_b32(rP, srcb[i], sp, 0));
+#pragma unroll
+        for (int i = RAW_NP; i < NWD; ++i)
+          P.w[i] = __uint_as_float(__builtin_amdgcn_raw_buffer_load_b32(rQ, srcb[i], sq, 0));
+        P.sa = __uint_as_float(__builtin_amdgcn_raw_buffer_load_b32(rP, sab[0], sp, 0));
+        P.ba = __uint_as_float(__builtin_amdgcn_raw_buffer_load_b32(rP, sab[1], sp, 0));
+      } else {
+        P.sr.load_t(pbk + (long long)k * RBL, RBL, t8);
+      }
 #pragma unroll
       for (int i = 0; i < AR::AR4; ++i) P.rec[i] = arl[(long long)k * ars + i * BCNF_WG];
 #pragma unroll
       for (int i = 0; i < AR::AR1; ++i) P.rec1[i] = ar1l[(long long)k * ar1s + i * BCNF_WG];
-      const float* an = pbk + (long long)k * RBL + j * L.RB + RBk::AN;
-      P.sa = an[0];
-      P.ba = an[1];
+      if constexpr (!RAWB) {
+        const float* an = pbk + (long long)k * RBL + j * L.RB + RBk::AN;
+        P.sa = an[0];
+        P.ba = an[1];
+      }
     };
     auto prep_store = [&](Prep& P, int k) {
 #pragma unroll
       for (int i = 0; i < AR::AR4; ++i) asm volatile("" : "+v"(P.rec[i]));
 #pragma unroll
       for (int i = 0; i < AR::AR1; ++i) asm volatile("" : "+v"(P.rec1[i]));
-      asm volatile("" : "+v"(P.sa), "+v"(P.ba));
+      if constexpr (RAWB) {
+#pragma unroll
+        for (int i = 0; i < NWD; ++i) asm volatile("" : "+v"(P.w[i]));
+        asm volatile("" : "+v"(P.sa), "+v"(P.ba));
+        float wv[NWD];
+#pragma unroll
+        for (int i = 0; i < NWD; ++i) wv[i] = P.w[i];
+        if (k == nb - 1) {
+          wv[0] = an_word ? an_val : wv[0];
+#pragma unroll
+          for (int i = 0; i < RAW_NQ; ++i) wv[RAW_NP + i] = q_diag[i] ? 1.f : wv[RAW_NP + i];
+          P.sa = j < L.Da ? 1.f : 0.f;
+          P.ba = 0.f;
+        }
+        char* slot = reinterpret_cast<char*>(recB + (k & 1) * RING);
+#pragma unroll
+        for (int i = 0; i < NWD; ++i) *reinterpret_cast<float*>(slot + dstb[i]) = wv[i];
+      } else {
+        asm volatile("" : "+v"(P.sa), "+v"(P.ba));
+      }
       float ar[4 * AR::AR4 + AR::AR1];
 #pragma unroll
       for (int i = 0; i < AR::AR4; ++i) {
@@ -2329,7 +2443,7 @@
       floatx4* gd = gsl + (k & 1) * BWD_G4 * BCNF_WG + t8;
 #pragma unroll
       for (int i = 0; i < BWD_G4; ++i) gd[i * BCNF_WG] = floatx4{gs[4 * i], gs[4 * i + 1], gs[4 * i + 2], gs[4 * i + 3]};
-      P.sr.store_t(recB + (k & 1) * RING, t8);
+      if constexpr (!RAWB) P.sr.store_t(recB + (k & 1) * RING, t8);
     };
     Prep Pa, Pb;
     prep_load(Pa, nb - 1);
@@ -2368,8 +2482,8 @@
     if (valid) {
       if (nll) {
         const float sc = (dloss ? dloss[0] + dloss[1] : 1.f) / (float)B;
-        gya = (j < Da) ? dz[b * D + j] * sc : 0.f;
-        gyb = (j < Db) ? dz[b * D + Da + j] * sc : 0.f;
+        gya = (j < Da) ? (FUSED ? ya_in : dz[b * D + j]) * sc : 0.f;
+        gyb = (j < Db) ? (FUSED ? yb_in : dz[b * D + Da + j]) * sc : 0.f;
         dl = -sc;
       } else {
         if (dz) {
@@ -2456,10 +2570,67 @@
     for (int i = 0; i < 4; ++i) g_phase[(helper ? 4 : 0) + i] = ph_acc[i];
 #endif
 #undef PHS
+  if constexpr (FUSED) return;
   if (loss_out && blockIdx.x == 0) {
     __syncthreads();
     nll_finalize<BWD_WG>(nll_part, (int)gridDim.x, B, loss_out, rng_w, guard, dT);
   }
+}
+
+template <int NH>
+__global__ __launch_bounds__(BWD_WG) void k_backward(BcnfLayout L, const float* __restrict__ pk,
+                                                     const float* __restrict__ dz, const float* __restrict__ dldj,
+                                                     const float* __restrict__ dloss, int nll, long long B,
+                                                     const float* __restrict__ arec,
+                                                     float* __restrict__ dy, float* __restrict__ d1,
+                                                     float* __restrict__ slab_all, long long slab_stride,
+                                                     const float* __restrict__ nll_part, float* __restrict__ loss_out,
+                                                     uint64_t* rng_w, int32_t* guard) {
+  extern __shared__ __attribute__((aligned(16))) float smem[];
+  bwd_body<NH, false, false>(smem, smem + 2 * RING, L, pk, dz, dldj, dloss, nll, B, arec, dy, d1, slab_all,
+                             slab_stride, nll_part, loss_out, rng_w, guard, RawArgs{}, 0.f, 0.f);
+}
+
+template <int NH>
+__global__ __launch_bounds__(BWD_WG) void k_backward_raw(BcnfLayout L, const float* __restrict__ dz,
+                                                         const float* __restrict__ dloss, long long B,
+                                                         const float* __restrict__ arec, float* __restrict__ d1,
+                                                         float* __restrict__ slab_all, long long slab_stride,
+                                                         const float* __restrict__ nll_part,
+                                                         float* __restrict__ loss_out, uint64_t* rng_w,
+                                                         int32_t* guard, RawArgs R) {
+  extern __shared__ __attribute__((aligned(16))) float smem[];
+  bwd_body<NH, true, false>(smem, smem + 2 * RING, L, nullptr, dz, nullptr, dloss, 1, B, arec, nullptr, d1, slab_all,
+                            slab_stride, nll_part, loss_out, rng_w, guard, R, 0.f, 0.f);
+}
+
+constexpr int FB_RECB_OFF = FWD_SLOTS * RING + FWD_HP + FWD_SLOTS * 8 * 256 + 4;
+template <int NH, bool DROP>
+__global__ __launch_bounds__(2 * BCNF_WG) void k_train_fb(BcnfLayout L, ProjArgs P, long long B,
+                                                          float* __restrict__ z, float* __restrict__ ldj_out,
+                                                          const uint64_t* rng, float* __restrict__ arec,
+                                                          float* __restrict__ nll_part, RawArgs R,
+                                                          const float* __restrict__ dloss, float* __restrict__ d1,
+                                                          float* __restrict__ slab_all, long long slab_stride) {
+  extern __shared__ __attribute__((aligned(16))) float smem[];
+  static_assert(FB_RECB_OFF % 4 == 0, "16-byte aligned record ring");
+  static_assert(2 * BwdJobs<NH>::ND * TILE + 3 * BwdJobs<NH>::NA * TILE + 2 * BWD_G4 * 4 * BCNF_WG <= FB_RECB_OFF,
+                "the backward's tiles fit under its record ring");
+  float ya = 0.f, yb = 0.f;
+  fwd_body<NH, DROP, true, true, true>(smem, L, R.pk, R.ypool, P, B, z, ldj_out, nullptr, rng, arec, nll_part, R, ya,
+                                       yb);
+  if (threadIdx.x < BCNF_WG) {
+    __builtin_amdgcn_s_setprio(0);
+    asm volatile("s_waitcnt vmcnt(0)" ::: "memory");
+  }
+  __syncthreads();
+  if (threadIdx.x == 0) {
+    float acc = 0.f;
+    for (int i = 0; i < 16; ++i) acc += smem[i];
+    nll_part[blockIdx.x] = acc;
+  }
+  bwd_body<NH, true, true>(smem + FB_RECB_OFF, smem, L, nullptr, nullptr, nullptr, dloss, 1, B, arec, nullptr, d1,
+                           slab_all, slab_stride, nullptr, nullptr, nullptr, nullptr, R, ya, yb);
 }
 
 template <int N>
@@ -2593,7 +2764,7 @@
                                                        const float* __restrict__ slab, long long stride, int nwg,
                                                        float* __restrict__ dparams, const float* __restrict__ wf,
                                                        const float* __restrict__ bf, float* __restrict__ wf1,
-                                                       FoldAdamArgs A) {
+                                                       FoldAdamArgs A, int fin_after) {
   extern __shared__ __attribute__((aligned(16))) float smem[];
   const int bx = blockIdx.x;
   if (bx < n_sk) {
@@ -2618,7 +2789,7 @@
     if (A.on && threadIdx.x == 0) adam_scalars_publish(A);
     return;
   }
-  if (A.on && !(A.guard && A.guard[BCNF_GUARD_HALTED])) {
+  if (A.on && !(A.guard && (A.guard[BCNF_GUARD_HALTED] || (fin_after && A.guard[BCNF_GUARD_DIVERGED])))) {
     reduce_body(L, slab, stride, nwg, dparams, bx - n_sk - 1, smem, &A);
     return;
   }
@@ -2707,6 +2878,34 @@
   const dim3 grid((unsigned)((B + 15) / 16));
   return launch<k_backward<NH>>(grid, dim3(BWD_WG), bwd_lds_bytes(L), st, L, pk, dz, dldj, dloss, nll, B, arec, dy, d1,
                                 slab, stride, part, loss_out, rng_w, guard);
+}
+
+template <int NH>
+int bwd_raw_dispatch(const BcnfLayout& L, const RawArgs& R, const float* z, const float* dloss, long long B,
+                     const float* arec, float* d1, float* slab, long long stride, const float* part, float* loss_out,
+                     uint64_t* rng_w, int32_t* guard, hipStream_t st) {
+  if (!layout_matches<NH>(L)) return BCNF_ERR_ARG;
+  const dim3 grid((unsigned)((B + 15) / 16));
+  return launch<k_backward_raw<NH>>(grid, dim3(BWD_WG), bwd_lds_bytes(L), st, L, z, dloss, B, arec, d1, slab, stride,
+                                    part, loss_out, rng_w, guard, R);
+}
+
+size_t fb_lds_bytes(const BcnfLayout& L) {
+  return std::max(fwd2_lds_bytes(L, true), sizeof(float) * (size_t)(FB_RECB_OFF + 2 * RING));
+}
+
+template <int NH>
+int fb_dispatch(const BcnfLayout& L, const RawArgs& R, const ProjArgs& P, long long B, float* z, float* ldj, bool drop,
+                const uint64_t* rng, float* arec, float* part, const float* dloss, float* d1, float* slab,
+                long long stride, hipStream_t st) {
+  if (!layout_matches<NH>(L)) return BCNF_ERR_ARG;
+  if (P.Cp % 16 != 0 || P.Cp / 16 > HP_SMAX || P.C > P.Cp) return BCNF_ERR_UNSUPPORTED;
+  const dim3 grid((unsigned)((B + 15) / 16));
+  const size_t lds = fb_lds_bytes(L);
+  return drop ? launch<k_train_fb<NH, true>>(grid, dim3(2 * BCNF_WG), lds, st, L, P, B, z, ldj, rng, arec, part, R,
+                                             dloss, d1, slab, stride)
+              : launch<k_train_fb<NH, false>>(grid, dim3(2 * BCNF_WG), lds, st, L, P, B, z, ldj, rng, arec, part, R,
+                                              dloss, d1, slab, stride);
 }
 
 constexpr int W1H_ROWS_PER_SPLIT = KC;
@@ -2903,98 +3102,9 @@
 bool raw_applicable(const BcnfLayout& L, int X) {
   return X <= RAW_KP - 4 && L.C <= 64 * RAW_TPW && L.nb >= 2 && L.act_norm;
 }
-}
-
-int bcnf_fold_bytes(const BcnfStackDesc* desc, int32_t in_features, int64_t* bytes) {
-  BcnfLayout L;
-  const int rc = fold_setup(desc, in_features, &L);
-  if (rc) return rc;
-  if (!bytes) return BCNF_ERR_ARG;
-  *bytes = fold_floats(L, in_features) * 4;
-  return BCNF_OK;
-}
-
-int bcnf_fold_slab_bytes(const BcnfStackDesc* desc, int32_t in_features, int64_t batch, int64_t* bytes) {
-  BcnfLayout L;
-  const int rc = fold_setup(desc, in_features, &L);
-  if (rc) return rc;
-  if (!bytes || batch < 0) return BCNF_ERR_ARG;
-  const BcnfLayout F = fold_layout(L, in_features, in_features);
-  *bytes = ((int64_t)((batch + 15) / 16) * slab_stride_of(L) + w1h_work_floats(F, batch) +
-            (int64_t)L.nb * 16 * F.Cp + 4 +
-            (int64_t)L.C * (in_features + 1)) * 4;
-  return BCNF_OK;
-}
-
-int bcnf_pack_params_fold(const BcnfStackDesc* desc, const float* params, const float* qmats,
-                          const float* feat_weight, const float* feat_bias, int32_t in_features, void* packed,
-                          float* fold, const BcnfGather2* gather, void* stream) {
-  BcnfLayout L;
-  int rc = fold_setup(desc, in_features, &L);
-  if (rc) return rc;
-  if (!params || !packed || !fold || !feat_weight || (L.nb > 1 && !qmats)) return BCNF_ERR_ARG;
-  BcnfGatherArgs ga = {};
-  if (gather) {
-    const BcnfGather2& g = *gather;
-    if (g.n < 1 || g.cols0 < 1 || g.cols1 < 1 || !g.idx || !g.src0 || !g.dst0 || !g.src1 || !g.dst1)
-      return BCNF_ERR_ARG;
-    if (g.n * (int64_t)(g.cols0 + g.cols1) >= (1LL << 31)) return BCNF_ERR_UNSUPPORTED;
-    ga = BcnfGatherArgs{g.idx, (const long long*)g.cursor, g.src0, g.dst0, g.src1, g.dst1, (int)g.n, 0, g.cols0,
-                        g.cols1, 0};
-    gather2_plan(g.n, &ga.rpw, &ga.nwg);
-  }
-  const int npw = pack_wgs(L, true);
-  const unsigned grid = (unsigned)(L.NKp / 16 * FOLD_SPLIT + ga.nwg + npw + 1);
-  return launch<k_pack_fold>(dim3(grid), dim3(BCNF_WG), 0, (hipStream_t)stream, L, params, qmats, (float*)packed,
-                             feat_weight, feat_bias, (int)in_features, fold, ga, npw);
-}
-
-int bcnf_fold_nll_forward(const BcnfStackDesc* desc, const void* packed, const float* fold, int32_t in_features,
-                          const float* y, const float* x, int32_t ldx, int64_t batch, float* z, float* ldj, int32_t training,
-                          uint64_t* rng_state, void* workspace, int32_t finalize, float* loss_out, int32_t* guard,
-                          void* stream) {
-  BcnfLayout L;
-  const int rc = fold_setup(desc, in_features, &L);
-  if (rc) return rc;
-  if (!fold || ldx < in_features) return BCNF_ERR_ARG;
-  return forward_impl(desc, packed, y, x, batch, z, ldj, nullptr, training, rng_state, workspace, true, true,
-                      finalize != 0, loss_out, guard, stream, fold, in_features, ldx);
-}
-
-int bcnf_lds_fill(float value, void* stream) {
-  return launch<k_fill_lds>(dim3(4 * 256), dim3(BCNF_WG), LDS_MAX, (hipStream_t)stream, value);
-}
-
-int bcnf_fold_raw_table_bytes(const BcnfStackDesc* desc, int32_t in_features, int64_t* bytes) {
-  BcnfLayout L;
-  const int rc = fold_setup(desc, in_features, &L);
-  if (rc) return rc;
-  if (!bytes) return BCNF_ERR_ARG;
-  if (!raw_applicable(L, in_features)) return BCNF_ERR_UNSUPPORTED;
-  std::vector<uint32_t> t((size_t)raw_table_words(L));
-  if (!build_raw_table(L, t.data())) return BCNF_ERR_UNSUPPORTED;
-  *bytes = (int64_t)t.size() * (int64_t)sizeof(uint32_t);
-  return BCNF_OK;
-}
-
-int bcnf_fold_raw_table(const BcnfStackDesc* desc, int32_t in_features, void* host_table) {
-  BcnfLayout L;
-  const int rc = fold_setup(desc, in_features, &L);
-  if (rc) return rc;
-  if (!host_table) return BCNF_ERR_ARG;
-  if (!raw_applicable(L, in_features)) return BCNF_ERR_UNSUPPORTED;
-  return build_raw_table(L, (uint32_t*)host_table) ? BCNF_OK : BCNF_ERR_UNSUPPORTED;
-}
-
-int bcnf_fold_train_forward(const BcnfStackDesc* desc, const float* params, const float* qmats, const void* table,
-                            const float* feat_weight, const float* feat_bias, int32_t in_features,
-                            const BcnfGather2* gather, const float* y, const float* x, int32_t ldx, int64_t batch,
-                            void* packed, float* z, float* ldj, int32_t training, uint64_t* rng_state,
-                            void* workspace, int32_t finalize, float* loss_out, int32_t* guard, void* stream) {
-  BcnfLayout L;
-  const int rc = fold_setup(desc, in_features, &L);
-  if (rc) return rc;
-  if (!raw_applicable(L, in_features)) return BCNF_ERR_UNSUPPORTED;
+int raw_args_setup(const BcnfLayout& L, const float* params, const float* qmats, const void* table,
+                   const float* feat_weight, const float* feat_bias, int32_t in_features, const BcnfGather2* gather,
+                   const float* y, const float* x, int32_t ldx, int64_t batch, void* packed, RawArgs* out) {
   if (!params || !qmats || !table || !feat_weight || !packed || batch < 1) return BCNF_ERR_ARG;
   RawArgs R = {};
   R.P = params;
@@ -3022,19 +3132,142 @@
     R.xpool = x;
     R.ldx = ldx;
   }
+  *out = R;
+  return BCNF_OK;
+}
+}
+
+int bcnf_fold_bytes(const BcnfStackDesc* desc, int32_t in_features, int64_t* bytes) {
+  BcnfLayout L;
+  const int rc = fold_setup(desc, in_features, &L);
+  if (rc) return rc;
+  if (!bytes) return BCNF_ERR_ARG;
+  *bytes = fold_floats(L, in_features) * 4;
+  return BCNF_OK;
+}
+
+int bcnf_fold_slab_bytes(const BcnfStackDesc* desc, int32_t in_features, int64_t batch, int64_t* bytes) {
+  BcnfLayout L;
+  const int rc = fold_setup(desc, in_features, &L);
+  if (rc) return rc;
+  if (!bytes || batch < 0) return BCNF_ERR_ARG;
+  const BcnfLayout F = fold_layout(L, in_features, in_features);
+  *bytes = ((int64_t)((batch + 15) / 16) * slab_stride_of(L) + w1h_work_floats(F, batch) +
+            (int64_t)L.nb * 16 * F.Cp + 4 +
+            (int64_t)L.C * (in_features + 1)) * 4;
+  return BCNF_OK;
+}
+
+int bcnf_pack_params_fold(const BcnfStackDesc* desc, const float* params, const float* qmats,
+                          const float* feat_weight, const float* feat_bias, int32_t in_features, void* packed,
+                          float* fold, const BcnfGather2* gather, void* stream) {
+  BcnfLayout L;
+  int rc = fold_setup(desc, in_features, &L);
+  if (rc) return rc;
+  if (!params || !packed || !fold || !feat_weight || (L.nb > 1 && !qmats)) return BCNF_ERR_ARG;
+  BcnfGatherArgs ga = {};
+  if (gather) {
+    const BcnfGather2& g = *gather;
+    if (g.n < 1 || g.cols0 < 1 || g.cols1 < 1 || !g.idx || !g.src0 || !g.dst0 || !g.src1 || !g.dst1)
+      return BCNF_ERR_ARG;
+    if (g.n * (int64_t)(g.cols0 + g.cols1) >= (1LL << 31)) return BCNF_ERR_UNSUPPORTED;
+    ga = BcnfGatherArgs{g.idx, (const long long*)g.cursor, g.src0, g.dst0, g.src1, g.dst1, (int)g.n, 0, g.cols0,
+                        g.cols1, 0};
+    gather2_plan(g.n, &ga.rpw, &ga.nwg);
+  }
+  const int npw = pack_wgs(L, true);
+  const unsigned grid = (unsigned)(L.NKp / 16 * FOLD_SPLIT + ga.nwg + npw + 1);
+  return launch<k_pack_fold>(dim3(grid), dim3(BCNF_WG), 0, (hipStream_t)stream, L, params, qmats, (float*)packed,
+                             feat_weight, feat_bias, (int)in_features, fold, ga, npw);
+}
+
+int bcnf_fold_nll_forward(const BcnfStackDesc* desc, const void* packed, const float* fold, int32_t in_features,
+                          const float* y, const float* x, int32_t ldx, int64_t batch, float* z, float* ldj, int32_t training,
+                          uint64_t* rng_state, void* workspace, int32_t finalize, float* loss_out, int32_t* guard,
+                          void* stream) {
+  BcnfLayout L;
+  const int rc = fold_setup(desc, in_features, &L);
+  if (rc) return rc;
+  if (!fold || ldx < in_features) return BCNF_ERR_ARG;
+  return forward_impl(desc, packed, y, x, batch, z, ldj, nullptr, training, rng_state, workspace, true, true,
+                      finalize != 0, loss_out, guard, stream, fold, in_features, ldx);
+}
+
+int bcnf_lds_fill(float value, void* stream) {
+  return launch<k_fill_lds>(dim3(4 * 256), dim3(BCNF_WG), LDS_MAX, (hipStream_t)stream, value);
+}
+
+int bcnf_fold_raw_table_bytes(const BcnfStackDesc* desc, int32_t in_features, int64_t* bytes) {
+  BcnfLayout L;
+  const int rc = fold_setup(desc, in_features, &L);
+  if (rc) return rc;
+  if (!bytes) return BCNF_ERR_ARG;
+  if (!raw_applicable(L, in_features)) return BCNF_ERR_UNSUPPORTED;
+  std::vector<uint32_t> t((size_t)raw_table_words(L));
+  if (!build_raw_table(L, t.data())) return BCNF_ERR_UNSUPPORTED;
+  *bytes = (int64_t)t.size() * (int64_t)sizeof(uint32_t);
+  return BCNF_OK;
+}
+
+int bcnf_fold_raw_table(const BcnfStackDesc* desc, int32_t in_features, void* host_table) {
+  BcnfLayout L;
+  const int rc = fold_setup(desc, in_features, &L);
+  if (rc) return rc;
+  if (!host_table) return BCNF_ERR_ARG;
+  if (!raw_applicable(L, in_features)) return BCNF_ERR_UNSUPPORTED;
+  return build_raw_table(L, (uint32_t*)host_table) ? BCNF_OK : BCNF_ERR_UNSUPPORTED;
+}
+
+int bcnf_fold_raw_btable_bytes(const BcnfStackDesc* desc, int32_t in_features, int64_t* bytes) {
+  BcnfLayout L;
+  const int rc = fold_setup(desc, in_features, &L);
+  if (rc) return rc;
+  if (!bytes) return BCNF_ERR_ARG;
+  if (!raw_applicable(L, in_features)) return BCNF_ERR_UNSUPPORTED;
+  std::vector<uint32_t> t((size_t)raw_btable_words());
+  if (!build_raw_btable(L, t.data())) return BCNF_ERR_UNSUPPORTED;
+  *bytes = (int64_t)t.size() * (int64_t)sizeof(uint32_t);
+  return BCNF_OK;
+}
+
+int bcnf_fold_raw_btable(const BcnfStackDesc* desc, int32_t in_features, void* host_table) {
+  BcnfLayout L;
+  const int rc = fold_setup(desc, in_features, &L);
+  if (rc) return rc;
+  if (!host_table) return BCNF_ERR_ARG;
+  if (!raw_applicable(L, in_features)) return BCNF_ERR_UNSUPPORTED;
+  return build_raw_btable(L, (uint32_t*)host_table) ? BCNF_OK : BCNF_ERR_UNSUPPORTED;
+}
+
+int bcnf_fold_train_forward(const BcnfStackDesc* desc, const float* params, const float* qmats, const void* table,
+                            const float* feat_weight, const float* feat_bias, int32_t in_features,
+                            const BcnfGather2* gather, const float* y, const float* x, int32_t ldx, int64_t batch,
+                            void* packed, float* z, float* ldj, int32_t training, uint64_t* rng_state,
+                            void* workspace, int32_t finalize, float* loss_out, int32_t* guard, void* stream) {
+  BcnfLayout L;
+  int rc = fold_setup(desc, in_features, &L);
+  if (rc) return rc;
+  if (!raw_applicable(L, in_features)) return BCNF_ERR_UNSUPPORTED;
+  RawArgs R;
+  if ((rc = raw_args_setup(L, params, qmats, table, feat_weight, feat_bias, in_features, gather, y, x, ldx, batch,
+                           packed, &R)))
+    return rc;
   return forward_impl(desc, packed, R.ypool, R.xpool, batch, z, ldj, nullptr, training, rng_state, workspace, true,
                       true, finalize != 0, loss_out, guard, stream, nullptr, 0, 0, &R);
 }
 
-int bcnf_fold_backward_tail(const BcnfStackDesc* desc, const void* packed, const void* slab, const float* x,
-                            int32_t ldx, int32_t in_features, const float* feat_weight, const float* feat_bias,
-                            const void* workspace, int64_t batch, int32_t training, float* dparams,
-                            float* dfeat_weight, float* dfeat_bias, const BcnfFoldAdam* adam, void* stream) {
+namespace {
+int fold_tail_impl(const BcnfStackDesc* desc, const void* packed, const void* slab, const float* x,
+                   int32_t ldx, int32_t in_features, const float* feat_weight, const float* feat_bias,
+                   const void* workspace, int64_t batch, int32_t training, float* dparams,
+                   float* dfeat_weight, float* dfeat_bias, const BcnfFoldAdam* adam, float* loss_out,
+                   uint64_t* rng_state, int32_t* guard, void* stream) {
   BcnfLayout L;
   int rc = fold_setup(desc, in_features, &L);
   if (rc) return rc;
   if (!packed || !slab || !x || !feat_weight || !workspace || !dparams || batch < 1 || ldx < in_features)
     return BCNF_ERR_ARG;
+  const int fin_after = loss_out != nullptr;
   FoldAdamArgs A = {};
   if (adam) {
     const BcnfFoldAdam& a = *adam;
@@ -3084,18 +3317,98 @@
   const bool nt3 = (F.Cp >> 4) <= 6;
 #define FOLD_TAIL(V, NT)                                                                                          \
   launch<k_fold_tail<V, NT>>(grid, dim3(BCNF_WG), lds, st, L, F, d1, x, (long long)batch, rps, work, gx_dw, (int)n_sk, \
-                             (int)in_features, (const float*)slab, S, nwg, dparams, feat_weight, feat_bias, wf1, A)
+                             (int)in_features, (const float*)slab, S, nwg, dparams, feat_weight, feat_bias, wf1, A, \
+                             fin_after)
   rc = vec ? (nt3 ? FOLD_TAIL(true, 3) : FOLD_TAIL(true, 8)) : (nt3 ? FOLD_TAIL(false, 3) : FOLD_TAIL(false, 8));
 #undef FOLD_TAIL
   if (rc) return rc;
   const long long total = (long long)L.nb * 16 * F.Cp;
-  rc = launch<k_fold_gx>(dim3((unsigned)((total + BCNF_WG - 1) / BCNF_WG)), dim3(BCNF_WG), 0, st, total,
-                         (const float*)work, (int)splits, gx);
+  const unsigned n_gx = (unsigned)((total + BCNF_WG - 1) / BCNF_WG);
+  if (fin_after) {
+    const bool drop = training && L.p > 0.f;
+    if (drop && !rng_state) return BCNF_ERR_ARG;
+    rc = launch<k_fold_gx_fin>(dim3(n_gx + 1), dim3(BCNF_WG), 0, st, total, (const float*)work, (int)splits, gx,
+                               (const float*)workspace + ws_part_off(L, batch), nwg, (long long)batch, loss_out,
+                               drop ? rng_state : nullptr, guard);
+  } else {
+    rc = launch<k_fold_gx>(dim3(n_gx), dim3(BCNF_WG), 0, st, total, (const float*)work, (int)splits, gx);
+  }
   if (rc) return rc;
   const int n_fin = (L.nb + (F.Cp >> 4)) * (L.Cp >> 4);
   return launch<k_fold_finish>(dim3((unsigned)n_fin), dim3(BCNF_WG), sizeof(float) * FIN_SMEM, st, L,
                                (const float*)packed, (const float*)gx, (const float*)wf1, bf1, (int)in_features,
                                dparams, dfeat_weight, dfeat_bias, A);
+}
+}
+
+int bcnf_fold_backward_tail(const BcnfStackDesc* desc, const void* packed, const void* slab, const float* x,
+                            int32_t ldx, int32_t in_features, const float* feat_weight, const float* feat_bias,
+                            const void* workspace, int64_t batch, int32_t training, float* dparams,
+                            float* dfeat_weight, float* dfeat_bias, const BcnfFoldAdam* adam, void* stream) {
+  return fold_tail_impl(desc, packed, slab, x, ldx, in_features, feat_weight, feat_bias, workspace, batch, training,
+                        dparams, dfeat_weight, dfeat_bias, adam, nullptr, nullptr, nullptr, stream);
+}
+
+int bcnf_fold_backward_tail_fin(const BcnfStackDesc* desc, const void* packed, const void* slab, const float* x,
+                                int32_t ldx, int32_t in_features, const float* feat_weight, const float* feat_bias,
+                                const void* workspace, int64_t batch, int32_t training, float* dparams,
+                                float* dfeat_weight, float* dfeat_bias, const BcnfFoldAdam* adam, float* loss_out,
+                                uint64_t* rng_state, int32_t* guard, void* stream) {
+  if (!loss_out) return BCNF_ERR_ARG;
+  return fold_tail_impl(desc, packed, slab, x, ldx, in_features, feat_weight, feat_bias, workspace, batch, training,
+                        dparams, dfeat_weight, dfeat_bias, adam, loss_out, rng_state, guard, stream);
+}
+
+int bcnf_fold_train_fb(const BcnfStackDesc* desc, const float* params, const float* qmats, const void* table,
+                       const void* btable, const float* feat_weight, const float* feat_bias, int32_t in_features,
+                       const BcnfGather2* gather, const float* y, const float* x, int32_t ldx, int64_t batch,
+                       void* packed, float* z, float* ldj, int32_t training, const uint64_t* rng_state,
+                       void* workspace, const float* dloss, void* slab, void* stream) {
+  BcnfLayout L;
+  int rc = fold_setup(desc, in_features, &L);
+  if (rc) return rc;
+  if (!raw_applicable(L, in_features)) return BCNF_ERR_UNSUPPORTED;
+  RawArgs R;
+  if ((rc = raw_args_setup(L, params, qmats, table, feat_weight, feat_bias, in_features, gather, y, x, ldx, batch,
+                           packed, &R)))
+    return rc;
+  if (!z || !workspace || !dloss || !slab || !btable) return BCNF_ERR_ARG;
+  R.btable = (const uint32_t*)btable;
+  const bool drop = training && L.p > 0.f;
+  if (drop && !rng_state) return BCNF_ERR_ARG;
+  float* ws = (float*)workspace;
+  const float* pk = (const float*)packed;
+  const ProjArgs P{R.xpool, pk + L.w1c_off, pk + L.b1c_off, (long long)L.ldh, L.C, L.Cp, L.NKp};
+  switch (L.NH) {
+#define BCNF_CASE(N) case N: return fb_dispatch<N>(L, R, P, batch, z, ldj, drop, rng_state, ws, ws + ws_part_off(L, batch), dloss, ws + ws_d1_off(L, batch), (float*)slab, slab_stride_of(L), (hipStream_t)stream);
+    BCNF_CASE(1) BCNF_CASE(2) BCNF_CASE(3) BCNF_CASE(4) BCNF_CASE(5) BCNF_CASE(6) BCNF_CASE(7) BCNF_CASE(8)
+#undef BCNF_CASE
+    default: return BCNF_ERR_UNSUPPORTED;
+  }
+}
+
+int bcnf_fold_nll_backward_raw(const BcnfStackDesc* desc, const float* params, const float* qmats, const void* btable,
+                               int32_t in_features, const float* z, const float* dloss, int64_t batch,
+                               int32_t training, void* workspace, void* slab, float* loss_out, uint64_t* rng_state,
+                               int32_t* guard, void* stream) {
+  BcnfLayout L;
+  const int rc = fold_setup(desc, in_features, &L);
+  if (rc) return rc;
+  if (!raw_applicable(L, in_features)) return BCNF_ERR_UNSUPPORTED;
+  if (!params || !qmats || !btable || !z || !workspace || !slab || batch < 1) return BCNF_ERR_ARG;
+  RawArgs R = {};
+  R.P = params;
+  R.Q = qmats;
+  R.btable = (const uint32_t*)btable;
+  const bool drop = training && L.p > 0.f;
+  float* ws = (float*)workspace;
+  uint64_t* rng_w = (loss_out && drop) ? rng_state : nullptr;
+  switch (L.NH) {
+#define BCNF_CASE(N) case N: return bwd_raw_dispatch<N>(L, R, z, dloss, batch, ws, ws + ws_d1_off(L, batch), (float*)slab, slab_stride_of(L), ws + ws_part_off(L, batch), loss_out, rng_w, guard, (hipStream_t)stream);
+    BCNF_CASE(1) BCNF_CASE(2) BCNF_CASE(3) BCNF_CASE(4) BCNF_CASE(5) BCNF_CASE(6) BCNF_CASE(7) BCNF_CASE(8)
+#undef BCNF_CASE
+    default: return BCNF_ERR_UNSUPPORTED;
+  }
 }
 
 int bcnf_grad_reduce(const BcnfStackDesc* desc, const void* slab, const float* h, const void* workspace,
diff --git a/bcnf_amd/fused.py b/bcnf_amd/fused.py
--- a/bcnf_amd/fused.py
+++ b/bcnf_amd/fused.py
@@ -334,17 +334,25 @@
     def raw_table(self, X: int):
         if not self.use_raw_forward or not hasattr(N.lib(), "bcnf_fold_train_forward"):
             return None
+        return self._device_table("bcnf_fold_raw_table", X)
+
+    def raw_btable(self, X: int):
+        if not hasattr(N.lib(), "bcnf_fold_raw_btable"):
+            return None
+        return self._device_table("bcnf_fold_raw_btable", X)
+
+    def _device_table(self, name, X):
         dev = self.flat.device
-        key = (X, str(dev))
+        key = (name, X, str(dev))
         if key not in self._raw_tables:
             if torch.cuda.is_current_stream_capturing():
                 return None
-            rc, (nb,) = N.query_status("bcnf_fold_raw_table_bytes", self._pdesc, X)
+            rc, (nb,) = N.query_status(name + "_bytes", self._pdesc, X)
             if rc != N.OK:
                 self._raw_tables[key] = None
             else:
                 host = torch.empty(nb // 4, dtype=torch.int32)
-                N.call("bcnf_fold_raw_table", self._pdesc, X, host)
+                N.call(name, self._pdesc, X, host)
                 self._raw_tables[key] = host.to(dev)
         return self._raw_tables[key]
 
@@ -382,11 +390,44 @@
     pending_adam = None
     grad_bucket = None
 
-    def _fold_backward_calls(self, x, z, dvals, wf, bf, training, saved, want_feat, finalize_into=None, adam=None):
+    use_fused_fb = os.environ.get("BCNF_FUSE_FB", "0") != "0"
+    armed_cot = None
+
+    def fused_fb_applies(self, B: int, X: int) -> bool:
+        if not self.use_fused_fb or not hasattr(N.lib(), "bcnf_fold_train_fb") or self.raw_table(X) is None or \
+                self.raw_btable(X) is None:
+            return False
+        dev = self.flat.device
+        return (B + 15) // 16 <= torch.cuda.get_device_properties(dev).multi_processor_count
+
+    def _fold_slab(self, x):
+        B, X = x.shape
+        sb = N.query_i64("bcnf_fold_slab_bytes", self._pdesc, X, B)
+        return torch.empty(max(sb // 4, 1), dtype=torch.float32, device=x.device)
+
+    def launch_fold_train_fb(self, y, x, wf, bf, training: bool, cot, gather=None):
+        self._check_device(y, x, wf, bf)
+        B, X = x.shape
+        if y.dim() != 2 or y.shape != (B, self.cfg.size):
+            raise ValueError(f"bcnf_amd folded forward: y {tuple(y.shape)} vs x {tuple(x.shape)}")
+        pk = self._empty_pack()
+        z, ldj, rng, ws = self._forward_buffers(y, training)
+        vals = torch.empty(3, dtype=torch.float32, device=y.device)
+        slab = self._fold_slab(x)
+        N.call("bcnf_fold_train_fb", self._pdesc, self.flat, self.qflat, self.raw_table(X), self.raw_btable(X), wf, bf, X,
+               gather, y, x, x.stride(0), B, pk, z, ldj, training, rng, ws, cot, slab, N.stream_handle(y.device))
+        return z, ldj, vals, (ws, pk), slab
+
+    def launch_fold_tail_fin(self, x, wf, bf, training: bool, saved, slab, want_feat: bool, vals, adam=None):
         ws, pk = saved
         B, X = x.shape
-        sb = N.query_i64("bcnf_fold_slab_bytes", self._pdesc, X, B)
-        slab = torch.empty(max(sb // 4, 1), dtype=torch.float32, device=x.device)
+        dparams, dwf, dbf = self._fold_grad_buffers(wf, bf, want_feat)
+        rng = self.rng_state() if self._dropping(training) else None
+        N.call("bcnf_fold_backward_tail_fin", self._pdesc, pk, slab, x, x.stride(0), X, wf, bf, ws, B, training,
+               dparams, dwf, dbf, adam, vals, rng, self.guard, N.stream_handle(x.device))
+        return dparams, dwf, dbf
+
+    def _fold_grad_buffers(self, wf, bf, want_feat):
         gb = self.grad_bucket
         if gb is not None and want_feat:
             bucket, offs = gb
@@ -397,14 +438,29 @@
             dparams = torch.empty_like(self.flat)
             dwf = torch.empty_like(wf) if want_feat else None
             dbf = torch.empty_like(bf) if (want_feat and bf is not None) else None
+        return dparams, dwf, dbf
+
+    def _fold_backward_calls(self, x, z, dvals, wf, bf, training, saved, want_feat, finalize_into=None, adam=None,
+                             raw_records=False):
+        ws, pk = saved
+        B, X = x.shape
+        slab = self._fold_slab(x)
+        dparams, dwf, dbf = self._fold_grad_buffers(wf, bf, want_feat)
         tail = ("bcnf_fold_backward_tail", self._pdesc, pk, slab, x, x.stride(0), X, wf, bf, ws, B, training, dparams,
                 dwf, dbf, adam, N.stream_handle(x.device))
-        return ((self._nll_backward_call(x, z, dvals, training, saved, slab, None, finalize_into), tail),
-                (dparams, dwf, dbf))
+        if raw_records:
+            rng = self.rng_state() if (finalize_into is not None and self._dropping(training)) else None
+            backward = ("bcnf_fold_nll_backward_raw", self._pdesc, self.flat, self.qflat, self.raw_btable(X), X, z, dvals,
+                        B, training, ws, slab, finalize_into, rng, self.guard if finalize_into is not None else None,
+                        N.stream_handle(x.device))
+        else:
+            backward = self._nll_backward_call(x, z, dvals, training, saved, slab, None, finalize_into)
+        return (backward, tail), (dparams, dwf, dbf)
 
     def launch_fold_nll_backward(self, x, z, dvals, wf, bf, training: bool, saved, want_feat: bool,
-                                 finalize_into=None, adam=None):
-        launches, out = self._fold_backward_calls(x, z, dvals, wf, bf, training, saved, want_feat, finalize_into, adam)
+                                 finalize_into=None, adam=None, raw_records=False):
+        launches, out = self._fold_backward_calls(x, z, dvals, wf, bf, training, saved, want_feat, finalize_into, adam,
+                                                  raw_records)
         for launch in launches:
             N.call(*launch)
         return out
@@ -589,7 +645,14 @@
 
     @staticmethod
     def forward(ctx, y, x, wf, bf, flat_param, stack: FusedStack, training: bool, defer: bool, gather):
-        z, _, vals, saved = stack.launch_fold_nll_forward(y, x, wf, bf, training, finalize=not defer, gather=gather)
+        cot, stack.armed_cot = stack.armed_cot, None
+        ctx.fb_cot = ctx.slab = None
+        if defer and cot is not None and x.shape[0] > 0 and stack.fused_fb_applies(x.shape[0], x.shape[1]):
+            z, _, vals, saved, ctx.slab = stack.launch_fold_train_fb(y, x, wf, bf, training, cot, gather=gather)
+            ctx.fb_cot = cot
+        else:
+            z, _, vals, saved = stack.launch_fold_nll_forward(y, x, wf, bf, training, finalize=not defer,
+                                                              gather=gather)
         ctx.stack = stack
         ctx.training = training
         ctx.saved = saved
@@ -602,10 +665,17 @@
         x, wf, bf, z, vals = ctx.saved_tensors
         need = ctx.needs_input_grad
         adam, ctx.stack.pending_adam = ctx.stack.pending_adam, None
-        dparams, dwf, dbf = ctx.stack.launch_fold_nll_backward(x, z, dvals.contiguous(), wf, bf, ctx.training,
-                                                               ctx.saved, want_feat=need[2] or need[3] or
-                                                               adam is not None,
-                                                               finalize_into=vals if ctx.defer else None, adam=adam)
+        want_feat = need[2] or need[3] or adam is not None
+        dvals = dvals.contiguous()
+        fb = ctx.fb_cot is not None
+        if fb and dvals.data_ptr() == ctx.fb_cot.data_ptr() and dvals.shape == ctx.fb_cot.shape:
+            dparams, dwf, dbf = ctx.stack.launch_fold_tail_fin(x, wf, bf, ctx.training, ctx.saved, ctx.slab,
+                                                               want_feat, vals, adam=adam)
+        else:
+            dparams, dwf, dbf = ctx.stack.launch_fold_nll_backward(x, z, dvals, wf, bf, ctx.training, ctx.saved,
+                                                                   want_feat=want_feat,
+                                                                   finalize_into=vals if ctx.defer else None,
+                                                                   adam=adam, raw_records=fb)
         return (None, None, dwf if need[2] else None, dbf if need[3] else None, dparams if need[4] else None,
                 None, None, None, None)
 
diff --git a/bcnf_amd/train.py b/bcnf_amd/train.py
--- a/bcnf_amd/train.py
+++ b/bcnf_amd/train.py
@@ -144,9 +144,16 @@
     def _forward_backward_body(self, y, traj, gather=None, adam=None):
         self.opt.zero_grad(set_to_none=True)
         if self.fused_loss:
-            vals = self.model.nll_loss(y, traj, defer_reduction=True, gather=gather)
-            if self._cot is None or self._cot.device != vals.device:
-                self._cot = torch.tensor([1.0, 0.0, 0.0], device=vals.device)
+            st = self.model.fused
+            if self._cot is None or self._cot.device != self.params[0].device:
+                self._cot = torch.tensor([1.0, 0.0, 0.0], device=self.params[0].device)
+            if hasattr(st, "use_fused_fb"):
+                st.armed_cot = self._cot
+            try:
+                vals = self.model.nll_loss(y, traj, defer_reduction=True, gather=gather)
+            finally:
+                if hasattr(st, "use_fused_fb"):
+                    st.armed_cot = None
             if adam is not None:
                 self.model.fused.pending_adam = adam(vals)
             torch.autograd.backward(vals, self._cot)
diff --git a/include/bcnf_amd.h b/include/bcnf_amd.h
--- a/include/bcnf_amd.h
+++ b/include/bcnf_amd.h
@@ -110,6 +110,22 @@
                             const void* workspace, int64_t batch, int32_t training, float* dparams,
                             float* dfeat_weight, float* dfeat_bias, const BcnfFoldAdam* adam ,
                             void* stream);
+int bcnf_fold_raw_btable_bytes(const BcnfStackDesc* desc, int32_t in_features, int64_t* bytes);
+int bcnf_fold_raw_btable(const BcnfStackDesc* desc, int32_t in_features, void* host_table);
+int bcnf_fold_train_fb(const BcnfStackDesc* desc, const float* params, const float* qmats, const void* table,
+                       const void* btable, const float* feat_weight, const float* feat_bias, int32_t in_features,
+                       const BcnfGather2* gather , const float* y, const float* x, int32_t ldx,
+                       int64_t batch, void* packed, float* z, float* ldj, int32_t training,
+                       const uint64_t* rng_state, void* workspace, const float* dloss, void* slab, void* stream);
+int bcnf_fold_backward_tail_fin(const BcnfStackDesc* desc, const void* packed, const void* slab, const float* x,
+                                int32_t ldx, int32_t in_features, const float* feat_weight, const float* feat_bias,
+                                const void* workspace, int64_t batch, int32_t training, float* dparams,
+                                float* dfeat_weight, float* dfeat_bias, const BcnfFoldAdam* adam ,
+                                float* loss_out, uint64_t* rng_state, int32_t* guard , void* stream);
+int bcnf_fold_nll_backward_raw(const BcnfStackDesc* desc, const float* params, const float* qmats, const void* btable,
+                               int32_t in_features, const float* z, const float* dloss ,
+                               int64_t batch, int32_t training, void* workspace, void* slab,
+                               float* loss_out , uint64_t* rng_state, int32_t* guard, void* stream);
 
 int bcnf_grad_reduce(const BcnfStackDesc* desc, const void* slab, const float* h, const void* workspace,
                      int64_t batch, int32_t training, float* dparams, void* stream);
```

After: 29.99 million samples/s. 2.9% lower.
